# TropComplique/MultiPoseNet

Measured on AMD Instinct MI355X. Metric: images/sec keypoint fwd+bwd+Adam @512x512 bs32/GPU, higher is better.
Workload: dtype bf16; 1 GPU; MobileNet-v1+FPN+keypoint_subnet fwd+bwd+Adam, 512x512, per-GPU batch 32; global_batch=32, parallelism=dp1, hip_graph=True, rccl_ranks=1

## Files before the change

include/mpn.h:

```cpp
#ifndef MPN_H_
#define MPN_H_

#include <stddef.h>
#include <stdint.h>

#ifdef __cplusplus
extern "C" {
#endif

#define MPN_VERSION 600

enum { MPN_F32 = 0, MPN_BF16 = 1, MPN_F16 = 2  };

enum {
    MPN_OK = 0,
    MPN_ERR_BAD_SHAPE = -1,
    MPN_ERR_BAD_DTYPE = -2,
    MPN_ERR_BAD_ALIGN = -3,
    MPN_ERR_HIP = -4,
    MPN_ERR_BAD_ARG = -5,
    MPN_ERR_WORKSPACE = -6
};

enum { MPN_ACT_NONE = 0, MPN_ACT_RELU = 1, MPN_ACT_RELU6 = 2 };

typedef void* mpn_stream_t;

int mpn_version(void);
int mpn_last_error(char* buf, size_t n);

size_t mpn_heatmap_decode_workspace_bytes(int B);
int mpn_heatmap_decode(const void* heatmaps, int dtype, int B, int h, int w, int C,
                       const double* box_hw, float threshold,
                       int32_t* out_xyv, float* out_score, int32_t* out_index,
                       void* workspace, size_t workspace_bytes, mpn_stream_t stream);

size_t mpn_conv_packed_bytes(int Cin, int Cout, int ksize, int transpose, int dtype);
int mpn_conv_pack_weights(const float* w_hwio, int Cin, int Cout, int ksize, int transpose,
                          int dtype, void* out, mpn_stream_t stream);
size_t mpn_conv_pack_desc_bytes(void);
int mpn_conv_pack_desc_fill(void* desc_host, const float* w_hwio, int Cin, int Cout, int ksize, int transpose,
                            int dtype, void* out, int block_begin);
int mpn_conv_pack_weights_batched(const void* descs_device, int ndesc, int total_blocks, int dtype,
                                  mpn_stream_t stream);
int mpn_conv_num_parts(int N, int H, int W, int ksize);
int mpn_conv_stats_rows(int N, int H, int W, int Cin, int Cout, int ksize, int dtype);
int mpn_conv_fwd(const void* x, const void* w_packed, void* y, int N, int H, int W, int Cin,
                 int Cout, int x_stride, int y_stride, int ksize, int dtype, const float* in_scale,
                 const float* in_shift, int in_act, float* stats_part, const void* up_res,
                 mpn_stream_t stream);
int mpn_conv_fwd_grouped(int njobs, const void* const* x, const void* const* w_packed, void* const* y, int N, const int* H,
                         const int* W, int Cin, int Cout, const int* x_stride, const int* y_stride, int ksize, int dtype,
                         const float* const* in_scale, const float* const* in_shift, int in_act,
                         float* const* stats_part, mpn_stream_t stream);
int mpn_conv_bwd_data_bn_supported(int K, int C, int ksize, int dtype);
int mpn_conv_bwd_data_bn(const void* dy, const void* w_packed_t, void* dx, int N, int H, int W, int K, int C, int dy_stride,
                         int dx_stride, int ksize, int dtype, const void* bn_x, int bn_x_stride, const float* bn_scale,
                         const float* bn_shift, int bn_act, float* part, mpn_stream_t stream);
int mpn_conv_bwd_data_bn_grouped(int njobs, const void* const* dy, const void* const* w_packed_t, void* const* dx, int N,
                                 const int* H, const int* W, int K, int C, const int* dy_stride, const int* dx_stride,
                                 int dtype, const void* const* bn_x, const int* bn_x_stride, const float* const* bn_scale,
                                 const float* const* bn_shift, int bn_act, float* const* part, mpn_stream_t stream);

int mpn_conv_wgrad_num_parts(int N, int H, int W, int Cin, int Cout, int ksize, int dtype);
int mpn_conv_bwd_weight(const void* x, const void* dy, float* part, int N, int H, int W, int Cin,
                        int Cout, int x_stride, int dy_stride, int ksize, int dtype, const float* in_scale,
                        const float* in_shift, int in_act, mpn_stream_t stream);

int mpn_conv1x1_bwd_fused_supported(int Cin, int Cout, int dtype);
int mpn_conv1x1_bwd_fused(const void* x, const void* dy, const float* w, void* dx, float* wpart, float* bn_part, int N, int H, int W,
                          int Cin, int Cout, int x_stride, int dy_stride, int dx_stride, int dtype, const float* in_scale,
                          const float* in_shift, int in_act, mpn_stream_t stream);
int mpn_conv1x1_bwd_fused_apply_supported(int Cin, int Cout, int dtype);
int mpn_conv1x1_bwd_fused_apply(const void* x, const void* g, const void* y_raw, const float* w, void* dx, float* wpart, float* bn_part,
                                int N, int H, int W, int Cin, int Cout, int x_stride, int g_stride, int y_stride, int dx_stride,
                                int dtype, const float* in_scale, const float* in_shift, int in_act, const float* ap_scale,
                                const float* ap_shift, const float* ap_mean, const float* ap_invstd, const float* ap_k1,
                                const float* ap_k2, int ap_act, mpn_stream_t stream);
int mpn_conv_wgrad_grouped_num_parts(int njobs, int N, const int* H, const int* W, int Cin, int Cout, int ksize, int dtype,
                                     int* nparts);
int mpn_conv_bwd_weight_grouped(int njobs, const void* const* x, const void* const* dy, float* const* part, int N,
                                const int* H, const int* W, int Cin, int Cout, const int* x_stride, const int* dy_stride,
                                int ksize, int dtype, const float* const* in_scale, const float* const* in_shift,
                                int in_act, mpn_stream_t stream);

int mpn_bn_stats_num_parts(long long M);
int mpn_bn_stats(const void* x, long long M, int C, int dtype, float* part, mpn_stream_t stream);
int mpn_bn_finalize(float* part, int nparts, int C, long long count, const float* gamma,
                    const float* beta, float* moving_mean, float* moving_var, float momentum,
                    float eps, float* scale, float* shift, float* save_mean, float* save_invstd,
                    mpn_stream_t stream);
int mpn_bn_bwd_reduce_grouped(int njobs, void* const* dA, const void* const* x, const long long* M, int C, int dtype,
                              const float* const* scale, const float* const* shift, const float* const* mean,
                              const float* const* invstd, int act, float* const* part, const int* dA_stride,
                              const int* x_stride, mpn_stream_t stream);
int mpn_bn_bwd_apply_grouped(int njobs, void* const* dA, const void* const* x, const long long* M, int C, int dtype,
                             const float* const* scale, const float* const* shift, const float* const* mean,
                             const float* const* invstd, const float* const* k1, const float* const* k2, int act,
                             const float* const* add_ch0, const int* dA_stride, const int* x_stride,
                             mpn_stream_t stream);
size_t mpn_bn_fin_desc_bytes(void);
size_t mpn_bn_bwd_fin_desc_bytes(void);
int mpn_bn_fin_desc_fill(void* desc_host, const float* part, int nparts, int C, long long count, const float* gamma,
                         const float* beta, float* moving_mean, float* moving_var, float* scale, float* shift,
                         float* save_mean, float* save_invstd, int block_begin);
int mpn_bn_bwd_fin_desc_fill(void* desc_host, const float* part, int nparts, int C, long long count, float* dgamma,
                             float* dbeta, float* k1, float* k2, int block_begin);
int mpn_bn_bwd_fin_desc_fill_raw(void* desc_host, const float* part, int nparts, int C, long long count, float* dgamma,
                                 float* dbeta, float* k1, float* k2, const float* mean, const float* invstd,
                                 int block_begin);
int mpn_bn_finalize_batched(const void* descs_device, int ndesc, int total_blocks, float momentum, float eps,
                            mpn_stream_t stream);
int mpn_bn_bwd_finalize_batched(const void* descs_device, int ndesc, int total_blocks, mpn_stream_t stream);
int mpn_bn_inference_affine(int C, const float* gamma, const float* beta, const float* moving_mean,
                            const float* moving_var, float eps, float* scale, float* shift,
                            mpn_stream_t stream);
int mpn_bn_act_apply(const void* x, void* y, long long M, int C, int dtype, const float* scale,
                     const float* shift, int act, mpn_stream_t stream);
int mpn_bn_bwd_reduce(const void* dA, const void* x, long long M, int C, int dtype,
                      const float* scale, const float* shift, const float* mean,
                      const float* invstd, int act, float* part, mpn_stream_t stream);
int mpn_bn_bwd_finalize(float* part, int nparts, int C, long long count, float* dgamma,
                        float* dbeta, float* k1, float* k2, mpn_stream_t stream);
int mpn_bn_bwd_finalize_raw(float* part, int nparts, int C, long long count, float* dgamma, float* dbeta, float* k1,
                            float* k2, const float* mean, const float* invstd, mpn_stream_t stream);
int mpn_bn_bwd_apply(void* dA, const void* x, long long M, int C, int dtype, const float* scale,
                     const float* shift, const float* mean, const float* invstd, const float* k1,
                     const float* k2, int act, const float* add_ch0, mpn_stream_t stream);

int mpn_dwconv_out_size(int size, int stride);
int mpn_dwconv_num_parts(int N, int H, int W, int C, int stride, int dtype);
int mpn_dwconv_fwd(const void* x, const float* w, void* y, int N, int H, int W, int C, int stride,
                   int dtype, const float* in_scale, const float* in_shift, int in_act, int flip,
                   float* stats_part, mpn_stream_t stream);
int mpn_dwconv_bwd_data(const void* dy, const float* w, void* dx, int N, int H, int W, int C,
                        int stride, int dtype, mpn_stream_t stream);
int mpn_dwconv_bwd_data_bn_num_parts(int N, int H, int W, int C, int stride, int dtype);
int mpn_dwconv_bwd_data_bn(const void* dy, const float* w, void* dx, int N, int H, int W, int C, int stride, int dtype,
                           const void* x_bn, const float* scale, const float* shift, const float* mean,
                           const float* invstd, int act, float* part, mpn_stream_t stream);
int mpn_dwconv_bwd_data_add_supported(int N, int H, int W, int C, int stride, int dtype);
int mpn_dwconv_bwd_data_add(const void* dy, const float* w, void* dx, int N, int H, int W, int C, int stride, int dtype,
                            const void* addend, const void* x_bn, const float* scale, const float* shift,
                            const float* mean, const float* invstd, int act, float* part, mpn_stream_t stream);
int mpn_dwconv_wgrad_num_parts(int N, int H, int W, int C, int stride, int dtype);
int mpn_dwconv_bwd_weight(const void* x, const void* dy, float* part, int N, int H, int W, int C,
                          int stride, int dtype, const float* in_scale, const float* in_shift,
                          int in_act, mpn_stream_t stream);

int mpn_dwconv_bwd_fused_supported(int N, int H, int W, int C, int stride, int dtype);
int mpn_dwconv_bwd_fused(const void* x, const void* dy, const float* w, void* dx, float* wpart, int N, int H, int W, int C,
                         int dtype, const float* in_scale, const float* in_shift, int in_act, const float* mean,
                         const float* invstd, float* bn_part, mpn_stream_t stream);
int mpn_dwconv_bwd_fused_s2(const void* x, const void* dy, const float* w, void* dx, float* wpart, int N, int H, int W, int C,
                            int dtype, const float* in_scale, const float* in_shift, int in_act, const float* mean,
                            const float* invstd, float* bn_part, const void* addend, mpn_stream_t stream);

int mpn_stem_conv_fwd(const void* images, int images_u8, const float* w, void* y, int N, int H,
                      int W, int C0, int dtype, mpn_stream_t stream);
int mpn_stem_conv_fwd_num_parts(int N, int H, int W, int C0, int dtype);
int mpn_stem_conv_fwd_stats(const void* images, int images_u8, const float* w, void* y, int N, int H, int W, int C0,
                            int dtype, float* stats_part, mpn_stream_t stream);
int mpn_stem_conv_wgrad_num_parts(int N, int H, int W);
int mpn_stem_conv_bwd_weight(const void* images, int images_u8, const void* dy, float* part, int N,
                             int H, int W, int C0, int dtype, mpn_stream_t stream);

int mpn_bilinear_up_fwd(const void* x, void* y, int N, int h, int w, int C, int upsample,
                        int y_channel_offset, int y_channels_total, int dtype,
                        const float* in_scale, const float* in_shift, int in_act,
                        mpn_stream_t stream);
int mpn_bilinear_up_bwd(const void* dy, void* dx, int N, int h, int w, int C, int upsample,
                        int y_channel_offset, int y_channels_total, int dtype, mpn_stream_t stream);
int mpn_sumpool2x2(const void* src, void* dst, int N, int h, int w, int C, int accumulate,
                   int dtype, mpn_stream_t stream);
int mpn_add_inplace(void* dst, const void* src, long long n, int dtype, mpn_stream_t stream);

int mpn_heatmap_head_fwd(const void* x, const float* w, const float* bias, long long M, int Cin,
                         int dtype, const float* in_scale, const float* in_shift, int in_act,
                         int mode, float* out, float* out_seg, mpn_stream_t stream);
int mpn_heatmap_head_bwd_num_parts(long long M);
int mpn_heatmap_head_bwd(const void* x, const float* dlogits, const float* w, long long M, int Cin,
                         int dtype, const float* in_scale, const float* in_shift, int in_act,
                         void* dA, float* part, mpn_stream_t stream);
int mpn_heatmap_head_bwd_bn_supported(int Cin, int dtype);
int mpn_heatmap_head_bwd_bn(const void* x, const float* dlogits, const float* w, long long M, int Cin, int dtype,
                            const float* in_scale, const float* in_shift, int in_act, void* dA, float* part,
                            float* bn_part, mpn_stream_t stream);

int mpn_keypoint_loss_num_parts(int B, int h, int w);
int mpn_keypoint_loss(const float* logits, const float* heatmaps, const float* loss_masks,
                      const float* segmentation_masks, const int* num_boxes, const void* p2,
                      const void* p3, const void* p4, const void* p5, int p_channels, int p_dtype,
                      float* dlogits, float* daux2, float* daux3, float* daux4, float* daux5,
                      float* part, float* losses_out, int B, int h, int w, mpn_stream_t stream);

int mpn_adam_prepare(long long* step, float* hyper, double initial_learning_rate,
                     double decay_steps, double alpha, double beta1, double beta2,
                     mpn_stream_t stream);
int mpn_adam_step(float* params, const float* grads, float* m, float* v, long long n,
                  const float* hyper, float beta1, float beta2, float eps, float clip,
                  float grad_scale, mpn_stream_t stream);
int mpn_adam_step_cast(float* params, const float* grads, float* m, float* v, long long n, const float* hyper, float beta1,
                       float beta2, float eps, float clip, float grad_scale, int ncast, const long long* cast_begin,
                       const long long* cast_count, void* const* cast_dst, int cast_dtype, mpn_stream_t stream);
int mpn_reduce_partials(const float* part, int nparts, long long n, float* out, int accumulate,
                        float scale, mpn_stream_t stream);
size_t mpn_reduce_desc_bytes(void);
int mpn_reduce_desc_fill(void* desc_host, const float* part, int nparts, long long n, float* out, float scale,
                         int block_begin);
int mpn_reduce_partials_batched(const void* descs_device, int ndesc, int total_blocks, mpn_stream_t stream);
int mpn_axpy(long long n, float a, const float* x, float* y, mpn_stream_t stream);
int mpn_axpy_batched(int count, const float* const* x, float* const* y, const long long* n, float a, mpn_stream_t stream);
int mpn_l2_loss_accumulate(long long n, const float* w, float scale, float* acc, mpn_stream_t stream);
size_t mpn_l2_loss_batched_workspace_bytes(int count, const long long* n);
int mpn_l2_loss_batched(int count, const float* const* w, const long long* n, float scale, float* acc, void* workspace,
                        size_t workspace_bytes, mpn_stream_t stream);

size_t mpn_heatmap_render_workspace_bytes(int total_persons);
int mpn_heatmap_render(const int32_t* keypoints, const float* boxes, const int32_t* first_person,
                       int B, int total_persons, int width, int height, int downsample, float* out,
                       void* workspace, size_t workspace_bytes, mpn_stream_t stream);

enum {
    MPN_AUGMENT_ROTATE = 1, MPN_AUGMENT_COLOR = 2, MPN_AUGMENT_GRAYSCALE = 4, MPN_AUGMENT_PIXEL_SCALE = 8,
    MPN_AUGMENT_FLIP = 16, MPN_AUGMENT_EVAL = 32
};
#define MPN_KEYPOINT_AUGMENT_DESC_BYTES 192
typedef struct mpn_keypoint_augment_desc {
    int64_t src_offset, mask_offset;
    int32_t src_h, src_w, mask_h, mask_w;
    int32_t crop_y, crop_x, crop_h, crop_w;
    int32_t valid_h, valid_w, valid_mh, valid_mw;
    float transform[8], mask_transform[8];
    float window[4];
    float scale_y, scale_x;
    float mask_scale_y, mask_scale_x;
    float color[3];
    uint32_t seed;
    int32_t flags;
    int32_t reserved[3];
} mpn_keypoint_augment_desc;
#ifdef __cplusplus
static_assert(sizeof(mpn_keypoint_augment_desc) == MPN_KEYPOINT_AUGMENT_DESC_BYTES, "descriptor size is fixed");
#endif
size_t mpn_keypoint_augment_desc_bytes(void);
int mpn_keypoint_augment(const uint8_t* sources, const uint8_t* masks, const void* descs, int B, int H, int W,
                         float* images, float* loss_masks, float* segmentation_masks, mpn_stream_t stream);

// ... 89 lines not shown
```

multiposenet_amd/_lib.py:

```python
import ctypes
import os

_HERE = os.path.dirname(os.path.abspath(__file__))
LIB_PATH = os.environ.get("MPN_LIB") or os.path.join(_HERE, "libmpn_hip.so")

MPN_VERSION = 600
MPN_F32, MPN_BF16, MPN_F16 = 0, 1, 2
ACT_NONE, ACT_RELU, ACT_RELU6 = 0, 1, 2

_c = ctypes
_P = _c.c_void_p
_I = _c.c_int
_F = _c.c_float
_D = _c.c_double
_Z = _c.c_size_t
_L = _c.c_longlong

SIGNATURES = {
    "mpn_version": (_I, []),
    "mpn_last_error": (_I, [_c.c_char_p, _Z]),
    "mpn_heatmap_decode_workspace_bytes": (_Z, [_I]),
    "mpn_heatmap_decode": (_I, [_P, _I, _I, _I, _I, _I, _P, _F, _P, _P, _P, _P, _Z, _P]),
    "mpn_heatmap_render_workspace_bytes": (_Z, [_I]),
    "mpn_heatmap_render": (_I, [_P, _P, _P, _I, _I, _I, _I, _I, _P, _P, _Z, _P]),
    "mpn_keypoint_augment_desc_bytes": (_Z, []),
    "mpn_keypoint_augment": (_I, [_P, _P, _P, _I, _I, _I, _P, _P, _P, _P]),
    "mpn_detector_augment_desc_bytes": (_Z, []),
    "mpn_detector_augment": (_I, [_P, _P, _I, _I, _I, _P, _P]),
    "mpn_prn_example_desc_bytes": (_Z, []),
    "mpn_prn_examples_workspace_bytes": (_Z, [_I]),
    "mpn_prn_examples": (_I, [_P, _P, _I, _P, _P, _P, _I, _P, _I, _I, _I, _I, _P, _P, _P, _Z, _P]),
    "mpn_conv_packed_bytes": (_Z, [_I, _I, _I, _I, _I]),
    "mpn_conv_pack_weights": (_I, [_P, _I, _I, _I, _I, _I, _P, _P]),
    "mpn_conv_pack_desc_bytes": (_Z, []),
    "mpn_conv_pack_desc_fill": (_I, [_P, _P, _I, _I, _I, _I, _I, _P, _I]),
    "mpn_conv_pack_weights_batched": (_I, [_P, _I, _I, _I, _P]),
    "mpn_conv_num_parts": (_I, [_I, _I, _I, _I]),
    "mpn_conv_stats_rows": (_I, [_I, _I, _I, _I, _I, _I, _I]),
    "mpn_conv_fwd": (_I, [_P, _P, _P, _I, _I, _I, _I, _I, _I, _I, _I, _I, _P, _P, _I, _P, _P, _P]),
    "mpn_conv_fwd_grouped": (_I, [_I, _P, _P, _P, _I, _P, _P, _I, _I, _P, _P, _I, _I, _P, _P, _I, _P, _P]),
    "mpn_conv_wgrad_num_parts": (_I, [_I, _I, _I, _I, _I, _I, _I]),
    "mpn_conv_bwd_weight": (_I, [_P, _P, _P, _I, _I, _I, _I, _I, _I, _I, _I, _I, _P, _P, _I, _P]),
    "mpn_conv1x1_bwd_fused_supported": (_I, [_I, _I, _I]),
    "mpn_conv1x1_bwd_fused": (_I, [_P, _P, _P, _P, _P, _P, _I, _I, _I, _I, _I, _I, _I, _I, _I, _P, _P, _I, _P]),
    "mpn_conv1x1_bwd_fused_apply_supported": (_I, [_I, _I, _I]),
    "mpn_conv1x1_bwd_fused_apply": (_I, [_P, _P, _P, _P, _P, _P, _P, _I, _I, _I, _I, _I, _I, _I, _I, _I, _I, _P, _P, _I, _P, _P, _P, _P, _P, _P, _I, _P]),
    "mpn_conv_wgrad_grouped_num_parts": (_I, [_I, _I, _P, _P, _I, _I, _I, _I, _P]),
    "mpn_conv_bwd_weight_grouped": (_I, [_I, _P, _P, _P, _I, _P, _P, _I, _I, _P, _P, _I, _I, _P, _P, _I, _P]),
    "mpn_bn_stats_num_parts": (_I, [_L]),
    "mpn_bn_stats": (_I, [_P, _L, _I, _I, _P, _P]),
    "mpn_bn_finalize": (_I, [_P, _I, _I, _L, _P, _P, _P, _P, _F, _F, _P, _P, _P, _P, _P]),
    "mpn_bn_inference_affine": (_I, [_I, _P, _P, _P, _P, _F, _P, _P, _P]),
    "mpn_bn_act_apply": (_I, [_P, _P, _L, _I, _I, _P, _P, _I, _P]),
    "mpn_bn_bwd_reduce": (_I, [_P, _P, _L, _I, _I, _P, _P, _P, _P, _I, _P, _P]),
    "mpn_bn_bwd_finalize": (_I, [_P, _I, _I, _L, _P, _P, _P, _P, _P]),
    "mpn_bn_bwd_apply": (_I, [_P, _P, _L, _I, _I, _P, _P, _P, _P, _P, _P, _I, _P, _P]),
    "mpn_dwconv_out_size": (_I, [_I, _I]),
    "mpn_dwconv_num_parts": (_I, [_I, _I, _I, _I, _I, _I]),
    "mpn_dwconv_fwd": (_I, [_P, _P, _P, _I, _I, _I, _I, _I, _I, _P, _P, _I, _I, _P, _P]),
    "mpn_dwconv_bwd_data": (_I, [_P, _P, _P, _I, _I, _I, _I, _I, _I, _P]),
    "mpn_dwconv_bwd_data_bn_num_parts": (_I, [_I, _I, _I, _I, _I, _I]),
    "mpn_dwconv_bwd_data_bn": (_I, [_P, _P, _P, _I, _I, _I, _I, _I, _I, _P, _P, _P, _P, _P, _I, _P, _P]),
    "mpn_dwconv_bwd_data_add_supported": (_I, [_I, _I, _I, _I, _I, _I]),
    "mpn_dwconv_bwd_data_add": (_I, [_P, _P, _P, _I, _I, _I, _I, _I, _I, _P, _P, _P, _P, _P, _P, _I, _P, _P]),
    "mpn_dwconv_wgrad_num_parts": (_I, [_I, _I, _I, _I, _I, _I]),
    "mpn_dwconv_bwd_weight": (_I, [_P, _P, _P, _I, _I, _I, _I, _I, _I, _P, _P, _I, _P]),
    "mpn_dwconv_bwd_fused_supported": (_I, [_I, _I, _I, _I, _I, _I]),
    "mpn_dwconv_bwd_fused": (_I, [_P, _P, _P, _P, _P, _I, _I, _I, _I, _I, _P, _P, _I, _P, _P, _P, _P]),
    "mpn_dwconv_bwd_fused_s2": (_I, [_P, _P, _P, _P, _P, _I, _I, _I, _I, _I, _P, _P, _I, _P, _P, _P, _P, _P]),
    "mpn_stem_conv_fwd": (_I, [_P, _I, _P, _P, _I, _I, _I, _I, _I, _P]),
    "mpn_stem_conv_fwd_num_parts": (_I, [_I, _I, _I, _I, _I]),
    "mpn_stem_conv_fwd_stats": (_I, [_P, _I, _P, _P, _I, _I, _I, _I, _I, _P, _P]),
    "mpn_stem_conv_wgrad_num_parts": (_I, [_I, _I, _I]),
    "mpn_stem_conv_bwd_weight": (_I, [_P, _I, _P, _P, _I, _I, _I, _I, _I, _P]),
    "mpn_bilinear_up_fwd": (_I, [_P, _P, _I, _I, _I, _I, _I, _I, _I, _I, _P, _P, _I, _P]),
    "mpn_bilinear_up_bwd": (_I, [_P, _P, _I, _I, _I, _I, _I, _I, _I, _I, _P]),
    "mpn_sumpool2x2": (_I, [_P, _P, _I, _I, _I, _I, _I, _I, _P]),
    "mpn_add_inplace": (_I, [_P, _P, _L, _I, _P]),
    "mpn_heatmap_head_fwd": (_I, [_P, _P, _P, _L, _I, _I, _P, _P, _I, _I, _P, _P, _P]),
    "mpn_heatmap_head_bwd_num_parts": (_I, [_L]),
    "mpn_heatmap_head_bwd": (_I, [_P, _P, _P, _L, _I, _I, _P, _P, _I, _P, _P, _P]),
    "mpn_heatmap_head_bwd_bn_supported": (_I, [_I, _I]),
    "mpn_heatmap_head_bwd_bn": (_I, [_P, _P, _P, _L, _I, _I, _P, _P, _I, _P, _P, _P, _P]),
    "mpn_keypoint_loss_num_parts": (_I, [_I, _I, _I]),
    "mpn_keypoint_loss": (_I, [_P] * 9 + [_I, _I] + [_P] * 7 + [_I, _I, _I, _P]),
    "mpn_adam_prepare": (_I, [_P, _P, _D, _D, _D, _D, _D, _P]),
    "mpn_adam_step": (_I, [_P, _P, _P, _P, _L, _P, _F, _F, _F, _F, _F, _P]),
    "mpn_adam_step_cast": (_I, [_P, _P, _P, _P, _L, _P, _F, _F, _F, _F, _F, _I, _P, _P, _P, _I, _P]),
    "mpn_reduce_partials": (_I, [_P, _I, _L, _P, _I, _F, _P]),
    "mpn_reduce_desc_bytes": (_Z, []),
    "mpn_reduce_desc_fill": (_I, [_P, _P, _I, _L, _P, _F, _I]),
    "mpn_reduce_partials_batched": (_I, [_P, _I, _I, _P]),
    "mpn_gemm_nt_num_parts": (_I, [_I]),
    "mpn_gemm_nt": (_I, [_P, _P, _P, _I, _I, _I, _I, _P]),
    "mpn_transpose_cast": (_I, [_P, _I, _P, _I, _I, _I, _P]),
    "mpn_cast": (_I, [_P, _I, _P, _I, _L, _P]),
    "mpn_bias_relu_fwd": (_I, [_P, _I, _P, _P, _I, _I, _I, _P]),
    "mpn_bias_relu_bwd": (_I, [_P, _I, _P, _P, _I, _P, _I, _I, _P]),
    "mpn_prn_loss": (_I, [_P, _P, _I, _P, _I, _I, _I, _P, _P, _P, _F, _P]),
    "mpn_bn_bwd_reduce_grouped": (_I, [_I, _P, _P, _P, _I, _I, _P, _P, _P, _P, _I, _P, _P, _P, _P]),
    "mpn_bn_bwd_apply_grouped": (_I, [_I, _P, _P, _P, _I, _I, _P, _P, _P, _P, _P, _P, _I, _P, _P, _P, _P]),
    "mpn_bn_fin_desc_bytes": (_Z, []),
    "mpn_bn_bwd_fin_desc_bytes": (_Z, []),
    "mpn_bn_fin_desc_fill": (_I, [_P, _P, _I, _I, _L, _P, _P, _P, _P, _P, _P, _P, _P, _I]),
    "mpn_bn_bwd_fin_desc_fill": (_I, [_P, _P, _I, _I, _L, _P, _P, _P, _P, _I]),
    "mpn_bn_finalize_batched": (_I, [_P, _I, _I, _F, _F, _P]),
    "mpn_bn_bwd_finalize_batched": (_I, [_P, _I, _I, _P]),
    "mpn_heatmap_minmax": (_I, [_P, _I, _I, _I, _I, _P, _P]),
    "mpn_prn_crop": (_I, [_P, _P, _P, _P, _I, _I, _I, _I, _I, _I, _I, _F, _P, _P]),
    "mpn_prn_decode": (_I, [_P, _I, _I, _I, _I, _P, _P, _P]),
    "mpn_conv_bwd_data_bn_supported": (_I, [_I, _I, _I, _I]),
    "mpn_conv_bwd_data_bn": (_I, [_P, _P, _P, _I, _I, _I, _I, _I, _I, _I, _I, _I, _P, _I, _P, _P, _I, _P, _P]),
    "mpn_bn_bwd_finalize_raw": (_I, [_P, _I, _I, _L, _P, _P, _P, _P, _P, _P, _P]),
    "mpn_conv_bwd_data_bn_grouped": (_I, [_I, _P, _P, _P, _I, _P, _P, _I, _I, _P, _P, _I, _P, _P, _P, _P, _I, _P, _P]),
    "mpn_bn_bwd_fin_desc_fill_raw": (_I, [_P, _P, _I, _I, _L, _P, _P, _P, _P, _P, _P, _I]),
    "mpn_prn_crop_slots": (_I, [_P, _P, _P, _P, _I, _I, _I, _I, _I, _I, _I, _I, _I, _F, _P, _P]),
    "mpn_prn_residual": (_I, [_P, _P, _I, _L, _P, _P]),
    "mpn_retina_loss_finalize": (_I, [_P, _P, _F, _F, _P, _P, _P, _P]),
    "mpn_axpy": (_I, [_L, _F, _P, _P, _P]),
    "mpn_axpy_batched": (_I, [_I, _P, _P, _P, _F, _P]),
    "mpn_patchify3x3s2": (_I, [_P, _P, _I, _I, _I, _I, _I, _P, _P, _I, _P]),
    "mpn_unpatchify3x3s2": (_I, [_P, _P, _I, _I, _I, _I, _I, _P]),
    "mpn_retina_match_workspace_bytes": (_Z, [_I, _I]),
    "mpn_retina_match": (_I, [_P, _P, _P, _I, _I, _I, _F, _F, _P, _P, _P, _P, _Z, _P]),
    "mpn_retina_loss_num_parts": (_I, [_I, _I]),
    "mpn_retina_loss": (_I, [_P, _P, _P, _P, _P, _P, _I, _P, _P, _P, _P, _P, _I, _F, _F, _F, _F, _P, _P]),
    "mpn_retina_nms_workspace_bytes": (_Z, [_I, _I]),
    "mpn_retina_nms_overflow_offset": (_Z, [_I, _I]),
    "mpn_retina_nms": (_I, [_P, _P, _P, _P, _I, _P, _P, _P, _I, _F, _F, _I, _P, _P, _P, _P, _Z, _P]),
    "mpn_l2_loss_accumulate": (_I, [_L, _P, _F, _P, _P]),
    "mpn_l2_loss_batched_workspace_bytes": (_Z, [_I, _P]),
    "mpn_l2_loss_batched": (_I, [_I, _P, _P, _F, _P, _P, _Z, _P]),
}

_lib = None


class MpnError(RuntimeError):
    pass


def lib():
    global _lib
    if _lib is None:
        if not os.path.exists(LIB_PATH):
            raise MpnError(
                f"{LIB_PATH} not found: build it with `python -m multiposenet_amd.build` "
                "(there is no CPU fallback)")
        import torch
        hip_rt = os.path.join(os.path.dirname(torch.__file__), "lib", "libamdhip64.so")
        if os.path.exists(hip_rt):
            ctypes.CDLL(hip_rt, mode=ctypes.RTLD_GLOBAL)
        l = ctypes.CDLL(LIB_PATH)
        l.mpn_version.restype = _I
        if l.mpn_version() != MPN_VERSION:
            raise MpnError(f"{LIB_PATH} is ABI revision {l.mpn_version()}, this binding needs {MPN_VERSION}: "
                           "rebuild with `python -m multiposenet_amd.build --force`")
# ... 115 lines not shown
```

multiposenet_amd/csrc/common.h:

```cpp
#pragma once
#include <hip/hip_runtime.h>
#include <stdint.h>
#include <stddef.h>
#include <atomic>
#include "../../include/mpn.h"

void mpn_set_error(const char* fmt, ...);

#define MPN_FAIL(code, ...)            \
    do {                               \
        mpn_set_error(__VA_ARGS__);    \
        return (code);                 \
    } while (0)

#define MPN_REQUIRE(cond, code, ...)   \
    do {                               \
        if (!(cond)) MPN_FAIL(code, __VA_ARGS__); \
    } while (0)

#define MPN_LAUNCH_CHECK()                                                        \
    do {                                                                          \
        hipError_t e_ = hipGetLastError();                                        \
        if (e_ != hipSuccess)                                                     \
            MPN_FAIL(MPN_ERR_HIP, "%s:%d launch failed: %s", __FILE__, __LINE__, \
                     hipGetErrorString(e_));                                      \
    } while (0)

#define MPN_HIP(call)                                                             \
    do {                                                                          \
        hipError_t e_ = (call);                                                   \
        if (e_ != hipSuccess)                                                     \
            MPN_FAIL(MPN_ERR_HIP, "%s:%d %s: %s", __FILE__, __LINE__, #call,      \
                     hipGetErrorString(e_));                                      \
    } while (0)

typedef std::atomic<unsigned long long> mpn_attr_mask_t;
static inline hipError_t mpn_ensure_dynamic_lds(const void* func, int bytes, mpn_attr_mask_t* mask) {
    int dev = 0;
    hipError_t e = hipGetDevice(&dev);
    if (e != hipSuccess) return e;
    const unsigned long long bit = 1ull << (dev & 63);
    if (mask->load(std::memory_order_acquire) & bit) return hipSuccess;
    e = hipFuncSetAttribute(func, hipFuncAttributeMaxDynamicSharedMemorySize, bytes);
    if (e == hipSuccess) mask->fetch_or(bit, std::memory_order_release);
    return e;
}

static inline bool mpn_aligned16(const void* p) { return (((uintptr_t)p) & 15u) == 0; }

typedef __bf16 bf16_t;
typedef _Float16 half_t;

template <typename T> struct StoreTraits;
template <> struct StoreTraits<float> {
    static constexpr int kDtype = MPN_F32;
    static constexpr int kVec = 4;
};
template <> struct StoreTraits<bf16_t> {
    static constexpr int kDtype = MPN_BF16;
    static constexpr int kVec = 8;
};
template <> struct StoreTraits<half_t> {
    static constexpr int kDtype = MPN_F16;
    static constexpr int kVec = 8;
};

__device__ __forceinline__ float to_f32(float x) { return x; }
__device__ __forceinline__ float to_f32(bf16_t x) { return (float)x; }
__device__ __forceinline__ float to_f32(half_t x) { return (float)x; }
template <typename T> __device__ __forceinline__ T from_f32(float x);
template <> __device__ __forceinline__ float from_f32<float>(float x) { return x; }
template <> __device__ __forceinline__ bf16_t from_f32<bf16_t>(float x) { return (bf16_t)x; }
template <> __device__ __forceinline__ half_t from_f32<half_t>(float x) { return (half_t)x; }

__device__ __forceinline__ unsigned pack_bf16x2(float lo, float hi) {
    typedef __bf16 b2_t __attribute__((ext_vector_type(2)));
    typedef float f2_t __attribute__((ext_vector_type(2)));
    const f2_t v = {lo, hi};
    return __builtin_bit_cast(unsigned, __builtin_convertvector(v, b2_t));
}

template <typename T> struct Vec16;
template <> struct Vec16<float> {
    static constexpr int N = 4;
    float4 raw;
    __device__ __forceinline__ void load(const float* p) { raw = *reinterpret_cast<const float4*>(p); }
    __device__ __forceinline__ void load_nt(const float* p) {
        typedef float f32x4n_t __attribute__((ext_vector_type(4)));
        const f32x4n_t q = __builtin_nontemporal_load(reinterpret_cast<const f32x4n_t*>(p));
        raw = make_float4(q.x, q.y, q.z, q.w);
    }
    __device__ __forceinline__ void store(float* p) const { *reinterpret_cast<float4*>(p) = raw; }
    __device__ __forceinline__ void zero() { raw = make_float4(0.f, 0.f, 0.f, 0.f); }
    __device__ __forceinline__ void unpack(float (&f)[4]) const { f[0] = raw.x; f[1] = raw.y; f[2] = raw.z; f[3] = raw.w; }
    __device__ __forceinline__ void pack(const float (&f)[4]) { raw = make_float4(f[0], f[1], f[2], f[3]); }
};
template <> struct Vec16<bf16_t> {
    static constexpr int N = 8;
    uint4 raw;
    __device__ __forceinline__ void load(const bf16_t* p) { raw = *reinterpret_cast<const uint4*>(p); }
    __device__ __forceinline__ void load_nt(const bf16_t* p) {
        typedef unsigned u32x4_t __attribute__((ext_vector_type(4)));
        const u32x4_t q = __builtin_nontemporal_load(reinterpret_cast<const u32x4_t*>(p));
        raw = make_uint4(q.x, q.y, q.z, q.w);
    }
    __device__ __forceinline__ void store(bf16_t* p) const { *reinterpret_cast<uint4*>(p) = raw; }
    __device__ __forceinline__ void zero() { raw = make_uint4(0u, 0u, 0u, 0u); }
    __device__ __forceinline__ void unpack(float (&f)[8]) const {
        const unsigned u[4] = {raw.x, raw.y, raw.z, raw.w};
#pragma unroll
        for (int i = 0; i < 4; ++i) {
            f[2 * i] = __uint_as_float(u[i] << 16);
            f[2 * i + 1] = __uint_as_float(u[i] & 0xffff0000u);
        }
    }
    __device__ __forceinline__ void pack(const float (&f)[8]) {
        unsigned u[4];
#pragma unroll
        for (int i = 0; i < 4; ++i) {
            u[i] = pack_bf16x2(f[2 * i], f[2 * i + 1]);
        }
        raw = make_uint4(u[0], u[1], u[2], u[3]);
    }
};

template <> struct Vec16<half_t> {
    static constexpr int N = 8;
    uint4 raw;
    __device__ __forceinline__ void load(const half_t* p) { raw = *reinterpret_cast<const uint4*>(p); }
    __device__ __forceinline__ void load_nt(const half_t* p) {
        typedef unsigned u32x4_t __attribute__((ext_vector_type(4)));
        const u32x4_t q = __builtin_nontemporal_load(reinterpret_cast<const u32x4_t*>(p));
        raw = make_uint4(q.x, q.y, q.z, q.w);
    }
    __device__ __forceinline__ void store(half_t* p) const { *reinterpret_cast<uint4*>(p) = raw; }
    __device__ __forceinline__ void zero() { raw = make_uint4(0u, 0u, 0u, 0u); }
    __device__ __forceinline__ void unpack(float (&f)[8]) const {
        typedef _Float16 h2_t __attribute__((ext_vector_type(2)));
        const unsigned u[4] = {raw.x, raw.y, raw.z, raw.w};
#pragma unroll
        for (int i = 0; i < 4; ++i) {
            const h2_t h = __builtin_bit_cast(h2_t, u[i]);
            f[2 * i] = (float)h[0];
            f[2 * i + 1] = (float)h[1];
        }
    }
    __device__ __forceinline__ void pack(const float (&f)[8]) {
        typedef _Float16 h2_t __attribute__((ext_vector_type(2)));
        unsigned u[4];
#pragma unroll
        for (int i = 0; i < 4; ++i) {
            const h2_t h = {(_Float16)f[2 * i], (_Float16)f[2 * i + 1]};
            u[i] = __builtin_bit_cast(unsigned, h);
        }
        raw = make_uint4(u[0], u[1], u[2], u[3]);
    }
};

template <typename T> struct H16;
template <> struct H16<bf16_t> {
    typedef __bf16 x8 __attribute__((ext_vector_type(8)));
    typedef __bf16 x4 __attribute__((ext_vector_type(4)));
    typedef float acc_t __attribute__((ext_vector_type(4)));
    static __device__ __forceinline__ acc_t mfma(const x8& a, const x8& b, const acc_t& c) {
// ... 42 lines not shown
```

multiposenet_amd/csrc/conv_wgrad.hip:

```cpp
#include "common.h"
#include <type_traits>

namespace {

template <typename T> using HT = H16<std::conditional_t<sizeof(T) == 2, T, bf16_t>>;
typedef float f32x4_t __attribute__((ext_vector_type(4)));

constexpr int kThreads = 256;
constexpr int kHaloW = 18, kHaloH = 10;

struct WgradParams {
    const void* x;
    const void* dy;
    float* part;
    const float* in_scale;
    const float* in_shift;
    int in_act;
    int N, H, W, Cin, Cout;
    int xs, dys;
    int tiles_x, tiles_y;
    long long M;
    int ntiles;
    int nsplit;
    int n_cg, n_cb;
    int xcd_remap;
    const float* wf;
    void* dx;
    int dxs;
    float* bn_part;
    const void* ap_x;
    int ap_xs;
    const float* ap_scale; const float* ap_shift; const float* ap_mean; const float* ap_invstd; const float* ap_k1; const float* ap_k2;
    int ap_act;
#ifdef MPN_DIAG
    unsigned long long* dbg;
#endif
};

__device__ __forceinline__ int fsw256(int r) { return (r & 3) | (((r >> 3) & 1) << 2); }
__device__ __forceinline__ int fsw64(int) { return 0; }
__device__ __forceinline__ int fsw128(int r) { return ((r >> 1) & 1) | (((r >> 3) & 1) << 1); }

template <int RB> __device__ __forceinline__ int lds_off(int row, int seg, int within) {
    const int f = (RB == 64) ? fsw64(row) : (RB == 128 ? fsw128(row) : fsw256(row));
    return row * RB + ((seg ^ f) << 5) + within;
}

template <typename T> struct Raw4h { uint2 v; };
__device__ __forceinline__ void raw4_unpack(const Raw4h<bf16_t>& r, float (&f)[4]) {
    f[0] = __uint_as_float(r.v.x << 16); f[1] = __uint_as_float(r.v.x & 0xffff0000u);
    f[2] = __uint_as_float(r.v.y << 16); f[3] = __uint_as_float(r.v.y & 0xffff0000u);
}
__device__ __forceinline__ void raw4_unpack(const Raw4h<half_t>& r, float (&f)[4]) {
    typedef _Float16 h2_t __attribute__((ext_vector_type(2)));
    const h2_t a = __builtin_bit_cast(h2_t, r.v.x), b = __builtin_bit_cast(h2_t, r.v.y);
    f[0] = (float)a[0]; f[1] = (float)a[1]; f[2] = (float)b[0]; f[3] = (float)b[1];
}
template <typename T> __device__ __forceinline__ float round_to_storage(float v);
template <> __device__ __forceinline__ float round_to_storage<bf16_t>(float v) { return to_f32((bf16_t)v); }
template <> __device__ __forceinline__ float round_to_storage<half_t>(float v) { return (float)(_Float16)v; }
template <typename T> __device__ __forceinline__ uint2 pack4_storage(const float (&g)[4]);
template <> __device__ __forceinline__ uint2 pack4_storage<bf16_t>(const float (&g)[4]) {
    return make_uint2(pack_bf16x2(g[0], g[1]), pack_bf16x2(g[2], g[3]));
}
template <> __device__ __forceinline__ uint2 pack4_storage<half_t>(const float (&g)[4]) {
    typedef _Float16 h2_t __attribute__((ext_vector_type(2)));
    const h2_t a = {(_Float16)g[0], (_Float16)g[1]}, b = {(_Float16)g[2], (_Float16)g[3]};
    return make_uint2(__builtin_bit_cast(unsigned, a), __builtin_bit_cast(unsigned, b));
}

template <typename H> __device__ __forceinline__ typename H::x4 tr_read(const unsigned char* base, int off) {
    return H::tr_read(base + off);
}

template <typename T, int TAPS, int RBA, int RBD>
__global__ __launch_bounds__(kThreads, 2) void conv_wgrad_kernel(const WgradParams p) {
    constexpr int ES = (int)sizeof(T);
    constexpr int VE = 16 / ES;
    constexpr int CG = RBA / ES;
    constexpr int BNW = RBD / ES;
    constexpr int DSLOTS = RBD / 16;
    constexpr int NPIXA = TAPS == 9 ? kHaloW * kHaloH : 128;
    constexpr int MT_TOTAL = CG / 16, NT_TOTAL = BNW / 16;
    constexpr int WM = MT_TOTAL >= 2 ? 2 : 1;
    constexpr int WN = 4 / WM;
    constexpr int MTW = MT_TOTAL / WM;
    constexpr int NTW = NT_TOTAL / WN;
    constexpr int KPIX = ES == 2 ? 32 : 4;
    constexpr int KSTEPS = 128 / KPIX;
    constexpr int ASLOTS = RBA / 16;
    constexpr int AVEC = (NPIXA * ASLOTS + kThreads - 1) / kThreads;
    constexpr int DVEC = 128 * DSLOTS / kThreads;

    extern __shared__ __attribute__((aligned(16))) unsigned char smem[];
    unsigned char* As = smem;
    unsigned char* Ds = smem + NPIXA * RBA;

    const int tid = threadIdx.x;
    const int lane = tid & 63, wave = tid >> 6;
    const int l15 = lane & 15, lq = lane >> 4;

    int b;
    {
        const int nwg = gridDim.x, q = nwg >> 3, r = nwg & 7, xcd = blockIdx.x & 7, k = blockIdx.x >> 3;
        b = (xcd < r ? xcd * (q + 1) : r * (q + 1) + (xcd - r) * q) + k;
    }
    const int cg = b % p.n_cg; b /= p.n_cg;
    const int cb = b % p.n_cb;
    const int split = b / p.n_cb;
    const int ci0 = cg * CG, co0 = cb * BNW;

    const int mt0 = (wave / WN) * MTW;
    const int nt0 = (wave % WN) * NTW;

    f32x4_t acc[TAPS][MTW][NTW];
#pragma unroll
// ... 166 lines not shown
    for (int t = 0; t < TAPS; ++t)
#pragma unroll
        for (int i = 0; i < MTW; ++i)
#pragma unroll
            for (int j = 0; j < NTW; ++j)
#pragma unroll
                for (int r = 0; r < 4; ++r) {
                    const int ci = ci0 + (mt0 + i) * 16 + lq * 4 + r;
                    const int co = co0 + (nt0 + j) * 16 + l15;
                    if (ci < p.Cin && co < p.Cout)
                        dst[((long long)t * p.Cin + ci) * p.Cout + co] = acc[t][i][j][r];
                }
}

template <typename T, int TAPS, int RBA, int RBD, int WM, bool STAGGER, bool DG = false, bool DAPPLY = false>
__device__ __forceinline__ void conv_wgrad_bf16_body(const WgradParams& p, const int blk, const int nblk) {
    using H = H16<T>;
    using X8 = typename H::x8;
    using X4 = typename H::x4;
    constexpr int NT = 512;
    constexpr int VE = 8;
    constexpr int CG = RBA / 2, BNW = RBD / 2;
    constexpr int ASLOTS = RBA / 16, DSLOTS = RBD / 16;
    constexpr int NPIXA = TAPS == 9 ? kHaloW * kHaloH : 128;
    constexpr int MT_TOTAL = CG / 16, NT_TOTAL = BNW / 16;
    constexpr int WN = 8 / WM;
    constexpr int MTW = MT_TOTAL / WM, NTW = NT_TOTAL / WN;
    static_assert(MTW * WM == MT_TOTAL && NTW * WN == NT_TOTAL, "wave layout must tile the block");
    constexpr int AVEC = (NPIXA * ASLOTS + NT - 1) / NT;
    constexpr int DVEC = 128 * DSLOTS / NT;
    constexpr int SA = RBA + 32, SD = RBD + 32;
    constexpr int ABYTES = NPIXA * SA, DBYTES = 128 * SD;
    static_assert(!DG || (TAPS == 1 && !STAGGER), "the fused data gradient: 1x1, waves in step");
    constexpr int OS = RBA + 16;
    constexpr int RBYTES = DG ? 128 * SA : 0, OBYTES = DG ? 128 * OS : 0;
    constexpr int KS2 = BNW / 32;

    constexpr int NBUF = DG ? 1 : 2;
    extern __shared__ __attribute__((aligned(16))) unsigned char smem[];
    float* aff = reinterpret_cast<float*>(smem + NBUF * ABYTES + NBUF * DBYTES);
    unsigned char* Rs = smem + NBUF * ABYTES + NBUF * DBYTES + 2 * CG * (int)sizeof(float);
    unsigned char* Os = Rs + RBYTES;

    const int tid = threadIdx.x;
    const int lane = tid & 63, wave = tid >> 6;
    const int l15 = lane & 15, lq = lane >> 4;

    int b = blk;
    if (p.xcd_remap) {
        const int nwg = nblk, q = nwg >> 3, r = nwg & 7, xcd = blk & 7, k = blk >> 3;
        b = (xcd < r ? xcd * (q + 1) : r * (q + 1) + (xcd - r) * q) + k;
    }
    const int cg = b % p.n_cg; b /= p.n_cg;
    const int cb = b % p.n_cb;
    const int split = b / p.n_cb;
    const int ci0 = cg * CG, co0 = cb * BNW;
    const int mt0 = (wave / WN) * MTW, nt0 = (wave % WN) * NTW;

    f32x4_t acc[TAPS][MTW][NTW];
#pragma unroll
    for (int t = 0; t < TAPS; ++t)
#pragma unroll
        for (int i = 0; i < MTW; ++i)
#pragma unroll
            for (int j = 0; j < NTW; ++j) acc[t][i][j] = (f32x4_t){0.f, 0.f, 0.f, 0.f};

    const T* __restrict__ x = reinterpret_cast<const T*>(p.x);
    const T* __restrict__ dy = reinterpret_cast<const T*>(p.dy);
    const bool affine = p.in_scale != nullptr;
    const float lo = (affine && p.in_act != MPN_ACT_NONE) ? 0.f : -INFINITY;
    const float hi = (affine && p.in_act == MPN_ACT_RELU6) ? 6.f : INFINITY;
    for (int c = tid; c < CG; c += NT) {
        const bool ok = affine && ci0 + c < p.Cin;
        aff[c] = ok ? p.in_scale[ci0 + c] : 1.f;
        aff[CG + c] = ok ? p.in_shift[ci0 + c] : 0.f;
    }

    const int aslot = tid % ASLOTS;
    const int dslot = tid % DSLOTS;

    Vec16<T> v[AVEC], dv[DVEC];
    Vec16<T> ev[DAPPLY ? DVEC : 1];
    unsigned inb = 0u, inbd = 0u;
    static_assert(!DAPPLY || DG, "the apply pass folds into the fused thin backward");
    float* apc = reinterpret_cast<float*>(Os + OBYTES + (DG ? 8 * 2 * CG * (int)sizeof(float) : 0));
    float alo = -INFINITY, ahi = INFINITY;
    if constexpr (DAPPLY) {
        for (int c = tid; c < BNW; c += NT) {
            const bool ok = co0 + c < p.Cout;
            const float s_ = ok ? p.ap_scale[co0 + c] : 0.f, h_ = ok ? p.ap_shift[co0 + c] : 0.f, m_ = ok ? p.ap_mean[co0 + c] : 0.f;
            const float i_ = ok ? p.ap_invstd[co0 + c] : 0.f, a_ = ok ? p.ap_k1[co0 + c] : 0.f, b_ = ok ? p.ap_k2[co0 + c] : 0.f;
            apc[c] = s_; apc[BNW + c] = h_;
            apc[2 * BNW + c] = -s_ * b_ * i_;
            apc[3 * BNW + c] = -s_ * (a_ - m_ * i_ * b_);
        }
        alo = (p.ap_act != MPN_ACT_NONE) ? 0.f : -INFINITY;
        ahi = (p.ap_act == MPN_ACT_RELU6) ? 6.f : INFINITY;
    }

    int relA[AVEC], hyx[AVEC], relD[DVEC];
    {
        const int ace = ci0 + aslot * VE, dce = co0 + dslot * VE;
#pragma unroll
        for (int i = 0; i < AVEC; ++i) {
            const int vi = tid + i * NT;
            const int pix = vi / ASLOTS;
            const bool ok = ace < p.Cin && vi < NPIXA * ASLOTS;
            if (TAPS == 9) {
                const int hy = pix / kHaloW, hx = pix - hy * kHaloW;
                relA[i] = ((hy - 1) * p.W + (hx - 1)) * p.xs + ace;
                hyx[i] = ok ? (hy << 8 | hx) : 0x7fff00;
            } else {
                relA[i] = pix * p.xs + ace;
                hyx[i] = ok ? pix : 0x7fffffff;
            }
        }
#pragma unroll
        for (int i = 0; i < DVEC; ++i) {
            const int r = (tid / DSLOTS) + i * (NT / DSLOTS);
            relD[i] = (TAPS == 9 ? ((r >> 4) * p.W + (r & 15)) : r) * p.dys + dce;
        }
    }
    const bool dvalid = co0 + dslot * VE < p.Cout;
    const int drow0 = tid / DSLOTS;
    constexpr bool BUF = TAPS == 1;
    typedef unsigned u32x4_t __attribute__((ext_vector_type(4)));
    unsigned relAb[BUF ? AVEC : 1], relDb[BUF ? DVEC : 1], relEb[(BUF && DAPPLY) ? DVEC : 1];
    __amdgpu_buffer_rsrc_t rsx, rsd, rse;
    if constexpr (BUF) {
        constexpr unsigned kOut = 0x80000000u;
#pragma unroll
        for (int i = 0; i < AVEC; ++i) relAb[i] = hyx[i] == 0x7fffffff ? kOut : (unsigned)relA[i] * (unsigned)sizeof(T);
#pragma unroll
        for (int i = 0; i < DVEC; ++i) relDb[i] = dvalid ? (unsigned)relD[i] * (unsigned)sizeof(T) : kOut;
        rsx = __builtin_amdgcn_make_buffer_rsrc(const_cast<T*>(x), 0, (int)(((p.M - 1) * p.xs + p.Cin) * (long long)sizeof(T)), 0x00020000);
        rsd = __builtin_amdgcn_make_buffer_rsrc(const_cast<T*>(dy), 0, (int)(((p.M - 1) * p.dys + p.Cout) * (long long)sizeof(T)), 0x00020000);
        if constexpr (DAPPLY) {
#pragma unroll
            for (int i = 0; i < DVEC; ++i)
                relEb[i] = dvalid ? (unsigned)((drow0 + i * (NT / DSLOTS)) * p.ap_xs + co0 + dslot * VE) * (unsigned)sizeof(T) : kOut;
            rse = __builtin_amdgcn_make_buffer_rsrc(const_cast<void*>(p.ap_x), 0, (int)(((p.M - 1) * p.ap_xs + p.Cout) * (long long)sizeof(T)), 0x00020000);
        }
    }

    auto load_tile = [&](int tile) {
        if constexpr (BUF) {
            const unsigned tbA = (unsigned)tile * 128u * (unsigned)p.xs * (unsigned)sizeof(T);
            const unsigned tbD = (unsigned)tile * 128u * (unsigned)p.dys * (unsigned)sizeof(T);
            if constexpr (DAPPLY) {
                const int mleft = (int)(p.M - (long long)tile * 128);
                unsigned md = 0u;
#pragma unroll
                for (int i = 0; i < DVEC; ++i) md |= ((dvalid && drow0 + i * (NT / DSLOTS) < mleft) ? 1u : 0u) << i;
                inbd = md;
            }
            __builtin_amdgcn_sched_barrier(0);
#pragma unroll
            for (int i = 0; i < AVEC; ++i) {
                const u32x4_t q = __builtin_amdgcn_raw_buffer_load_b128(rsx, (int)(relAb[i] + tbA), 0, 0);
                v[i].raw = make_uint4(q.x, q.y, q.z, q.w);
            }
#pragma unroll
            for (int i = 0; i < DVEC; ++i) {
                const u32x4_t q = __builtin_amdgcn_raw_buffer_load_b128(rsd, (int)(relDb[i] + tbD), 0, 0);
                dv[i].raw = make_uint4(q.x, q.y, q.z, q.w);
            }
            if constexpr (DAPPLY) {
                const unsigned tbE = (unsigned)tile * 128u * (unsigned)p.ap_xs * (unsigned)sizeof(T);
#pragma unroll
                for (int i = 0; i < DVEC; ++i) {
                    const u32x4_t q = __builtin_amdgcn_raw_buffer_load_b128(rse, (int)(relEb[i] + tbE), 0, 0);
                    ev[i].raw = make_uint4(q.x, q.y, q.z, q.w);
                }
            }
            __builtin_amdgcn_sched_barrier(0);
            return;
        }
        int oy0 = 0, ox0 = 0, baseA, baseD, mleft = 0;
        if (TAPS == 9) {
            const int tx = tile % p.tiles_x;
            const int t2 = tile / p.tiles_x;
            const int ty = t2 % p.tiles_y;
            const int img = t2 / p.tiles_y;
            oy0 = ty * 8;
            ox0 = tx * 16;
            const int pix0 = (img * p.H + oy0) * p.W + ox0;
            baseA = pix0 * p.xs;
            baseD = pix0 * p.dys;
        } else {
            baseA = tile * 128 * p.xs;
            baseD = tile * 128 * p.dys;
            mleft = (int)(p.M - (long long)tile * 128);
        }
        int oa[AVEC], od[DVEC];
        unsigned ma = 0u, md = 0u;
#pragma unroll
        for (int i = 0; i < AVEC; ++i) {
            bool ok;
            if (TAPS == 9) {
                const int iy = oy0 + (hyx[i] >> 8) - 1, ix = ox0 + (hyx[i] & 255) - 1;
                ok = (unsigned)iy < (unsigned)p.H && (unsigned)ix < (unsigned)p.W;
            } else {
                ok = hyx[i] < mleft;
            }
            oa[i] = ok ? baseA + relA[i] : 0;
            ma |= (ok ? 1u : 0u) << i;
        }
#pragma unroll
        for (int i = 0; i < DVEC; ++i) {
            const int r = drow0 + i * (NT / DSLOTS);
            bool ok = dvalid;
            if (TAPS == 9) ok = ok && oy0 + (r >> 4) < p.H && ox0 + (r & 15) < p.W;
            else ok = ok && r < mleft;
            od[i] = ok ? baseD + relD[i] : 0;
            md |= (ok ? 1u : 0u) << i;
        }
        inb = ma;
        inbd = md;
        __builtin_amdgcn_sched_barrier(0);
#pragma unroll
        for (int i = 0; i < AVEC; ++i) v[i].load(x + oa[i]);
#pragma unroll
        for (int i = 0; i < DVEC; ++i) dv[i].load(dy + od[i]);
        if constexpr (DAPPLY) {
            const T* __restrict__ ax = reinterpret_cast<const T*>(p.ap_x);
#pragma unroll
            for (int i = 0; i < DVEC; ++i) {
                const int r = drow0 + i * (NT / DSLOTS);
                const bool ok = (inbd >> i) & 1u;
                ev[i].load(ax + (ok ? (long long)(tile * 128 + r) * p.ap_xs + co0 + dslot * VE : 0));
            }
        }
        __builtin_amdgcn_sched_barrier(0);
    };

    auto commit_tile = [&](unsigned char* As, unsigned char* Ds) {
        float sc[VE], sh[VE];
        if (affine) {
#pragma unroll
            for (int j = 0; j < VE; j += 4) {
                const float4 a = *reinterpret_cast<const float4*>(aff + aslot * VE + j);
                const float4 c = *reinterpret_cast<const float4*>(aff + CG + aslot * VE + j);
                sc[j] = a.x; sc[j + 1] = a.y; sc[j + 2] = a.z; sc[j + 3] = a.w;
                sh[j] = c.x; sh[j + 1] = c.y; sh[j + 2] = c.z; sh[j + 3] = c.w;
            }
        }
#pragma unroll
        for (int i = 0; i < AVEC; ++i) {
            const int vi = tid + i * NT;
            if (vi < NPIXA * ASLOTS) {
                const int pix = vi / ASLOTS;
                uint4 q = *reinterpret_cast<const uint4*>(&v[i].raw);
                if (affine) {
                    float f[VE];
                    v[i].unpack(f);
#pragma unroll
                    for (int j = 0; j < VE; ++j) f[j] = __builtin_amdgcn_fmed3f(f[j] * sc[j] + sh[j], lo, hi);
                    Vec16<T> o;
                    o.pack(f);
                    q = *reinterpret_cast<const uint4*>(&o.raw);
                }
                if (!BUF && !((inb >> i) & 1u)) q = make_uint4(0u, 0u, 0u, 0u);
                *reinterpret_cast<uint4*>(As + pix * SA + aslot * 16) = q;
                if constexpr (DG) {
                    uint4 r = *reinterpret_cast<const uint4*>(&v[i].raw);
                    if (!BUF && !((inb >> i) & 1u)) r = make_uint4(0u, 0u, 0u, 0u);
                    *reinterpret_cast<uint4*>(Rs + pix * SA + aslot * 16) = r;
                }
            }
        }
#pragma unroll
        for (int i = 0; i < DVEC; ++i) {
            const int r = (tid / DSLOTS) + i * (NT / DSLOTS);
            uint4 q = *reinterpret_cast<const uint4*>(&dv[i].raw);
            if constexpr (DAPPLY) {
                float d[VE], f[VE], asc[VE], ash[VE], acb[VE], acc_[VE];
                dv[i].unpack(d);
                ev[i].unpack(f);
#pragma unroll
                for (int j4 = 0; j4 < VE; j4 += 4) {
                    const f32x4_t q0 = *reinterpret_cast<const f32x4_t*>(apc + dslot * VE + j4), q1 = *reinterpret_cast<const f32x4_t*>(apc + BNW + dslot * VE + j4);
                    const f32x4_t q2 = *reinterpret_cast<const f32x4_t*>(apc + 2 * BNW + dslot * VE + j4), q3 = *reinterpret_cast<const f32x4_t*>(apc + 3 * BNW + dslot * VE + j4);
#pragma unroll
                    for (int j = 0; j < 4; ++j) { asc[j4 + j] = q0[j]; ash[j4 + j] = q1[j]; acb[j4 + j] = q2[j]; acc_[j4 + j] = q3[j]; }
                }
#pragma unroll
                for (int j = 0; j < VE; ++j) {
                    const float pre = f[j] * asc[j] + ash[j];
                    const float gg = (pre > alo && pre < ahi) ? d[j] : 0.f;
                    d[j] = asc[j] * gg + (acb[j] * f[j] + acc_[j]);
                }
                Vec16<T> o;
                o.pack(d);
                q = *reinterpret_cast<const uint4*>(&o.raw);
            }
            if ((!BUF || DAPPLY) && !((inbd >> i) & 1u)) q = make_uint4(0u, 0u, 0u, 0u);
            *reinterpret_cast<uint4*>(Ds + r * SD + dslot * 16) = q;
        }
    };

#ifdef MPN_DIAG
    unsigned long long ph[4] = {0, 0, 0, 0}, t_prev = 0;
#define MPN_WG_STAMP(k) do { if (p.dbg) { const unsigned long long t_ = __builtin_amdgcn_s_memtime(); \
                                          ph[k] += t_ - t_prev; t_prev = t_; } } while (0)
#else
#define MPN_WG_STAMP(k) do { } while (0)
#endif
    const int grp = STAGGER ? wave >> 2 : 0;
    const int ntl = p.ntiles > split ? (p.ntiles - split + p.nsplit - 1) / p.nsplit : 0;
    const int ahead = 1 + grp;
    constexpr int DGS = MT_TOTAL >= 8 ? 4 : (MT_TOTAL >= 4 ? 2 : 1), MTH = MT_TOTAL / DGS;
    const int dg_mt0 = DG ? (wave % DGS) * MTH : 0, dg_pt0 = DG ? (wave / DGS) * DGS : 0;
    X8 wfr[DG ? MTH : 1][DG ? KS2 : 1];
    float bsum[DG ? MTH : 1][4], bsq[DG ? MTH : 1][4];
    if constexpr (DG) {
#pragma unroll
        for (int mt = 0; mt < MTH; ++mt) {
#pragma unroll
            for (int ks = 0; ks < KS2; ++ks) {
                const int ci = ci0 + (dg_mt0 + mt) * 16 + l15, co = co0 + ks * 32 + lq * 8;
                float f[8];
#pragma unroll
                for (int j = 0; j < 8; ++j) f[j] = (ci < p.Cin && co + j < p.Cout) ? p.wf[(long long)ci * p.Cout + co + j] : 0.f;
                Vec16<T> o;
                o.pack(f);
                wfr[mt][ks] = __builtin_bit_cast(X8, o.raw);
            }
#pragma unroll
            for (int r = 0; r < 4; ++r) { bsum[mt][r] = 0.f; bsq[mt][r] = 0.f; }
        }
    }
    if (ntl > 0) load_tile(split);
    __syncthreads();
    if (ntl > 0) commit_tile(smem, smem + NBUF * ABYTES);
    if (grp == 1) {
        if (ntl > 1) load_tile(split + p.nsplit);
        __syncthreads();
        if (ntl > 1) commit_tile(smem + ABYTES, smem + NBUF * ABYTES + DBYTES);
    }
#ifdef MPN_DIAG
    if (p.dbg) t_prev = __builtin_amdgcn_s_memtime();
#endif
#pragma unroll 1
    for (int it = 0; it < ntl; ++it) {
        const int buf = NBUF == 2 ? (it & 1) : 0;
        unsigned char* As = smem + buf * ABYTES;
        unsigned char* Ds = smem + NBUF * ABYTES + buf * DBYTES;
        const bool more = it + ahead < ntl;
        if (more) load_tile(split + (it + ahead) * p.nsplit);
        MPN_WG_STAMP(1);
        __syncthreads();
        MPN_WG_STAMP(2);
        const int qq = l15 >> 2, pp = l15 & 3;
        const unsigned char* a_lane = As + (4 * lq + qq) * SA + pp * 8 + mt0 * 32;
        const unsigned char* d_lane = Ds + (4 * lq + qq) * SD + pp * 8 + nt0 * 32;
        constexpr int STEPS = TAPS * MTW;
        constexpr int TOTAL = 4 * STEPS;
        constexpr int RING0 = NTW >= 4 ? 4 : ((TAPS == 9 && RBA == 256) ? 4 : 6);
        constexpr int RING = RING0 < STEPS ? RING0 : STEPS;
        constexpr int KSA = (TAPS == 9 ? 2 * kHaloW : 32) * SA, KSD = 32 * SD;
        auto a_load = [&](int gs) -> X8 {
            const int ks = gs / STEPS, step = gs % STEPS;
            const int t = step / MTW, i = step % MTW;
            const int row = TAPS == 9 ? (t / 3) * kHaloW + (t % 3) : 0;
            const int second = TAPS == 9 ? kHaloW : 16;
            const X4 l4 = tr_read<H>(a_lane, ks * KSA + row * SA + i * 32);
            const X4 h4 = tr_read<H>(a_lane, ks * KSA + (row + second) * SA + i * 32);
            return __builtin_shufflevector(l4, h4, 0, 1, 2, 3, 4, 5, 6, 7);
        };
        auto b_load = [&](int ks, int j) -> X8 {
            const X4 l4 = tr_read<H>(d_lane, ks * KSD + j * 32);
            const X4 h4 = tr_read<H>(d_lane, ks * KSD + 16 * SD + j * 32);
            return __builtin_shufflevector(l4, h4, 0, 1, 2, 3, 4, 5, 6, 7);
        };
        X8 bfr[2][NTW];
        X8 ar[RING];
#pragma unroll
        for (int j = 0; j < NTW; ++j) bfr[0][j] = b_load(0, j);
#pragma unroll
        for (int r = 0; r < RING - 1; ++r) ar[r] = a_load(r);
        __builtin_amdgcn_sched_barrier(0);
#pragma unroll
        for (int gs = 0; gs < TOTAL; ++gs) {
            const int ks = gs / STEPS, step = gs % STEPS;
            if (step == STEPS - RING && ks + 1 < 4) {
#pragma unroll
                for (int j = 0; j < NTW; ++j) bfr[(ks + 1) & 1][j] = b_load(ks + 1, j);
            }
            if (gs + RING - 1 < TOTAL) ar[(gs + RING - 1) % RING] = a_load(gs + RING - 1);
            const int t = step / MTW, i = step % MTW;
#pragma unroll
            for (int j = 0; j < NTW; ++j)
                acc[t][i][j] = H::mfma(ar[gs % RING], bfr[ks & 1][j], acc[t][i][j]);
            __builtin_amdgcn_sched_barrier(0);
        }
        if constexpr (DG) {
            const bool bnr = p.bn_part != nullptr;
#pragma unroll 1
            for (int j = 0; j < DGS; ++j) {
                const int px = (dg_pt0 + j) * 16 + l15;
                f32x4_t dacc[MTH];
#pragma unroll
                for (int mt = 0; mt < MTH; ++mt) dacc[mt] = (f32x4_t){0.f, 0.f, 0.f, 0.f};
#pragma unroll
                for (int ks = 0; ks < KS2; ++ks) {
                    const X8 dfr = *reinterpret_cast<const X8*>(Ds + px * SD + ks * 64 + lq * 16);
#pragma unroll
                    for (int mt = 0; mt < MTH; ++mt) dacc[mt] = H::mfma(wfr[mt][ks], dfr, dacc[mt]);
                }
#pragma unroll
                for (int mt = 0; mt < MTH; ++mt) {
                    const int cl = (dg_mt0 + mt) * 16 + lq * 4;
                    Raw4h<T> r4;
                    r4.v = *reinterpret_cast<const uint2*>(Rs + px * SA + cl * 2);
                    float xf[4];
                    raw4_unpack(r4, xf);
                    const f32x4_t sc4 = *reinterpret_cast<const f32x4_t*>(aff + cl), sh4 = *reinterpret_cast<const f32x4_t*>(aff + CG + cl);
                    float g[4];
#pragma unroll
                    for (int r = 0; r < 4; ++r) {
                        const float pre = xf[r] * sc4[r] + sh4[r];
                        const float d = round_to_storage<T>(dacc[mt][r]);
                        g[r] = (!bnr || (pre > lo && pre < hi)) ? d : 0.f;
                        bsum[mt][r] += g[r];
                        bsq[mt][r] += g[r] * xf[r];
                    }
                    *reinterpret_cast<uint2*>(Os + px * OS + cl * 2) = pack4_storage<T>(g);
                }
            }
        }
        MPN_WG_STAMP(3);
        __syncthreads();
        MPN_WG_STAMP(2);
        if (more) {
            const int nb = NBUF == 2 ? ((it + ahead) & 1) : 0;
            commit_tile(smem + nb * ABYTES, smem + NBUF * ABYTES + nb * DBYTES);
        }
        if constexpr (DG) {
            const int tile = split + it * p.nsplit;
            const int mleft = (int)(p.M - (long long)tile * 128);
            T* __restrict__ dxp = reinterpret_cast<T*>(p.dx) + (long long)tile * 128 * p.dxs + ci0;
            for (int v0 = tid; v0 < 128 * ASLOTS; v0 += NT) {
                const int pr = v0 / ASLOTS, sl = v0 - pr * ASLOTS;
                if (pr < mleft && ci0 + sl * 8 < p.Cin)
                    *reinterpret_cast<uint4*>(dxp + (long long)pr * p.dxs + sl * 8) = *reinterpret_cast<const uint4*>(Os + pr * OS + sl * 16);
            }
        }
        MPN_WG_STAMP(0);
    }
    if (STAGGER && grp == 0) __syncthreads();
#ifdef MPN_DIAG
    if (p.dbg && lane == 0) {
#pragma unroll
        for (int k = 0; k < 4; ++k) p.dbg[((size_t)blockIdx.x * 8 + wave) * 4 + k] = ph[k];
    }
#endif
#undef MPN_WG_STAMP

    if constexpr (DG) {
        float* red = reinterpret_cast<float*>(Os + OBYTES);
        __syncthreads();
        for (int o = tid; o < 8 * 2 * CG; o += NT) red[o] = 0.f;
        __syncthreads();
#pragma unroll
        for (int mt = 0; mt < MTH; ++mt)
#pragma unroll
            for (int r = 0; r < 4; ++r) {
                float a = bsum[mt][r], b = bsq[mt][r];
#pragma unroll
                for (int o = 1; o < 16; o <<= 1) { a += __shfl_xor(a, o, 64); b += __shfl_xor(b, o, 64); }
                if (l15 == 0) {
                    red[(wave * 2 + 0) * CG + (dg_mt0 + mt) * 16 + lq * 4 + r] = a;
                    red[(wave * 2 + 1) * CG + (dg_mt0 + mt) * 16 + lq * 4 + r] = b;
                }
            }
        __syncthreads();
        for (int o = tid; o < 2 * CG; o += NT) {
            const int which = o / CG, c = o - which * CG;
            if (p.bn_part != nullptr && ci0 + c < p.Cin) {
                float a = 0.f;
#pragma unroll
                for (int w8 = 0; w8 < 8; ++w8) a += red[(w8 * 2 + which) * CG + c];
                p.bn_part[((long long)split * 2 + which) * p.Cin + ci0 + c] = a;
            }
        }
    }
    float* __restrict__ dst = p.part + (long long)split * TAPS * p.Cin * p.Cout;
#pragma unroll
    for (int t = 0; t < TAPS; ++t)
#pragma unroll
        for (int i = 0; i < MTW; ++i)
#pragma unroll
            for (int j = 0; j < NTW; ++j)
#pragma unroll
                for (int r = 0; r < 4; ++r) {
                    const int ci = ci0 + (mt0 + i) * 16 + lq * 4 + r;
                    const int co = co0 + (nt0 + j) * 16 + l15;
                    if (ci < p.Cin && co < p.Cout) {
                        __builtin_nontemporal_store(acc[t][i][j][r], &dst[((long long)t * p.Cin + ci) * p.Cout + co]);
                    }
                }
}

template <typename T, int TAPS, int RBA, int RBD, int WM, bool STAGGER>
__global__ __launch_bounds__(512, 1) void conv_wgrad_bf16_kernel(const WgradParams p) {
    conv_wgrad_bf16_body<T, TAPS, RBA, RBD, WM, STAGGER>(p, blockIdx.x, gridDim.x);
}

template <typename T, int RBA, int RBD, int WM, bool DAPPLY>
__global__ __launch_bounds__(512, 1) void conv1x1_bwd_fused_kernel(const WgradParams p) {
    conv_wgrad_bf16_body<T, 1, RBA, RBD, WM, false, true, DAPPLY>(p, blockIdx.x, gridDim.x);
}

constexpr int kMaxWgradGroup = 5;
struct WgradGroup {
    WgradParams p[kMaxWgradGroup];
    int begin[kMaxWgradGroup + 1];
    int njobs;
};
template <typename T, int TAPS, int RBA, int RBD, int WM, bool STAGGER>
__global__ __launch_bounds__(512, 1) void conv_wgrad_bf16_grouped_kernel(const WgradGroup g) {
    int job = 0;
#pragma unroll
    for (int j = 1; j < kMaxWgradGroup; ++j)
        if (j < g.njobs && (int)blockIdx.x >= g.begin[j]) job = j;
    conv_wgrad_bf16_body<T, TAPS, RBA, RBD, WM, STAGGER>(g.p[job], (int)blockIdx.x - g.begin[job], g.begin[job + 1] - g.begin[job]);
}

struct WgradGeom {
    int n_cg, n_cb, ntiles, nsplit;
};

static bool wgrad_thin1x1(int Cin, int Cout, int ksize) { return ksize == 1 && Cin <= 32 && Cout <= 64; }

WgradGeom wgrad_geom(int N, int H, int W, int Cin, int Cout, int ksize, int es) {
    WgradGeom g;
    int cgsz, bnw, blocks;
    if (es == 2) {
        const bool narrow = ksize == 3 && Cout <= 64;
        cgsz = (ksize == 3 && !narrow) ? 64 : 128;
        bnw = narrow ? 64 : 128;
        if (wgrad_thin1x1(Cin, Cout, ksize)) { cgsz = 32; bnw = 64; }
        blocks = 256;
    } else {
        const bool narrow = ksize == 3 && Cout * es <= 128;
        cgsz = (narrow ? 128 : (ksize == 3 ? 64 : 256)) / es;
        bnw = (narrow ? 128 : 256) / es;
        blocks = 512;
    }
    g.n_cg = (Cin + cgsz - 1) / cgsz;
    g.n_cb = (Cout + bnw - 1) / bnw;
    g.ntiles = ksize == 3 ? N * ((H + 7) / 8) * ((W + 15) / 16) : (int)(((long long)N * H * W + 127) / 128);
    int ns = blocks / (g.n_cg * g.n_cb);
    if (ns < 1) ns = 1;
    const int min_tiles = es == 2 ? 4 : 1;
    if (ns > g.ntiles / min_tiles) ns = g.ntiles / min_tiles;
    if (ns < 1) ns = 1;
    g.nsplit = ns;
    return g;
}

template <typename T, int TAPS, int RBA, int RBD, int WM, bool STAGGER>
int launch_wgrad_bf16(const WgradParams& p, hipStream_t st) {
    constexpr int NPIXA = TAPS == 9 ? kHaloW * kHaloH : 128;
    constexpr int smem = 2 * NPIXA * (RBA + 32) + 2 * 128 * (RBD + 32) + 2 * (RBA / 2) * (int)sizeof(float);
    static_assert(smem <= 160 * 1024, "LDS budget");
    static mpn_attr_mask_t attr_mask{0};
    MPN_HIP(mpn_ensure_dynamic_lds((const void*)conv_wgrad_bf16_kernel<T, TAPS, RBA, RBD, WM, STAGGER>, smem, &attr_mask));
    conv_wgrad_bf16_kernel<T, TAPS, RBA, RBD, WM, STAGGER><<<dim3((unsigned)(p.n_cg * p.n_cb * p.nsplit)), dim3(512), smem, st>>>(p);
    MPN_LAUNCH_CHECK();
    return MPN_OK;
}

template <typename T, int TAPS, int RBA, int RBD>
int launch_wgrad_g(const WgradParams& p, hipStream_t st) {
    constexpr int NPIXA = TAPS == 9 ? kHaloW * kHaloH : 128;
    constexpr int smem = NPIXA * RBA + 128 * RBD;
    static mpn_attr_mask_t attr_mask{0};
    MPN_HIP(mpn_ensure_dynamic_lds((const void*)conv_wgrad_kernel<T, TAPS, RBA, RBD>, smem, &attr_mask));
    conv_wgrad_kernel<T, TAPS, RBA, RBD><<<dim3((unsigned)(p.n_cg * p.n_cb * p.nsplit)), dim3(kThreads), smem, st>>>(p);
    MPN_LAUNCH_CHECK();
    return MPN_OK;
}

template <typename T, int TAPS>
int launch_wgrad(const WgradParams& p, hipStream_t st) {
    constexpr int ES = (int)sizeof(T);
    if (TAPS == 9 && p.Cout * ES <= 128) return launch_wgrad_g<T, TAPS, 128, 128>(p, st);
    return launch_wgrad_g<T, TAPS, (TAPS == 9 ? 64 : 256), 256>(p, st);
}

#ifdef MPN_DIAG
void* g_wgrad_dbg = nullptr;
#endif

}

#ifdef MPN_DIAG
extern "C" void mpn_diag_set_wgrad_stamps(void* buf) { g_wgrad_dbg = buf; }
#endif

extern "C" int mpn_conv_wgrad_num_parts(int N, int H, int W, int Cin, int Cout, int ksize, int dtype) {
    return wgrad_geom(N, H, W, Cin, Cout, ksize, dtype == MPN_F32 ? 4 : 2).nsplit;
}

namespace {
template <typename T, int TAPS, int RBA, int RBD, int WM, bool STAGGER>
int launch_wgrad_bf16_grouped(const WgradGroup& g, int blocks, hipStream_t st);
template <typename T>
int launch_wgrad_single_as_group(const WgradParams& p, hipStream_t st) {
    WgradGroup grp = {};
    grp.p[0] = p;
    const int blocks = p.n_cg * p.n_cb * p.nsplit;
    grp.begin[0] = 0;
    for (int j = 1; j <= kMaxWgradGroup; ++j) grp.begin[j] = blocks;
    grp.njobs = 1;
    return launch_wgrad_bf16_grouped<T, 9, 128, 256, 4, true>(grp, blocks, st);
}
}

extern "C" int mpn_conv_bwd_weight(const void* x, const void* dy, float* part, int N, int H, int W, int Cin, int Cout,
                                   int x_stride, int dy_stride, int ksize, int dtype, const float* in_scale,
                                   const float* in_shift, int in_act, mpn_stream_t stream) {
    MPN_REQUIRE(ksize == 1 || ksize == 3, MPN_ERR_BAD_SHAPE, "conv wgrad: ksize must be 1 or 3");
    MPN_REQUIRE(dtype == MPN_F32 || dtype == MPN_BF16 || dtype == MPN_F16, MPN_ERR_BAD_DTYPE, "conv wgrad: dtype %d", dtype);
    const int es = dtype == MPN_F32 ? 4 : 2;
    const int ve = 16 / es;
    MPN_REQUIRE(N > 0 && H > 0 && W > 0 && Cin > 0 && Cout > 0 && Cin % ve == 0 && Cout % ve == 0, MPN_ERR_BAD_SHAPE,
                "conv wgrad: bad shape (channels must be multiples of %d)", ve);
    MPN_REQUIRE(x && dy && part, MPN_ERR_BAD_ARG, "conv wgrad: null pointer");
    MPN_REQUIRE(mpn_aligned16(x) && mpn_aligned16(dy), MPN_ERR_BAD_ALIGN, "conv wgrad: pointers must be 16-byte aligned");
    MPN_REQUIRE((in_scale == nullptr) == (in_shift == nullptr), MPN_ERR_BAD_ARG, "conv wgrad: scale/shift mismatch");
    MPN_REQUIRE((long long)N * H * W * Cin < (1ll << 31) && (long long)N * H * W * Cout < (1ll << 31), MPN_ERR_BAD_SHAPE,
                "conv wgrad: tensors must have fewer than 2^31 elements");
    const WgradGeom g = wgrad_geom(N, H, W, Cin, Cout, ksize, es);
    WgradParams p;
    p.x = x; p.dy = dy; p.part = part;
    p.in_scale = in_scale; p.in_shift = in_shift; p.in_act = in_act;
    p.N = N; p.H = H; p.W = W; p.Cin = Cin; p.Cout = Cout;
    p.xs = x_stride > 0 ? x_stride : Cin; p.dys = dy_stride > 0 ? dy_stride : Cout;
    MPN_REQUIRE(p.xs >= Cin && p.dys >= Cout && p.xs % ve == 0 && p.dys % ve == 0, MPN_ERR_BAD_SHAPE,
                "conv wgrad: pixel strides (%d, %d) must be multiples of %d not below the channel counts", x_stride, dy_stride, ve);
    MPN_REQUIRE((long long)N * H * W * p.xs < (1ll << 31) && (long long)N * H * W * p.dys < (1ll << 31), MPN_ERR_BAD_SHAPE,
                "conv wgrad: strided tensors must span fewer than 2^31 elements");
    MPN_REQUIRE(ksize != 1 || es != 2 || ((long long)N * H * W * p.xs < (1ll << 30) && (long long)N * H * W * p.dys < (1ll << 30)),
                MPN_ERR_BAD_SHAPE, "conv wgrad: 16-bit 1x1 tensors must span fewer than 2^31 bytes");
    p.tiles_x = (W + 15) / 16; p.tiles_y = (H + 7) / 8;
    p.M = (long long)N * H * W;
    p.ntiles = g.ntiles; p.nsplit = g.nsplit; p.n_cg = g.n_cg; p.n_cb = g.n_cb; p.xcd_remap = 1;
#ifdef MPN_DIAG
    p.dbg = (unsigned long long*)g_wgrad_dbg;
#endif
// ... 129 lines not shown
template <typename T, int RBA, int RBD, int WM, bool DAPPLY = false>
int launch_conv1x1_bwd_fused(const WgradParams& p, hipStream_t st) {
    constexpr int CG = RBA / 2;
    constexpr int smem = 128 * (RBA + 32) + 128 * (RBD + 32) + 2 * CG * (int)sizeof(float) + 128 * (RBA + 32) + 128 * (RBA + 16) +
                         8 * 2 * CG * (int)sizeof(float) + (DAPPLY ? 4 * (RBD / 2) * (int)sizeof(float) : 0);
    static_assert(smem <= 160 * 1024, "LDS budget");
    static mpn_attr_mask_t attr_mask{0};
    MPN_HIP(mpn_ensure_dynamic_lds((const void*)conv1x1_bwd_fused_kernel<T, RBA, RBD, WM, DAPPLY>, smem, &attr_mask));
    conv1x1_bwd_fused_kernel<T, RBA, RBD, WM, DAPPLY><<<dim3((unsigned)p.nsplit), dim3(512), smem, st>>>(p);
    MPN_LAUNCH_CHECK();
    return MPN_OK;
}
}

extern "C" int mpn_conv1x1_bwd_fused_supported(int Cin, int Cout, int dtype) {
    return (dtype == MPN_BF16 && Cin > 0 && Cout > 0 && Cin % 8 == 0 && Cout % 8 == 0 && Cin <= 128 && Cout <= 128) ? 1 : 0;
}

namespace {
struct Conv1x1Apply { const void* y_raw; int y_stride; const float *scale, *shift, *mean, *invstd, *k1, *k2; int act; };
int conv1x1_bwd_fused_impl(const void* x, const void* dy, const float* w, void* dx, float* wpart, float* bn_part, int N, int H,
                           int W, int Cin, int Cout, int x_stride, int dy_stride, int dx_stride, int dtype,
                           const float* in_scale, const float* in_shift, int in_act, const Conv1x1Apply* ap, mpn_stream_t stream) {
    MPN_REQUIRE(mpn_conv1x1_bwd_fused_supported(Cin, Cout, dtype), MPN_ERR_BAD_SHAPE, "conv1x1_bwd_fused: layer not covered (Cin %d, Cout %d)", Cin, Cout);
    MPN_REQUIRE(x && dy && w && dx && wpart && in_scale && in_shift && N > 0 && H > 0 && W > 0, MPN_ERR_BAD_ARG, "conv1x1_bwd_fused: bad arguments");
    MPN_REQUIRE(bn_part != nullptr || ap == nullptr, MPN_ERR_BAD_ARG, "conv1x1_bwd_fused_apply: needs the reduction's slab");
    MPN_REQUIRE(mpn_aligned16(x) && mpn_aligned16(dy) && mpn_aligned16(dx), MPN_ERR_BAD_ALIGN, "conv1x1_bwd_fused: pointers must be 16-byte aligned");
    MPN_REQUIRE(dx != x && dx != dy, MPN_ERR_BAD_ARG, "conv1x1_bwd_fused: dx must not alias an input");
    WgradParams p = {};
    p.x = x; p.dy = dy; p.part = wpart; p.in_scale = in_scale; p.in_shift = in_shift; p.in_act = in_act;
    p.N = N; p.H = H; p.W = W; p.Cin = Cin; p.Cout = Cout;
    p.xs = x_stride > 0 ? x_stride : Cin; p.dys = dy_stride > 0 ? dy_stride : Cout; p.dxs = dx_stride > 0 ? dx_stride : Cin;
    MPN_REQUIRE(p.xs >= Cin && p.dys >= Cout && p.dxs >= Cin && p.xs % 8 == 0 && p.dys % 8 == 0 && p.dxs % 8 == 0, MPN_ERR_BAD_SHAPE,
                "conv1x1_bwd_fused: pixel strides must be multiples of 8 not below the channel counts");
    MPN_REQUIRE((long long)N * H * W * p.xs < (1ll << 31) && (long long)N * H * W * p.dys < (1ll << 31), MPN_ERR_BAD_SHAPE,
                "conv1x1_bwd_fused: tensors must span fewer than 2^31 elements");
    MPN_REQUIRE((long long)N * H * W * p.xs < (1ll << 30) && (long long)N * H * W * p.dys < (1ll << 30), MPN_ERR_BAD_SHAPE,
                "conv1x1_bwd_fused: tensors must span fewer than 2^31 bytes");
    const WgradGeom g = wgrad_geom(N, H, W, Cin, Cout, 1, 2);
    MPN_REQUIRE(g.n_cg == 1 && g.n_cb == 1, MPN_ERR_BAD_SHAPE, "conv1x1_bwd_fused: one block tile must hold the layer");
    p.tiles_x = (W + 15) / 16; p.tiles_y = (H + 7) / 8;
    p.M = (long long)N * H * W;
    p.ntiles = g.ntiles; p.nsplit = g.nsplit; p.n_cg = 1; p.n_cb = 1; p.xcd_remap = 1;
    p.wf = w; p.dx = dx; p.bn_part = bn_part;
#ifdef MPN_DIAG
    p.dbg = nullptr;
#endif
    hipStream_t st = (hipStream_t)stream;
    const bool thin32 = Cin <= 32 && Cout <= 64, wide = Cin > 64;
    if (ap != nullptr) {
        MPN_REQUIRE(!wide, MPN_ERR_BAD_SHAPE, "conv1x1_bwd_fused_apply: layer not covered (Cin %d, Cout %d)", Cin, Cout);
        MPN_REQUIRE(ap->y_raw && ap->scale && ap->shift && ap->mean && ap->invstd && ap->k1 && ap->k2 && mpn_aligned16(ap->y_raw), MPN_ERR_BAD_ARG,
                    "conv1x1_bwd_fused_apply: bad batch-norm arguments");
        p.ap_x = ap->y_raw; p.ap_xs = ap->y_stride > 0 ? ap->y_stride : Cout;
        MPN_REQUIRE(p.ap_xs >= Cout && p.ap_xs % 8 == 0 && (long long)N * H * W * p.ap_xs < (1ll << 31), MPN_ERR_BAD_SHAPE, "conv1x1_bwd_fused_apply: bad raw-output stride");
        p.ap_scale = ap->scale; p.ap_shift = ap->shift; p.ap_mean = ap->mean; p.ap_invstd = ap->invstd; p.ap_k1 = ap->k1; p.ap_k2 = ap->k2; p.ap_act = ap->act;
        return thin32 ? launch_conv1x1_bwd_fused<bf16_t, 64, 128, 2, true>(p, st) : launch_conv1x1_bwd_fused<bf16_t, 128, 256, 2, true>(p, st);
    }
    if (wide) return launch_conv1x1_bwd_fused<bf16_t, 256, 256, 4>(p, st);
    return thin32 ? launch_conv1x1_bwd_fused<bf16_t, 64, 128, 2>(p, st) : launch_conv1x1_bwd_fused<bf16_t, 128, 256, 2>(p, st);
}
}

extern "C" int mpn_conv1x1_bwd_fused(const void* x, const void* dy, const float* w, void* dx, float* wpart, float* bn_part, int N, int H,
                                     int W, int Cin, int Cout, int x_stride, int dy_stride, int dx_stride, int dtype,
                                     const float* in_scale, const float* in_shift, int in_act, mpn_stream_t stream) {
    return conv1x1_bwd_fused_impl(x, dy, w, dx, wpart, bn_part, N, H, W, Cin, Cout, x_stride, dy_stride, dx_stride, dtype, in_scale, in_shift,
                                  in_act, nullptr, stream);
}

extern "C" int mpn_conv1x1_bwd_fused_apply_supported(int Cin, int Cout, int dtype) {
    return (mpn_conv1x1_bwd_fused_supported(Cin, Cout, dtype) && Cin <= 64) ? 1 : 0;
}

extern "C" int mpn_conv1x1_bwd_fused_apply(const void* x, const void* g, const void* y_raw, const float* w, void* dx, float* wpart,
                                           float* bn_part, int N, int H, int W, int Cin, int Cout, int x_stride, int g_stride, int y_stride,
                                           int dx_stride, int dtype, const float* in_scale, const float* in_shift, int in_act,
                                           const float* ap_scale, const float* ap_shift, const float* ap_mean, const float* ap_invstd,
                                           const float* ap_k1, const float* ap_k2, int ap_act, mpn_stream_t stream) {
    const Conv1x1Apply ap = {y_raw, y_stride, ap_scale, ap_shift, ap_mean, ap_invstd, ap_k1, ap_k2, ap_act};
    return conv1x1_bwd_fused_impl(x, g, w, dx, wpart, bn_part, N, H, W, Cin, Cout, x_stride, g_stride, dx_stride, dtype, in_scale, in_shift,
                                  in_act, &ap, stream);
}
```

multiposenet_amd/csrc/stem.hip:

```cpp
#include "common.h"

namespace {

constexpr int kThreads = 256;
constexpr int kTile = 16;
constexpr int kIn = 2 * kTile + 1;
constexpr int kMaxC0 = 64;
constexpr int kFwdTW = 2 * kTile;

template <typename T, bool U8>
__device__ __forceinline__ void stage_patch(const void* images, float* patch, int img, int oy0, int ox0, int H, int W,
                                            int pad_t, int pad_l) {
    const int iy0 = oy0 * 2 - pad_t, ix0 = ox0 * 2 - pad_l;
    constexpr int NEL = kIn * kIn * 3;
    constexpr int PER = (NEL + kThreads - 1) / kThreads;
    float v[PER];
#pragma unroll
    for (int k = 0; k < PER; ++k) {
        const int i = threadIdx.x + k * kThreads;
        const int ch = i % 3;
        const int px = (i / 3) % kIn;
        const int py = i / (3 * kIn);
        const int iy = iy0 + py, ix = ix0 + px;
        float raw = 0.5f;
// ... 289 lines not shown
            pmask |= (ok ? 1u : 0u) << k;
        }
#pragma unroll
        for (int k = 0; k < DPER; ++k) {
            if (k < ndv) {
                const int i = threadIdx.x + k * kThreads;
                const int vq = i % vpp, px = i / vpp;
                const int oy = oy0 + px / kTile, ox = ox0 + px % kTile;
                const bool ok = oy < OH && ox < OW;
                dvv[k].load(dy + (ok ? (((long long)img * OH + oy) * OW + ox) * C0 + vq * VE : 0));
                dmask |= (ok ? 1u : 0u) << k;
            }
        }
    };
    auto commit_tile = [&]() {
#pragma unroll
        for (int k = 0; k < PER; ++k) {
            const int i = threadIdx.x + k * kThreads;
            if (i < NEL) patch[i] = ((pmask >> k) & 1u) ? 2.0f * pv[k] - 1.0f : 0.0f;
        }
#pragma unroll
        for (int k = 0; k < DPER; ++k) {
            if (k < ndv) {
                const int i = threadIdx.x + k * kThreads;
                const int vq = i % vpp, px = i / vpp;
                float f[VE];
                dvv[k].unpack(f);
                const bool ok = (dmask >> k) & 1u;
#pragma unroll
                for (int j = 0; j < VE; j += 4)
                    *reinterpret_cast<float4*>(g + px * C0 + vq * VE + j) =
                        ok ? make_float4(f[j], f[j + 1], f[j + 2], f[j + 3]) : make_float4(0.f, 0.f, 0.f, 0.f);
            }
        }
    };

    int t = blockIdx.x;
    if (t < ntiles) {
        load_tile(t);
        commit_tile();
    }
    for (; t < ntiles; t += gridDim.x) {
        const bool more = t + (int)gridDim.x < ntiles;
        if (more) load_tile(t + gridDim.x);
        __syncthreads();
        if (active) {
            for (int px = ph; px < kTile * kTile; px += nphase) {
                const int ly = px / kTile, lx = px - ly * kTile;
                const float* pp = patch + ((2 * ly + ky) * kIn + 2 * lx + kx) * 3;
                const float a0 = pp[0], a1 = pp[1], a2 = pp[2];
                const float4 g0 = *reinterpret_cast<const float4*>(g + px * C0 + cq * 8);
                const float4 g1 = *reinterpret_cast<const float4*>(g + px * C0 + cq * 8 + 4);
                const f32x2_t gv[4] = {(f32x2_t){g0.x, g0.y}, (f32x2_t){g0.z, g0.w}, (f32x2_t){g1.x, g1.y}, (f32x2_t){g1.z, g1.w}};
                const f32x2_t b0 = (f32x2_t){a0, a0}, b1 = (f32x2_t){a1, a1}, b2 = (f32x2_t){a2, a2};
#pragma unroll
                for (int j = 0; j < 4; ++j) {
                    acc[0][j] += b0 * gv[j];
                    acc[1][j] += b1 * gv[j];
                    acc[2][j] += b2 * gv[j];
                }
            }
        }
        __syncthreads();
        if (more) commit_tile();
    }
    __syncthreads();
    if (active) {
#pragma unroll
        for (int a = 0; a < 3; ++a)
#pragma unroll
            for (int j = 0; j < 4; ++j) {
                g[ph * nout + (pos * 3 + a) * C0 + cq * 8 + 2 * j] = acc[a][j].x;
                g[ph * nout + (pos * 3 + a) * C0 + cq * 8 + 2 * j + 1] = acc[a][j].y;
            }
    }
    __syncthreads();
    for (int o = threadIdx.x; o < nout; o += kThreads) {
        float s = 0.f;
        for (int q = 0; q < nphase; ++q) s += g[q * nout + o];
        part[(long long)blockIdx.x * nout + o] = s;
    }
}

template <bool U8, int MB>
__global__ __launch_bounds__(kThreads) void stem_wgrad_mfma_kernel(const void* __restrict__ images, const bf16_t* __restrict__ dy,
                                                                   float* __restrict__ part, int N, int H, int W, int OH, int OW,
                                                                   int pad_t, int pad_l, int tiles_x, int tiles_y) {
    typedef H16<bf16_t> HT;
    typedef HT::x8 x8;
    typedef HT::x4 x4;
    typedef HT::acc_t acc_t;
    constexpr int C0 = 16 * MB;
    constexpr int DRS = C0 * 2 + 16;
    extern __shared__ __attribute__((aligned(16))) unsigned char stem_smem[];
    float* patch = reinterpret_cast<float*>(stem_smem);
    unsigned char* dimg = stem_smem + kPR * kPS * sizeof(float);
    const int ntiles = N * tiles_y * tiles_x;
    const int lane = threadIdx.x & 63, wv = threadIdx.x >> 6;
    const int n = lane & 15, kg = lane >> 4, q = n >> 2, pq = n & 3;
    constexpr int VPP = C0 / 8;
    constexpr int DV = kTile * kFwdTW * VPP / kThreads;
    float pv[kPR];
    uint4 dv[DV];
    unsigned long long pmask = 0ull;
    unsigned dmask = 0u;
    const int p_pc = threadIdx.x < kPC ? threadIdx.x : 0;
    auto load_tile = [&](int t) __attribute__((always_inline)) {
        const int tx = t % tiles_x;
        const int t2 = t / tiles_x;
        const int ty = t2 % tiles_y;
        const int img = t2 / tiles_y;
        const int iy0 = ty * kTile * 2 - pad_t, ix0 = tx * kFwdTW * 2 - pad_l;
        pmask = 0ull;
        dmask = 0u;
        int tid = threadIdx.x;
        asm volatile("" : "+v"(tid));
        {
            const int ix = ix0 + p_pc / 3;
            const bool col_ok = tid < kPC && ix >= 0 && ix < W;
            const long long base = ((long long)img * H * W + ix0) * 3 + p_pc;
#pragma unroll
            for (int py = 0; py < kPR; ++py) {
                const int iy = iy0 + py;
                const bool ok = col_ok && iy >= 0 && iy < H;
                const long long off = ok ? base + (long long)iy * W * 3 : 0;
                pv[py] = U8 ? (float)reinterpret_cast<const unsigned char*>(images)[off] * (1.0f / 255.0f)
                            : reinterpret_cast<const float*>(images)[off];
                pmask |= (unsigned long long)(ok ? 1u : 0u) << py;
            }
        }
#pragma unroll
        for (int k = 0; k < DV; ++k) {
            const int i = tid + k * kThreads;
            const int vq = i % VPP, px = i / VPP;
            const int oy = ty * kTile + px / kFwdTW, ox = tx * kFwdTW + px % kFwdTW;
            const bool ok = oy < OH && ox < OW;
            dv[k] = *reinterpret_cast<const uint4*>(dy + (ok ? (((long long)img * OH + oy) * OW + ox) * C0 + vq * 8 : 0));
            dmask |= (ok ? 1u : 0u) << k;
        }
    };
    auto commit_tile = [&]() __attribute__((always_inline)) {
        int tid = threadIdx.x;
        asm volatile("" : "+v"(tid));
        if (tid < kPC) {
#pragma unroll
            for (int py = 0; py < kPR; ++py)
                patch[py * kPS + p_pc] = ((pmask >> py) & 1ull) ? 2.0f * pv[py] - 1.0f : 0.0f;
        }
#pragma unroll
        for (int k = 0; k < DV; ++k) {
            const int i = tid + k * kThreads;
            const int vq = i % VPP, px = i / VPP;
            *reinterpret_cast<uint4*>(dimg + px * DRS + vq * 16) = ((dmask >> k) & 1u) ? dv[k] : make_uint4(0u, 0u, 0u, 0u);
        }
    };
    int kbase[2];
    bool kval[2];
#pragma unroll
    for (int nb = 0; nb < 2; ++nb) {
        const int k = nb * 16 + n;
        kval[nb] = k < 27;
        kbase[nb] = kval[nb] ? (k / 9) * kPS + (k % 9) : 0;
    }
    acc_t acc[MB][2];
#pragma unroll
    for (int mb = 0; mb < MB; ++mb)
#pragma unroll
        for (int nb = 0; nb < 2; ++nb) acc[mb][nb] = (acc_t){0.f, 0.f, 0.f, 0.f};

    int t = blockIdx.x;
    if (t < ntiles) {
        load_tile(t);
        commit_tile();
    }
    for (; t < ntiles; t += gridDim.x) {
        const bool more = t + (int)gridDim.x < ntiles;
        if (more) load_tile(t + gridDim.x);
        __syncthreads();
#pragma unroll 1
        for (int sr = 0; sr < 4; ++sr) {
            const int r = wv * 4 + sr;
            x8 a[MB];
#pragma unroll
            for (int mb = 0; mb < MB; ++mb) {
                const unsigned char* src = dimg + (r * kFwdTW + 8 * kg + q) * DRS + (mb * 16 + 4 * pq) * 2;
                const x4 lo4 = HT::tr_read(src);
                const x4 hi4 = HT::tr_read(src + 4 * DRS);
                a[mb] = __builtin_shufflevector(lo4, hi4, 0, 1, 2, 3, 4, 5, 6, 7);
            }
#pragma unroll
            for (int nb = 0; nb < 2; ++nb) {
                const float* src = patch + (2 * r) * kPS + 6 * (8 * kg) + kbase[nb];
                x8 b_hi, b_lo;
#pragma unroll
                for (int i = 0; i < 8; ++i) {
                    const float raw = src[6 * i];
                    const float f = kval[nb] ? raw : 0.0f;
                    const bf16_t h = (bf16_t)f;
                    b_hi[i] = h;
                    b_lo[i] = (bf16_t)(f - (float)h);
                }
#pragma unroll
                for (int mb = 0; mb < MB; ++mb) {
                    acc[mb][nb] = HT::mfma(a[mb], b_lo, acc[mb][nb]);
                    acc[mb][nb] = HT::mfma(a[mb], b_hi, acc[mb][nb]);
                }
            }
        }
        __syncthreads();
        if (more) commit_tile();
    }
    __syncthreads();
    float* red = reinterpret_cast<float*>(stem_smem);
#pragma unroll
    for (int mb = 0; mb < MB; ++mb)
#pragma unroll
        for (int nb = 0; nb < 2; ++nb)
            *reinterpret_cast<float4*>(red + ((wv * (MB * 2) + mb * 2 + nb) * 64 + lane) * 4) =
                make_float4(acc[mb][nb][0], acc[mb][nb][1], acc[mb][nb][2], acc[mb][nb][3]);
    __syncthreads();
    for (int o = threadIdx.x; o < 27 * C0; o += kThreads) {
        const int k = o / C0, co = o - k * C0;
        const int nb = k >> 4, nn = k & 15, mb = co >> 4, m = co & 15;
        const int ln = (m >> 2) * 16 + nn, e = m & 3;
        float sacc = 0.f;
#pragma unroll
        for (int w4 = 0; w4 < 4; ++w4) sacc += red[((w4 * (MB * 2) + mb * 2 + nb) * 64 + ln) * 4 + e];
        part[(long long)blockIdx.x * (27 * C0) + o] = sacc;
    }
}

template <bool U8, int MB>
int launch_stem_wgrad_mfma(int grid, hipStream_t st, const void* images, const void* dy, float* part, int N, int H, int W, int OH,
                           int OW, int pt, int pl, int tiles_x, int tiles_y) {
    constexpr int sm = kPR * kPS * (int)sizeof(float) + kTile * kFwdTW * (16 * MB * 2 + 16);
    static mpn_attr_mask_t attr_mask{0};
    MPN_HIP(mpn_ensure_dynamic_lds((const void*)stem_wgrad_mfma_kernel<U8, MB>, sm, &attr_mask));
    stem_wgrad_mfma_kernel<U8, MB><<<grid, kThreads, sm, st>>>(images, (const bf16_t*)dy, part, N, H, W, OH, OW, pt, pl, tiles_x, tiles_y);
    return MPN_OK;
}

void same_pad(int size, int* out, int* pad_before) {
    *out = (size + 1) / 2;
    int total = (*out - 1) * 2 + 3 - size;
    if (total < 0) total = 0;
    *pad_before = total / 2;
}

int check(int N, int H, int W, int C0, int dtype) {
    MPN_REQUIRE(dtype == MPN_F32 || dtype == MPN_BF16, MPN_ERR_BAD_DTYPE, "stem: dtype %d", dtype);
    const int ve = dtype == MPN_F32 ? 4 : 8;
    MPN_REQUIRE(N > 0 && H > 0 && W > 0, MPN_ERR_BAD_SHAPE, "stem: bad shape");
    MPN_REQUIRE(C0 > 0 && C0 <= kMaxC0 && C0 % ve == 0, MPN_ERR_BAD_SHAPE, "stem: C0 (%d) must be <= %d and a multiple of %d",
                C0, kMaxC0, ve);
    return MPN_OK;
}

}

extern "C" int mpn_stem_conv_fwd_num_parts(int N, int H, int W, int C0, int dtype) {
    if (check(N, H, W, C0, dtype)) return 0;
    const int ppr = C0 * (dtype == MPN_F32 ? 4 : 2) / 16;
    if (ppr <= 0 || kThreads % ppr != 0 || 2 * C0 > kThreads) return 0;
    int OH, OW, pt, pl;
    same_pad(H, &OH, &pt);
    same_pad(W, &OW, &pl);
    return N * ((OH + kTile - 1) / kTile) * ((OW + kFwdTW - 1) / kFwdTW);
}

extern "C" int mpn_stem_conv_fwd(const void* images, int images_u8, const float* w, void* y, int N, int H, int W, int C0,
                                 int dtype, mpn_stream_t stream) {
    return mpn_stem_conv_fwd_stats(images, images_u8, w, y, N, H, W, C0, dtype, nullptr, stream);
}

extern "C" int mpn_stem_conv_fwd_stats(const void* images, int images_u8, const float* w, void* y, int N, int H, int W, int C0,
                                       int dtype, float* stats_part, mpn_stream_t stream) {
    if (int rc = check(N, H, W, C0, dtype)) return rc;
    MPN_REQUIRE(images && w && y, MPN_ERR_BAD_ARG, "stem_fwd: null pointer");
    MPN_REQUIRE(stats_part == nullptr || mpn_stem_conv_fwd_num_parts(N, H, W, C0, dtype) > 0, MPN_ERR_BAD_SHAPE,
                "stem_fwd: fused statistics not available for C0 = %d (mpn_stem_conv_fwd_num_parts == 0)", C0);
    int OH, OW, pt, pl;
    same_pad(H, &OH, &pt);
    same_pad(W, &OW, &pl);
    const int tiles_y = (OH + kTile - 1) / kTile, tiles_x = (OW + kFwdTW - 1) / kFwdTW;
    const int grid = N * tiles_y * tiles_x;
    hipStream_t st = (hipStream_t)stream;
    if (dtype == MPN_BF16 && C0 % 16 == 0) {
        const int otile_bytes = 2 * kThreads * (C0 * 2 + 16), patch_bytes = kPR * kPS * (int)sizeof(float);
        const int sm = otile_bytes > patch_bytes ? otile_bytes : patch_bytes;
#define MPN_STEM_MFMA(MB)                                                                                                       \
    do {                                                                                                                        \
        if (images_u8) stem_fwd_mfma_kernel<true, MB><<<grid, kThreads, sm, st>>>(images, w, (bf16_t*)y, N, H, W, OH, OW, pt, pl, tiles_x, tiles_y, stats_part); \
        else stem_fwd_mfma_kernel<false, MB><<<grid, kThreads, sm, st>>>(images, w, (bf16_t*)y, N, H, W, OH, OW, pt, pl, tiles_x, tiles_y, stats_part); \
    } while (0)
        if (sm <= 64 * 1024) {
            switch (C0 / 16) {
                case 1: MPN_STEM_MFMA(1); break;
                case 2: MPN_STEM_MFMA(2); break;
                case 3: MPN_STEM_MFMA(3); break;
                default: MPN_STEM_MFMA(4); break;
            }
#undef MPN_STEM_MFMA
            MPN_LAUNCH_CHECK();
            return MPN_OK;
        }
    }
    MPN_DISPATCH_DTYPE(dtype, {
        const int sm = 2 * kThreads * (C0 * (int)sizeof(T) + 16);
        if (images_u8) {
            if (sm > 48 * 1024)
                MPN_HIP(hipFuncSetAttribute((const void*)stem_fwd_kernel<T, true>, hipFuncAttributeMaxDynamicSharedMemorySize, sm));
            stem_fwd_kernel<T, true><<<grid, kThreads, sm, st>>>(images, w, (T*)y, N, H, W, C0, OH, OW, pt, pl, tiles_x, tiles_y, stats_part);
        } else {
            if (sm > 48 * 1024)
                MPN_HIP(hipFuncSetAttribute((const void*)stem_fwd_kernel<T, false>, hipFuncAttributeMaxDynamicSharedMemorySize, sm));
            stem_fwd_kernel<T, false><<<grid, kThreads, sm, st>>>(images, w, (T*)y, N, H, W, C0, OH, OW, pt, pl, tiles_x, tiles_y, stats_part);
        }
    });
    MPN_LAUNCH_CHECK();
    return MPN_OK;
}

extern "C" int mpn_stem_conv_wgrad_num_parts(int N, int H, int W) {
    const int ntiles = N * (((H + 1) / 2 + kTile - 1) / kTile) * (((W + 1) / 2 + kTile - 1) / kTile);
    return ntiles < 512 ? ntiles : 512;
}

extern "C" int mpn_stem_conv_bwd_weight(const void* images, int images_u8, const void* dy, float* part, int N, int H, int W,
                                        int C0, int dtype, mpn_stream_t stream) {
    if (int rc = check(N, H, W, C0, dtype)) return rc;
    MPN_REQUIRE(images && dy && part, MPN_ERR_BAD_ARG, "stem_wgrad: null pointer");
    int OH, OW, pt, pl;
    same_pad(H, &OH, &pt);
    same_pad(W, &OW, &pl);
    const int tiles_y = (OH + kTile - 1) / kTile, tiles_x = (OW + kTile - 1) / kTile;
    const int grid = mpn_stem_conv_wgrad_num_parts(N, H, W);
    hipStream_t st = (hipStream_t)stream;
    MPN_REQUIRE(C0 % 8 == 0, MPN_ERR_BAD_SHAPE, "stem_wgrad: C0 must be a multiple of 8");
    if (dtype == MPN_BF16 && C0 % 16 == 0) {
        const int tx32 = (OW + kFwdTW - 1) / kFwdTW;
        int rc;
#define MPN_STEM_WG(MB)                                                                                                         \
    rc = images_u8 ? launch_stem_wgrad_mfma<true, MB>(grid, st, images, dy, part, N, H, W, OH, OW, pt, pl, tx32, tiles_y)       \
                   : launch_stem_wgrad_mfma<false, MB>(grid, st, images, dy, part, N, H, W, OH, OW, pt, pl, tx32, tiles_y)
        switch (C0 / 16) {
            case 1: MPN_STEM_WG(1); break;
            case 2: MPN_STEM_WG(2); break;
            case 3: MPN_STEM_WG(3); break;
            default: MPN_STEM_WG(4); break;
        }
#undef MPN_STEM_WG
        if (rc) return rc;
        MPN_LAUNCH_CHECK();
        return MPN_OK;
    }
    const size_t sm = (size_t)(kIn * kIn * 3 + 1 + kTile * kTile * C0) * sizeof(float);
    MPN_REQUIRE(sm <= 64 * 1024, MPN_ERR_BAD_SHAPE, "stem_wgrad: C0 too large");
    MPN_DISPATCH_DTYPE(dtype, {
        if (images_u8)
            stem_wgrad_kernel<T, true><<<grid, kThreads, sm, st>>>(images, (const T*)dy, part, N, H, W, C0, OH, OW, pt, pl, tiles_x, tiles_y);
        else
            stem_wgrad_kernel<T, false><<<grid, kThreads, sm, st>>>(images, (const T*)dy, part, N, H, W, C0, OH, OW, pt, pl, tiles_x, tiles_y);
    });
    MPN_LAUNCH_CHECK();
    return MPN_OK;
}
```

multiposenet_amd/net.py:

```python
import math
import os
from collections import OrderedDict

import numpy as np
import torch

from . import _lib, ops
from ._lib import ACT_NONE, ACT_RELU, ACT_RELU6
from .model_state import ModelState, _Arena, is_trainable, resolve_device

NUM_KEYPOINTS = 17
DOWNSAMPLE = 4
DIVISOR = 128
DEPTH = 128
STRIDES_AND_FILTERS = [(1, 64), (2, 128), (1, 128), (2, 256), (1, 256), (2, 512), (1, 512), (1, 512),
                       (1, 512), (1, 512), (1, 512), (2, 1024), (1, 1024)]
FEATURE_BLOCKS = {3: "c2", 5: "c3", 11: "c4", 13: "c5"}


def depth(x, depth_multiplier):
    return max(int(x * depth_multiplier), 8)


def variable_shapes(depth_multiplier=1.0):
    s = OrderedDict()

    def bn(prefix, c):
        for n in ("gamma", "beta", "moving_mean", "moving_variance"):
            s[f"{prefix}/{n}"] = (c,)

    c = depth(32, depth_multiplier)
    s["MobilenetV1/Conv2d_0/weights"] = (3, 3, 3, c)
    bn("MobilenetV1/Conv2d_0/BatchNorm", c)
    for i, (_, f) in enumerate(STRIDES_AND_FILTERS, 1):
        s[f"MobilenetV1/Conv2d_{i}_depthwise/depthwise_weights"] = (3, 3, c, 1)
        bn(f"MobilenetV1/Conv2d_{i}_depthwise/BatchNorm", c)
        f = depth(f, depth_multiplier)
        s[f"MobilenetV1/Conv2d_{i}_pointwise/weights"] = (1, 1, c, f)
        bn(f"MobilenetV1/Conv2d_{i}_pointwise/BatchNorm", f)
        c = f
    feat = {2: depth(128, depth_multiplier), 3: depth(256, depth_multiplier),
            4: depth(512, depth_multiplier), 5: depth(1024, depth_multiplier)}
    s["keypoint_fpn/lateral5/kernel"] = (1, 1, feat[5], DEPTH)
    s["keypoint_fpn/p5/kernel"] = (3, 3, DEPTH, DEPTH)
    for i in (4, 3, 2):
        s[f"keypoint_fpn/lateral{i}/kernel"] = (1, 1, feat[i], DEPTH)
        s[f"keypoint_fpn/p{i}/kernel"] = (3, 3, DEPTH, DEPTH)
    for l in (2, 3, 4, 5):
        bn(f"p{l}_batch_norm", DEPTH)
    for l in (2, 3, 4, 5):
        s[f"phi_subnet_{l}/conv1/kernel"] = (3, 3, DEPTH, DEPTH)
        bn(f"phi_subnet_{l}/bn1", DEPTH)
        s[f"phi_subnet_{l}/conv2/kernel"] = (3, 3, DEPTH, DEPTH)
        bn(f"phi_subnet_{l}/bn2", DEPTH)
    s["final_conv3x3/kernel"] = (3, 3, 4 * DEPTH, 64)
    bn("final_bn", 64)
    s["heatmaps/kernel"] = (1, 1, 64, NUM_KEYPOINTS + 1)
    s["heatmaps/bias"] = (NUM_KEYPOINTS + 1,)
    return s


def internal_shapes(depth_multiplier=1.0):
    ref = variable_shapes(depth_multiplier)
    c0 = depth(32, depth_multiplier)
    c0p = (c0 + 15) // 16 * 16
    if c0p == c0:
        return ref, {}
    shapes, pads = OrderedDict(), {}
    for name, shape in ref.items():
        axis = None
        if name.startswith("MobilenetV1/Conv2d_0/") or name.startswith("MobilenetV1/Conv2d_1_depthwise/BatchNorm/"):
            axis = len(shape) - 1
        elif name in ("MobilenetV1/Conv2d_1_depthwise/depthwise_weights", "MobilenetV1/Conv2d_1_pointwise/weights"):
            axis = 2
        if axis is not None:
            assert shape[axis] == c0
            pads[name] = (axis, c0)
            shape = tuple(c0p if i == axis else d for i, d in enumerate(shape))
        shapes[name] = shape
    return shapes, pads


def initial_values(seed=0, depth_multiplier=1.0):
    rs = np.random.RandomState(seed)
    out = OrderedDict()
    for name, shape in variable_shapes(depth_multiplier).items():
        if name.endswith("/gamma") or name.endswith("moving_variance"):
            v = np.ones(shape)
        elif name.endswith("/beta") or name.endswith("moving_mean"):
            v = np.zeros(shape)
        elif name == "heatmaps/bias":
            v = np.array([-math.log(99.0)] * NUM_KEYPOINTS + [0.0])
        elif name == "heatmaps/kernel":
            v = rs.randn(*shape) * 1e-4
        else:
            fan_in = shape[0] * shape[1] * (shape[2] if not name.endswith("depthwise_weights") else 1)
            v = rs.randn(*shape) * math.sqrt(1.0 / fan_in) * 1.2
        out[name] = v.astype(np.float32)
    return out


DP_DEEP_FROM_BLOCK = 7


def backbone_deep_begin_of(arena, first_block=DP_DEEP_FROM_BLOCK):
    return arena.offsets[f"MobilenetV1/Conv2d_{first_block}_depthwise/depthwise_weights"][0]


def backbone_grad_end_of(arena):
    end = 0
    for k, (o, n, _) in arena.offsets.items():
        if k.startswith("MobilenetV1/"):
            end = max(end, o + (n + 3) // 4 * 4)
    return end


@ops._lib.device_guarded("_init", "load_state_dict", "repack_weights", "prepare_inference", "forward", "predict",
                         "backbone_forward", "subnet_forward", "compute_losses", "backward", "add_weight_decay_gradients",
                         "add_weight_decay_loss", "optimizer_step")
class KeypointNet(ModelState):
    def __init__(self, values=None, depth_multiplier=1.0, dtype=torch.bfloat16, device="cuda:0", seed=0):
        if dtype not in (torch.float32, torch.bfloat16):
            raise ValueError("dtype must be torch.float32 or torch.bfloat16")
        self.dtype, self.device, self.dm = dtype, resolve_device(device), depth_multiplier
        self._init(values, depth_multiplier, dtype, seed)

    def _init(self, values, depth_multiplier, dtype, seed):
        shapes, pads = internal_shapes(depth_multiplier)
        for n, s in shapes.items():
            if n.endswith("gamma") and (s[0] % 16 != 0):
                raise ValueError(f"depth_multiplier={depth_multiplier}: {n} has {s[0]} channels; every layer behind the stem "
                                 f"must be a multiple of 16 channels wide (depth multipliers that are multiples of 0.25)")
        self._init_state(shapes, pads=pads)
        self.load_state_dict(values if values is not None else initial_values(seed, depth_multiplier))
        self._build_layers()
        self._bufs = {}

    def _build_layers(self):
        self.stem_w = self.vars["MobilenetV1/Conv2d_0/weights"]
        self.stem_dw = self.grads["MobilenetV1/Conv2d_0/weights"]
        self.stem_bn = self._bn("MobilenetV1/Conv2d_0/BatchNorm", ACT_RELU6)
        self.blocks = []
        for i, (stride, _) in enumerate(STRIDES_AND_FILTERS, 1):
            d, p = f"MobilenetV1/Conv2d_{i}_depthwise", f"MobilenetV1/Conv2d_{i}_pointwise"
            self.blocks.append(dict(
                i=i, stride=stride,
                dw_w=self.vars[d + "/depthwise_weights"], dw_dw=self.grads[d + "/depthwise_weights"],
                dw_bn=self._bn(d + "/BatchNorm", ACT_RELU6),
                pw=self._conv(p + "/weights"), pw_bn=self._bn(p + "/BatchNorm", ACT_RELU6)))
        self.lateral = {l: self._conv(f"keypoint_fpn/lateral{l}/kernel") for l in (5, 4, 3, 2)}
        self.pconv = {l: self._conv(f"keypoint_fpn/p{l}/kernel") for l in (5, 4, 3, 2)}
        self.p_bn = {l: self._bn(f"p{l}_batch_norm", ACT_RELU) for l in (2, 3, 4, 5)}
        self.phi = {}
        for l in (2, 3, 4, 5):
            s = f"phi_subnet_{l}"
            self.phi[l] = dict(conv1=self._conv(s + "/conv1/kernel"), bn1=self._bn(s + "/bn1", ACT_RELU),
                               conv2=self._conv(s + "/conv2/kernel"), bn2=self._bn(s + "/bn2", ACT_RELU))
        self.final_conv = self._conv("final_conv3x3/kernel")
        self.final_bn = self._bn("final_bn", ACT_RELU)
        self.concat_scale = torch.ones(4 * DEPTH, dtype=torch.float32, device=self.device)
        self.concat_shift = torch.zeros(4 * DEPTH, dtype=torch.float32, device=self.device)
        self.phi[2]["bn2"].scale = self.concat_scale[:DEPTH]
        self.phi[2]["bn2"].shift = self.concat_shift[:DEPTH]
        self.concat_affine = ops.Affine(self.concat_scale, self.concat_shift, ACT_RELU)
        self.heat_w, self.heat_b = self.vars["heatmaps/kernel"], self.vars["heatmaps/bias"]
        ok, nk, _ = self._train_arena.offsets["heatmaps/kernel"]
        ob, nb, _ = self._train_arena.offsets["heatmaps/bias"]
        assert ob == ok + nk, "heatmaps/kernel and heatmaps/bias must be adjacent in the arena"
        self._head_grad = self.grad[ok:ob + nb]
        self.fuse_dw_bn = True
        self.fuse_conv_bn = True
        self._l2 = None
        self._wd = None
        self.cache_inference_affine = False
        self._infer_clean = False
        self.fuse_stem_stats = True
        self._build_pack_table()
        self.all_bn = [self.stem_bn] + [b[k] for b in self.blocks for k in ("dw_bn", "pw_bn")] + \
            [self.p_bn[l] for l in (2, 3, 4, 5)] + [self.phi[l][k] for l in (2, 3, 4, 5) for k in ("bn1", "bn2")] + [self.final_bn]

    def _build_pack_table(self):
        import ctypes
        lib = ops._lib.lib()
        nb = lib.mpn_conv_pack_desc_bytes()
        jobs = [(c, t) for c in self.convs for t in (0, 1)]
        host = (ctypes.c_ubyte * (nb * len(jobs)))()
        begin = 0
        dc = ops._lib.dtype_code(self.dtype)
        for j, (c, t) in enumerate(jobs):
            out = c.packed.bwd if t else c.packed.fwd
            blocks = lib.mpn_conv_pack_desc_fill(ctypes.byref(host, j * nb), ops.ptr(c.w), c.cin, c.cout, c.ksize, t, dc,
                                                 ops.ptr(out), begin)
            assert blocks > 0
            begin += blocks
        self._pack_table = torch.frombuffer(bytearray(host), dtype=torch.uint8).to(self.device)
        self._pack_jobs, self._pack_blocks = len(jobs), begin

    def repack_weights(self):
        if ops.LAUNCH_JOBS_ALONE:
            for c in self.convs:
                c.packed.repack()
            return
        ops.call("mpn_conv_pack_weights_batched", ops.ptr(self._pack_table), self._pack_jobs, self._pack_blocks,
                 ops._lib.dtype_code(self.dtype), ops.stream_ptr())

    def _buffers(self, N, H, W, head=True):
        key = (N, H, W) if head else (N, H, W, "backbone")
        b = self._bufs.get(key)
        if b is not None:
            return b
        if H % DIVISOR or W % DIVISOR:
            raise ValueError(f"image height and width must be multiples of {DIVISOR} (got {H}x{W})")
        dt, dev = self.dtype, self.device

        def act(h, w, c):
            return torch.empty((N, h, w, c), dtype=dt, device=dev)

        b = {"shape": (N, H, W)}
        h, w = H // 2, W // 2
        c = self.stem_w.shape[3]
        b["stem"] = act(h, w, c)
        b["dw"], b["pw"], b["hw"] = [], [], [(h, w)]
        for blk in self.blocks:
            if blk["stride"] == 2:
                h, w = h // 2, w // 2
            b["dw"].append(act(h, w, c))
            c = blk["pw"].cout
            b["pw"].append(act(h, w, c))
            b["hw"].append((h, w))
        if not head:
            nbn0 = ops._lib.lib().mpn_bn_stats_num_parts
            b["stat_part"] = torch.empty(nbn0(N * (H // 2) * (W // 2)) * 2 * b["stem"].shape[3], dtype=torch.float32, device=dev)
            self._bufs[key] = b
            return b
        lv = {l: (H >> l, W >> l) for l in (2, 3, 4, 5)}
        b["lv"] = lv
        b["x"] = {l: act(*lv[l], DEPTH) for l in lv}
        b["p"] = {l: act(*lv[l], DEPTH) for l in lv}
        b["y1"] = {l: act(*lv[l], DEPTH) for l in lv}
        b["concat"] = act(*lv[2], 4 * DEPTH)
        b["y2"] = {l: act(*lv[l], DEPTH) for l in lv if l != 2}
        b["y2"][2] = b["concat"][..., :DEPTH]
        b["final"] = act(*lv[2], 64)
        b["logits"] = torch.empty((N, lv[2][0], lv[2][1], NUM_KEYPOINTS + 1), dtype=torch.float32, device=dev)
        nbn = ops._lib.lib().mpn_bn_stats_num_parts

        def rows(t):
            return t.numel() // t.shape[3]

        stat_floats = nbn(rows(b["stem"])) * 2 * b["stem"].shape[3]
        for i, blk in enumerate(self.blocks):
            hh, ww = b["hw"][i]
            cdw, cpw = b["dw"][i].shape[3], blk["pw"].cout
            stat_floats = max(stat_floats, ops.dwconv_num_parts(N, hh, ww, cdw, blk["stride"], dt) * 2 * cdw,
                              nbn(rows(b["dw"][i])) * 2 * cdw,
                              ops.conv_num_parts(N, *b["hw"][i + 1], 1) * 2 * cpw, nbn(rows(b["pw"][i])) * 2 * cpw,
                              ops.dwconv_bwd_data_bn_num_parts(N, hh, ww, cdw, blk["stride"], dt) * 2 * cdw,
                              ops.dwconv_wgrad_num_parts(N, hh, ww, cdw, blk["stride"], dt) * 2 * cdw,
                              ops.conv_wgrad_num_parts(N, *b["hw"][i + 1], cdw, cpw, 1, dt) * 2 * cdw)
        for l in lv:
            stat_floats = max(stat_floats, ops.conv_num_parts(N, *lv[l], 3) * 2 * DEPTH, nbn(N * lv[l][0] * lv[l][1]) * 2 * DEPTH)
        b["stat_part"] = torch.empty(stat_floats, dtype=torch.float32, device=dev)
        b["stat_lv"] = {l: torch.empty(max(ops.conv_num_parts(N, *lv[l], 3), nbn(N * lv[l][0] * lv[l][1])) * 2 * DEPTH,
                                       dtype=torch.float32, device=dev) for l in lv}
        b["fin"] = None
        b["loss_part"] = torch.empty(ops._lib.lib().mpn_keypoint_loss_num_parts(N, *lv[2]) * 8, dtype=torch.float32, device=dev)
        b["losses"] = torch.zeros(8, dtype=torch.float32, device=dev)
        self._bufs[key] = b
        return b

    def _grad_buffers(self, b):
        if "g" in b:
            return b["g"]
        N, H, W = b["shape"]
        dt, dev = self.dtype, self.device
        g = {}
        g["dlogits"] = torch.empty_like(b["logits"])
        g["daux"] = {l: torch.empty((N, *b["lv"][l]), dtype=torch.float32, device=dev) for l in b["lv"]}
        g["final"] = torch.empty_like(b["final"])
        g["concat"] = torch.empty_like(b["concat"])
        for k in ("y1", "p", "x"):
            g[k] = {l: torch.empty_like(b[k][l]) for l in b["lv"]}
        g["y2"] = {l: torch.empty_like(b["y2"][l]) for l in b["lv"] if l != 2}
        g["y2"][2] = g["concat"][..., :DEPTH]
        g["c"] = {}
        for i, name in FEATURE_BLOCKS.items():
            g["c"][name] = torch.empty_like(b["pw"][i - 1])
        g["pw"] = [torch.empty_like(t) for t in b["pw"]]
        g["dw"] = [torch.empty_like(t) for t in b["dw"]]
        g["stem"] = torch.empty_like(b["stem"])
        lib, dc = ops._lib.lib(), ops._lib.dtype_code(dt)
        sites = []
        grouped_np = {}
        for group in self._wgrad_groups():
            hws = [self._conv_hw(b, c) for c in group]
            for c, np_ in zip(group, ops.conv_wgrad_grouped_num_parts(N, hws, group[0].cin, group[0].cout, group[0].ksize, dt)):
                grouped_np[id(c.dw)] = np_
        for c in self.convs:
            hw = self._conv_hw(b, c)
            np_ = grouped_np.get(id(c.dw))
            if np_ is None:
                np_ = ops.conv_wgrad_num_parts(N, hw[0], hw[1], c.cin, c.cout, c.ksize, dt)
            sites.append((id(c.dw), np_, c.w.numel(), c.dw))
        for i, blk in enumerate(self.blocks):
            hh, ww = b["hw"][i]
            cc = b["dw"][i].shape[3]
            sites.append((id(blk["dw_dw"]), lib.mpn_dwconv_wgrad_num_parts(N, hh, ww, cc, blk["stride"], dc), 9 * cc, blk["dw_dw"]))
        sites.append((id(self.stem_dw), lib.mpn_stem_conv_wgrad_num_parts(N, H, W), self.stem_w.numel(), self.stem_dw))
        sites.append((id(self._head_grad), lib.mpn_heatmap_head_bwd_num_parts(N * b["lv"][2][0] * b["lv"][2][1]),
                      self._head_grad.numel(), self._head_grad))
        total = sum(((np_ * n + 3) // 4) * 4 for _, np_, n, _ in sites)
        slab = torch.empty(total, dtype=torch.float32, device=dev)
        deep_keys = {id(blk[k]) if k == "dw_dw" else id(blk[k].dw) for blk in self.blocks if blk["i"] >= DP_DEEP_FROM_BLOCK
                     for k in ("pw", "dw_dw")}
        shallow_keys = {id(blk[k]) if k == "dw_dw" else id(blk[k].dw) for blk in self.blocks if blk["i"] < DP_DEEP_FROM_BLOCK
                        for k in ("pw", "dw_dw")} | {id(self.stem_dw)}
        g["slab"], jobs, off = {}, ([], [], []), 0
        for key, np_, n, out in sites:
            view = slab[off:off + np_ * n]
            g["slab"][key] = view
            jobs[1 if key in deep_keys else (2 if key in shallow_keys else 0)].append((view, np_, n, out.view(-1)))
            off += ((np_ * n + 3) // 4) * 4
        g["reducer"] = tuple(ops.SlabReducer(j, dev) for j in jobs)
        b["g"] = g
        return g

    def _wgrad_groups(self):
        LV = (2, 3, 4, 5)
        return [[self.phi[l]["conv2"] for l in LV], [self.phi[l]["conv1"] for l in LV], [self.pconv[l] for l in LV]]

    def _conv_hw(self, b, c):
        n = c.name
        if n.startswith("MobilenetV1"):
            i = int(n.split("Conv2d_")[1].split("_")[0])
            return b["hw"][i]
        if n.startswith("keypoint_fpn") or n.startswith("phi_subnet"):
            l = int(n.split("/")[0][-1]) if n.startswith("phi") else int(n.split("/")[1].replace("lateral", "").replace("p", ""))
            return b["lv"][l]
        return b["lv"][2]

    def _finish_bn(self, bn, b, nparts, count, training):
        if training:
            ops.bn_finalize(bn, b["stat_part"], nparts, count, training=True)

    def prepare_inference(self):
        if self.cache_inference_affine and self._infer_clean:
            return
        for bn in self.all_bn:
            ops.bn_inference_affine(bn)
        self._infer_clean = True

    def backbone_forward(self, images, is_training, b=None):
        N, H, W, _ = images.shape
        b = b or self._buffers(N, H, W)
        if not is_training:
            self.prepare_inference()
        else:
            self.mark_variables_changed()
        sp = b["stat_part"]
        c0 = self.stem_w.shape[3]
        stem_rows = ops.stem_conv_fwd_num_parts(N, H, W, c0, self.dtype) if (is_training and self.fuse_stem_stats) else 0
        if stem_rows * 2 * c0 > sp.numel():
            stem_rows = 0
        stem = ops.stem_conv_fwd(images, self.stem_w, c0, self.dtype, out=b["stem"], stats_part=sp if stem_rows > 0 else None)
        if is_training:
            cnt = stem.numel() // stem.shape[3]
            if stem_rows > 0:
                ops.bn_finalize(self.stem_bn, sp, stem_rows, cnt)
            else:
                _, nparts = ops.bn_stats(stem, sp)
                ops.bn_finalize(self.stem_bn, sp, nparts, cnt)
        x, aff = stem, self.stem_bn.affine
        feats = {}
# ... 112 lines not shown
        if part in (None, 0):
            self._backward_head(b, g, feats, sp, slab)
            g["reducer"][0].run()
        for ph in (1, 2):
            if part in (None, ph):
                self._backward_backbone(b, g, images, sp, slab, ph)
                g["reducer"][ph].run()

    def _backward_head(self, b, g, feats, sp, slab):
        if self._fused_conv_bn() and ops.heatmap_head_bwd_bn_supported(b["final"].shape[3], self.dtype):
            rows = ops.heatmap_head_bwd(b["final"], g["dlogits"], self.heat_w, self.final_bn.affine, g["final"], self._head_grad,
                                        slab[id(self._head_grad)], reduce=False, bn_part=sp)
            ops.bn_backward(self.final_bn, g["final"], b["final"], sp, reduced_parts=rows, raw=True)
        else:
            ops.heatmap_head_bwd(b["final"], g["dlogits"], self.heat_w, self.final_bn.affine, g["final"], self._head_grad,
                                 slab[id(self._head_grad)], reduce=False)
            ops.bn_backward(self.final_bn, g["final"], b["final"], sp)
        ops.conv_bwd_weight(b["concat"], g["final"], 3, self.concat_affine, self.final_conv.dw, slab[id(self.final_conv.dw)], reduce=False)
        ops.conv_fwd(g["final"], self.final_conv.packed.bwd, 4 * DEPTH, 3, None, out=g["concat"])
        if b["fin"] is None:
            b["fin"] = self._finalize_tables(b)
        fin, spl = b["fin"], b["stat_lv"]
        LV = (2, 3, 4, 5)
        sps = [spl[l] for l in LV]
        bn2s, bn1s, pbns = [self.phi[l]["bn2"] for l in LV], [self.phi[l]["bn1"] for l in LV], [self.p_bn[l] for l in LV]
        gy2, gy1, gp = [g["y2"][l] for l in LV], [g["y1"][l] for l in LV], [g["p"][l] for l in LV]
        by2, by1, bp = [b["y2"][l] for l in LV], [b["y1"][l] for l in LV], [b["p"][l] for l in LV]
        for l in (3, 4, 5):
            ops.bilinear_up_bwd(g["concat"], 2 ** (l - 2), (l - 2) * DEPTH, DEPTH, out=g["y2"][l])
        ops.bn_bwd_reduce_grouped(bn2s, gy2, by2, sps)
        fin["dbn2"].run()
        none4 = [None] * 4
        fused = self._fused_conv_bn()
        ops.bn_bwd_apply_grouped(bn2s, gy2, by2)
        ops.conv_bwd_weight_grouped(by1, gy2, 3, [self.phi[l]["bn1"].affine for l in LV], [slab[id(self.phi[l]["conv2"].dw)] for l in LV])
        if fused:
            ops.conv_bwd_data_bn_grouped(gy2, [self.phi[l]["conv2"].packed.bwd for l in LV], DEPTH, bn1s, by1, gy1, sps)
        else:
            ops.conv_fwd_grouped([g["y2"][l] for l in LV], [self.phi[l]["conv2"].packed.bwd for l in LV], DEPTH, 3, none4,
                                 [g["y1"][l] for l in LV], none4)
            ops.bn_bwd_reduce_grouped(bn1s, gy1, by1, sps)
        fin["dbn1"].run()
        ops.bn_bwd_apply_grouped(bn1s, gy1, by1)
        ops.conv_bwd_weight_grouped(bp, gy1, 3, [self.p_bn[l].affine for l in LV], [slab[id(self.phi[l]["conv1"].dw)] for l in LV])
        if fused:
            ops.conv_bwd_data_bn_grouped(gy1, [self.phi[l]["conv1"].packed.bwd for l in LV], DEPTH, pbns, bp, gp, sps)
        else:
            ops.conv_fwd_grouped([g["y1"][l] for l in LV], [self.phi[l]["conv1"].packed.bwd for l in LV], DEPTH, 3, none4,
                                 [g["p"][l] for l in LV], none4)
            ops.bn_bwd_reduce_grouped(pbns, gp, bp, sps)
        fin["dp"].run()
        ops.bn_bwd_apply_grouped(pbns, gp, bp, [g["daux"][l] for l in LV])
        ops.conv_bwd_weight_grouped([b["x"][l] for l in LV], gp, 3, none4, [slab[id(self.pconv[l].dw)] for l in LV])
        ops.conv_fwd_grouped(gp, [self.pconv[l].packed.bwd for l in LV], DEPTH, 3, none4, [g["x"][l] for l in LV], none4)
        g["c5_reduced"] = 0
        for l in (2, 3, 4, 5):
            if l > 2:
                ops.sumpool2x2(g["x"][l - 1], g["x"][l], accumulate=True)
            raw, aff = feats[f"c{l}"]
            ops.conv_bwd_weight(raw, g["x"][l], 1, aff, self.lateral[l].dw, slab[id(self.lateral[l].dw)], reduce=False)
            if l == 5 and self.fuse_conv_bn and ops.conv_bwd_data_bn_supported(DEPTH, raw.shape[3], 1, self.dtype):
                g["c5_reduced"] = ops.conv_bwd_data_bn(g["x"][l], self.lateral[l].packed.bwd, raw.shape[3], 1, self.blocks[-1]["pw_bn"], raw,
                                                       g["c"][f"c{l}"], sp)
            else:
                ops.conv_fwd(g["x"][l], self.lateral[l].packed.bwd, raw.shape[3], 1, None, out=g["c"][f"c{l}"])

    def _backward_backbone(self, b, g, images, sp, slab, phase):
        first, last = DP_DEEP_FROM_BLOCK - 1, len(self.blocks) - 1
        if phase == 1:
            dA, reduced, lateral_added = g["c"]["c5"], g.get("c5_reduced", 0), False
            rng = range(last, first - 1, -1)
        else:
            dA, reduced, lateral_added = g["bb_chain"]
            rng = range(first - 1, -1, -1)
        for i in rng:
            feature = FEATURE_BLOCKS.get(self.blocks[i]["i"])
            if feature in ("c2", "c3", "c4") and not lateral_added:
                ops.add_inplace(dA, g["c"][feature])
            dY = self._backward_pointwise(b, g, sp, slab, i, dA, reduced, raw=i == last)
            dA, reduced, lateral_added = self._backward_depthwise(b, g, sp, slab, i, dY)
        if phase == 1:
            g["bb_chain"] = (dA, reduced, lateral_added)
            return
        ops.bn_backward(self.stem_bn, g["stem"], b["stem"], sp, reduced_parts=reduced)
        ops.stem_conv_bwd_weight(images, g["stem"], self.stem_dw, slab[id(self.stem_dw)], reduce=False)

    def _backward_pointwise(self, b, g, sp, slab, i, dA, reduced, raw):
        blk = self.blocks[i]
        pw, x, dY = blk["pw"], b["dw"][i], g["dw"][i]
        fused = self.fuse_conv_bn and ops.conv1x1_bwd_fused_supported(pw.cin, pw.cout, self.dtype) and pw.cin <= 64
        apply = fused and ops.conv1x1_bwd_fused_apply_supported(pw.cin, pw.cout, self.dtype)
        ops.bn_backward(blk["pw_bn"], dA, b["pw"][i], sp, reduced_parts=reduced, raw=raw, apply=not apply)
        rows = 0
        with _lib.tagged("pointwise"):
            if fused:
                rows = ops.conv1x1_bwd_fused(x, dA, pw.w, blk["dw_bn"], dY, slab[id(pw.dw)], sp,
                                             apply_bn=blk["pw_bn"] if apply else None, y_raw=b["pw"][i] if apply else None)
            else:
                ops.conv_bwd_weight(x, dA, 1, blk["dw_bn"].affine, pw.dw, slab[id(pw.dw)], reduce=False)
                if self.fuse_conv_bn and ops.conv_bwd_data_bn_supported(pw.cout, pw.cin, 1, self.dtype):
                    rows = ops.conv_bwd_data_bn(dA, pw.packed.bwd, pw.cin, 1, blk["dw_bn"], x, dY, sp)
                else:
                    ops.conv_fwd(dA, pw.packed.bwd, pw.cin, 1, None, out=dY)
        ops.bn_backward(blk["dw_bn"], dY, x, sp, reduced_parts=rows, raw=True)
        return dY

    def _backward_depthwise(self, b, g, sp, slab, i, dY):
        blk = self.blocks[i]
        x, bn, dA = (b["pw"][i - 1], self.blocks[i - 1]["pw_bn"], g["pw"][i - 1]) if i > 0 else (b["stem"], self.stem_bn, g["stem"])
        N, hw, C, s = dA.shape[0], b["hw"][i], dA.shape[3], blk["stride"]
        lateral = g["c"][FEATURE_BLOCKS[self.blocks[i - 1]["i"]]] if i > 0 and self.blocks[i - 1]["i"] in FEATURE_BLOCKS else None
        if self.fuse_dw_bn and (s == 2 or lateral is None) and ops.dwconv_bwd_fused_supported(N, *hw, C, s, self.dtype):
            _, reduced = ops.dwconv_bwd_fused(x, dY, blk["dw_w"], bn, None, out=dA, wpart=slab[id(blk["dw_dw"])], bn_part=sp,
                                              reduce=False, stride=s, addend=lateral)
            return dA, reduced, lateral is not None
        ops.dwconv_bwd_weight(x, dY, s, bn.affine, blk["dw_dw"], slab[id(blk["dw_dw"])], reduce=False)
        late = lateral is not None and not ops.dwconv_bwd_data_add_supported(N, *hw, C, s, self.dtype)
        addend = None if late else lateral
        if self.fuse_dw_bn and not late and ops.dwconv_bwd_data_bn_num_parts(N, *hw, C, s, self.dtype) > 0:
            _, reduced = ops.dwconv_bwd_data(dY, blk["dw_w"], hw, s, out=dA, bn=bn, x_bn=x, part=sp, addend=addend)
            return dA, reduced, addend is not None
        ops.dwconv_bwd_data(dY, blk["dw_w"], hw, s, out=dA, addend=addend)
        return dA, 0, addend is not None

    def add_weight_decay_gradients(self, weight_decay):
        if self._wd is None:
            ks = [k for k in self.vars if ("weights" in k or "kernel" in k) and "depthwise_weights" not in k]
            self._wd = ops.AxpyBatch([self.vars[k] for k in ks], [self.grads[k] for k in ks])
        self._wd.run(weight_decay)

    def add_weight_decay_loss(self, weight_decay):
        total = self._last[0]["losses"][6:7]
        if self._l2 is None:
            self._l2 = ops.L2LossBatch([w for k, w in self.vars.items()
                                        if ("weights" in k or "kernel" in k) and "depthwise_weights" not in k])
        self._l2.run(weight_decay, total)

    def optimizer_step(self, initial_learning_rate, num_steps, grad_scale=1.0):
        ops.adam_prepare(self.global_step, self.hyper, initial_learning_rate, num_steps)
        ops.adam_step(self.theta, self.grad, self.adam_m, self.adam_v, self.hyper, grad_scale=grad_scale)
        self.mark_variables_changed()
        self.repack_weights()
```

multiposenet_amd/ops.py:

```python
import ctypes
from collections import namedtuple

import torch

from . import _lib
from ._lib import ACT_NONE, ACT_RELU, ACT_RELU6, call, ptr, stream_ptr

BN_MOMENTUM = 0.95
BN_EPSILON = 1e-3

LAUNCH_JOBS_ALONE = False

Affine = namedtuple("Affine", ["scale", "shift", "act"])


def _f32(n, dev):
    return torch.empty(n, dtype=torch.float32, device=dev)


def _check_nhwc(x, name="x"):
    if x.dim() != 4 or not x.is_contiguous():
        raise ValueError(f"{name} must be a contiguous NHWC tensor, got shape {tuple(x.shape)}")
    if x.dtype not in (torch.float32, torch.bfloat16):
        raise ValueError(f"{name}: unsupported dtype {x.dtype}")
# ... 63 lines not shown
        raise ValueError(f"x must be an NHWC f32/bf16/f16 tensor, got {tuple(x.shape)} {x.dtype}")
    N, H, W, cin = x.shape
    xs = _slice_stride(x, cin)
    if out is None:
        out = torch.empty((N, H, W, cout), dtype=x.dtype, device=x.device)
    ys = _slice_stride(out, cout)
    sc, sh, act = _aff(affine)
    call("mpn_conv_fwd", ptr(x), ptr(packed), ptr(out), N, H, W, cin, cout, xs, ys, ksize, _lib.dtype_code(x.dtype),
         sc, sh, act, ptr(stats_part), ptr(up_res), stream_ptr())
    return out


def conv_fwd_grouped(xs, packeds, cout, ksize, affines, outs, stats_parts):
    import ctypes
    n = len(xs)
    if LAUNCH_JOBS_ALONE and n > 1:
        for j in range(n):
            conv_fwd_grouped([xs[j]], [packeds[j]], cout, ksize, [affines[j]], [outs[j]], [stats_parts[j]])
        return outs
    N, _, _, cin = xs[0].shape
    PA, IA = ctypes.c_void_p * n, ctypes.c_int * n
    sc, sh, act = [], [], ACT_NONE
    for a in affines:
        s_, h_, a_ = _aff(a)
        sc.append(s_); sh.append(h_)
        if a is not None:
            act = a_
    call("mpn_conv_fwd_grouped", n, PA(*[ptr(x) for x in xs]), PA(*[ptr(p) for p in packeds]), PA(*[ptr(o) for o in outs]), N,
         IA(*[x.shape[1] for x in xs]), IA(*[x.shape[2] for x in xs]), cin, cout, IA(*[_slice_stride(x, cin) for x in xs]),
         IA(*[_slice_stride(o, cout) for o in outs]), ksize, _lib.dtype_code(xs[0].dtype), PA(*sc), PA(*sh), int(act), PA(*[ptr(t) for t in stats_parts]), stream_ptr())
    return outs


def conv_bwd_data_bn_supported(k, c, ksize, dtype):
    return bool(_lib.lib().mpn_conv_bwd_data_bn_supported(int(k), int(c), int(ksize), _lib.dtype_code(dtype)))


def conv_bwd_data_bn(dy, packed_t, c, ksize, bn, x_bn, out, part):
    N, H, W, k = dy.shape
    call("mpn_conv_bwd_data_bn", ptr(dy), ptr(packed_t), ptr(out), N, H, W, k, int(c), _slice_stride(dy, k), _slice_stride(out, c), int(ksize),
         _lib.dtype_code(dy.dtype), ptr(x_bn), _slice_stride(x_bn, c), ptr(bn.scale), ptr(bn.shift), int(bn.act), ptr(part), stream_ptr())
    return conv_stats_rows(N, H, W, k, c, ksize, dy.dtype)


def conv_bwd_data_bn_grouped(dys, packeds_t, c, bns, xs_bn, outs, parts):
    import ctypes
    n = len(dys)
    if LAUNCH_JOBS_ALONE and n > 1:
        return [conv_bwd_data_bn_grouped([dys[j]], [packeds_t[j]], c, [bns[j]], [xs_bn[j]], [outs[j]], [parts[j]])[0] for j in range(n)]
    N, _, _, k = dys[0].shape
    PA, IA = ctypes.c_void_p * n, ctypes.c_int * n
    call("mpn_conv_bwd_data_bn_grouped", n, PA(*[ptr(t) for t in dys]), PA(*[ptr(p) for p in packeds_t]), PA(*[ptr(o) for o in outs]), N,
         IA(*[t.shape[1] for t in dys]), IA(*[t.shape[2] for t in dys]), k, int(c), IA(*[_slice_stride(t, k) for t in dys]),
         IA(*[_slice_stride(o, c) for o in outs]), _lib.dtype_code(dys[0].dtype), PA(*[ptr(x) for x in xs_bn]),
         IA(*[_slice_stride(x, c) for x in xs_bn]), PA(*[ptr(b.scale) for b in bns]), PA(*[ptr(b.shift) for b in bns]), int(bns[0].act),
         PA(*[ptr(t) for t in parts]), stream_ptr())
    return [conv_stats_rows(N, t.shape[1], t.shape[2], k, c, 3, t.dtype) for t in dys]


def conv1x1_bwd_fused_supported(cin, cout, dtype):
    return _lib.lib().mpn_conv1x1_bwd_fused_supported(int(cin), int(cout), _lib.dtype_code(dtype)) == 1


def conv1x1_bwd_fused_apply_supported(cin, cout, dtype):
    return _lib.lib().mpn_conv1x1_bwd_fused_apply_supported(int(cin), int(cout), _lib.dtype_code(dtype)) == 1


def conv1x1_bwd_fused(x, dy, w, bn, out, wpart, bn_part, apply_bn=None, y_raw=None):
    N, H, W, cin = x.shape
    cout = dy.shape[3]
    rows = conv_wgrad_num_parts(N, H, W, cin, cout, 1, x.dtype)
    if wpart.numel() < rows * cin * cout or (bn_part is not None and bn_part.numel() < rows * 2 * cin):
        raise ValueError("conv1x1_bwd_fused: partial slab too small")
    if apply_bn is not None:
        a = apply_bn
        call("mpn_conv1x1_bwd_fused_apply", ptr(x), ptr(dy), ptr(y_raw), ptr(w), ptr(out), ptr(wpart), ptr(bn_part), N, H, W, cin, cout,
             _slice_stride(x, cin), _slice_stride(dy, cout), _slice_stride(y_raw, cout), _slice_stride(out, cin), _lib.dtype_code(x.dtype),
             ptr(bn.scale), ptr(bn.shift), int(bn.act), ptr(a.scale), ptr(a.shift), ptr(a.mean), ptr(a.invstd), ptr(a.k1), ptr(a.k2),
             int(a.act), stream_ptr())
        return rows
    call("mpn_conv1x1_bwd_fused", ptr(x), ptr(dy), ptr(w), ptr(out), ptr(wpart), ptr(bn_part), N, H, W, cin, cout, _slice_stride(x, cin),
         _slice_stride(dy, cout), _slice_stride(out, cin), _lib.dtype_code(x.dtype), ptr(bn.scale), ptr(bn.shift), int(bn.act), stream_ptr())
    return rows


def conv_wgrad_num_parts(N, H, W, cin, cout, ksize, dtype):
    return _lib.lib().mpn_conv_wgrad_num_parts(N, H, W, cin, cout, ksize, _lib.dtype_code(dtype))


def conv_bwd_weight(x, dy, ksize, affine, dw_out, part=None, reduce=True):
    N, H, W, cin = x.shape
    cout = dy.shape[3]
    nparts = conv_wgrad_num_parts(N, H, W, cin, cout, ksize, x.dtype)
    n = ksize * ksize * cin * cout
    if part is None:
        part = _f32(nparts * n, x.device)
    sc, sh, act = _aff(affine)
    call("mpn_conv_bwd_weight", ptr(x), ptr(dy), ptr(part), N, H, W, cin, cout, _slice_stride(x, cin), _slice_stride(dy, cout),
         ksize, _lib.dtype_code(x.dtype), sc, sh, act, stream_ptr())
    if reduce:
        call("mpn_reduce_partials", ptr(part), nparts, n, ptr(dw_out), 0, 1.0, stream_ptr())
    return dw_out


class SlabReducer:

    def __init__(self, jobs, device):
        import ctypes
        self._alone = [SlabReducer([j], device) for j in jobs] if LAUNCH_JOBS_ALONE and len(jobs) > 1 else None
        lib = _lib.lib()
        nb = lib.mpn_reduce_desc_bytes()
        host = (ctypes.c_ubyte * (nb * len(jobs)))()
        begin = 0
        for j, (part, nparts, n, out) in enumerate(jobs):
            blocks = lib.mpn_reduce_desc_fill(ctypes.byref(host, j * nb), ptr(part), int(nparts), int(n), ptr(out), 1.0, begin)
            if blocks <= 0:
                raise ValueError("bad slab reduction job")
            begin += blocks
        self.table = torch.frombuffer(bytearray(host), dtype=torch.uint8).to(device)
        self.njobs, self.blocks = len(jobs), begin
        self._keep = jobs

    def run(self):
        if self._alone is not None:
            for r in self._alone:
                r.run()
            return
        call("mpn_reduce_partials_batched", ptr(self.table), self.njobs, self.blocks, stream_ptr())


def conv_wgrad_grouped_num_parts(N, hws, cin, cout, ksize, dtype):
    import ctypes
    n = len(hws)
    if LAUNCH_JOBS_ALONE and n > 1:
        return [conv_wgrad_grouped_num_parts(N, [hw], cin, cout, ksize, dtype)[0] for hw in hws]
    IA = ctypes.c_int * n
    out = IA()
    call("mpn_conv_wgrad_grouped_num_parts", n, N, IA(*[h for h, _ in hws]), IA(*[w for _, w in hws]), cin, cout, ksize,
         _lib.dtype_code(dtype), out)
    return list(out)


def conv_bwd_weight_grouped(xs, dys, ksize, affines, parts):
    import ctypes
    n = len(xs)
    if LAUNCH_JOBS_ALONE and n > 1:
        for j in range(n):
            conv_bwd_weight_grouped([xs[j]], [dys[j]], ksize, [affines[j]], [parts[j]])
        return
    PA, IA = ctypes.c_void_p * n, ctypes.c_int * n
    N, cin, cout = xs[0].shape[0], xs[0].shape[3], dys[0].shape[3]
    sc, sh, act = zip(*[_aff(a) for a in affines])
    if len(set(act)) != 1:
        raise ValueError("grouped jobs must share the activation")
    call("mpn_conv_bwd_weight_grouped", n, PA(*[ptr(t) for t in xs]), PA(*[ptr(t) for t in dys]), PA(*[ptr(t) for t in parts]), N,
         IA(*[t.shape[1] for t in xs]), IA(*[t.shape[2] for t in xs]), cin, cout, IA(*[_slice_stride(t, cin) for t in xs]),
         IA(*[_slice_stride(t, cout) for t in dys]), ksize, _lib.dtype_code(xs[0].dtype), PA(*sc), PA(*sh), int(act[0]), stream_ptr())


class BNState:

    def __init__(self, gamma, beta, moving_mean, moving_var, act):
        C = gamma.numel()
        dev = gamma.device
        self.C, self.act = C, act
        self.gamma, self.beta, self.moving_mean, self.moving_var = gamma, beta, moving_mean, moving_var
# ... 242 lines not shown


def dwconv_bwd_weight(x, dy, stride, affine, dw_out, part=None, reduce=True):
    N, H, W, C = x.shape
    dc = _lib.dtype_code(x.dtype)
    nparts = _lib.lib().mpn_dwconv_wgrad_num_parts(N, H, W, C, stride, dc)
    if part is None:
        part = _f32(nparts * 9 * C, x.device)
    sc, sh, act = _aff(affine)
    call("mpn_dwconv_bwd_weight", ptr(x), ptr(dy), ptr(part), N, H, W, C, stride, dc, sc, sh, act, stream_ptr())
    if reduce:
        call("mpn_reduce_partials", ptr(part), nparts, 9 * C, ptr(dw_out), 0, 1.0, stream_ptr())
    return dw_out


def dwconv_bwd_fused_supported(N, H, W, C, stride, dtype):
    return _lib.lib().mpn_dwconv_bwd_fused_supported(N, H, W, C, stride, _lib.dtype_code(dtype)) == 1


def dwconv_bwd_fused(x, dy, w, bn, dw_out, out=None, wpart=None, bn_part=None, reduce=True, reduce_bn=True, stride=1, addend=None):
    N, H, W, C = x.shape
    dc = _lib.dtype_code(x.dtype)
    if not dwconv_bwd_fused_supported(N, H, W, C, stride, x.dtype):
        raise ValueError("dwconv_bwd_fused: shape not supported")
    if addend is not None and (stride != 2 or addend.shape != x.shape or addend.dtype != x.dtype or not addend.is_contiguous()):
        raise ValueError("dwconv_bwd_fused: addend needs stride 2 and the result's shape and dtype")
    if out is None:
        out = torch.empty_like(x)
    rows = _lib.lib().mpn_dwconv_wgrad_num_parts(N, H, W, C, stride, dc)
    if wpart is None:
        wpart = _f32(rows * 9 * C, x.device)
    if reduce_bn and bn_part is None:
        bn_part = _f32(rows * 2 * C, x.device)
    if wpart.numel() < rows * 9 * C or (reduce_bn and bn_part.numel() < rows * 2 * C):
        raise ValueError("dwconv_bwd_fused: partial slab too small")
    if stride == 2:
        call("mpn_dwconv_bwd_fused_s2", ptr(x), ptr(dy), ptr(w), ptr(out), ptr(wpart), N, H, W, C, dc, ptr(bn.scale), ptr(bn.shift),
             int(bn.act), ptr(bn.mean), ptr(bn.invstd), ptr(bn_part) if reduce_bn else None, ptr(addend), stream_ptr())
    else:
        call("mpn_dwconv_bwd_fused", ptr(x), ptr(dy), ptr(w), ptr(out), ptr(wpart), N, H, W, C, dc, ptr(bn.scale), ptr(bn.shift),
             int(bn.act), ptr(bn.mean), ptr(bn.invstd), ptr(bn_part) if reduce_bn else None, stream_ptr())
    if reduce:
        call("mpn_reduce_partials", ptr(wpart), rows, 9 * C, ptr(dw_out), 0, 1.0, stream_ptr())
    return out, (rows if reduce_bn else 0)


def stem_conv_fwd_num_parts(N, H, W, c0, dtype):
    return _lib.lib().mpn_stem_conv_fwd_num_parts(N, H, W, c0, _lib.dtype_code(dtype))


def stem_conv_fwd(images, w, c0, dtype, out=None, stats_part=None):
    if images.dim() != 4 or images.shape[3] != 3 or not images.is_contiguous():
        raise ValueError("images must be contiguous [N,H,W,3]")
    u8 = images.dtype == torch.uint8
    if not u8 and images.dtype != torch.float32:
        raise ValueError("images must be float32 in [0,1] or uint8")
    N, H, W, _ = images.shape
    if out is None:
        out = torch.empty((N, (H + 1) // 2, (W + 1) // 2, c0), dtype=dtype, device=images.device)
    if stats_part is not None:
        rows = stem_conv_fwd_num_parts(N, H, W, c0, dtype)
        if rows <= 0 or stats_part.numel() < rows * 2 * c0:
            raise ValueError("stem_conv_fwd: fused statistics not available for this shape, or slab too small")
        call("mpn_stem_conv_fwd_stats", ptr(images), int(u8), ptr(w), ptr(out), N, H, W, c0, _lib.dtype_code(dtype),
             ptr(stats_part), stream_ptr())
        return out
    call("mpn_stem_conv_fwd", ptr(images), int(u8), ptr(w), ptr(out), N, H, W, c0, _lib.dtype_code(dtype), stream_ptr())
    return out


def stem_conv_bwd_weight(images, dy, dw_out, part=None, reduce=True):
    N, H, W, _ = images.shape
    c0 = dy.shape[3]
    nparts = _lib.lib().mpn_stem_conv_wgrad_num_parts(N, H, W)
    if part is None:
        part = _f32(nparts * 27 * c0, dy.device)
    call("mpn_stem_conv_bwd_weight", ptr(images), int(images.dtype == torch.uint8), ptr(dy), ptr(part), N, H, W, c0,
         _lib.dtype_code(dy.dtype), stream_ptr())
    if reduce:
        call("mpn_reduce_partials", ptr(part), nparts, 27 * c0, ptr(dw_out), 0, 1.0, stream_ptr())
    return dw_out


def bilinear_up_fwd(x, upsample, out, channel_offset, affine=None):
    N, h, w, C = x.shape
    sc, sh, act = _aff(affine)
    call("mpn_bilinear_up_fwd", ptr(x), ptr(out), N, h, w, C, upsample, channel_offset, out.shape[3],
         _lib.dtype_code(x.dtype), sc, sh, act, stream_ptr())
    return out


def bilinear_up_bwd(dy, upsample, channel_offset, C, out=None):
    N, OH, OW, ctot = dy.shape
    h, w = OH // upsample, OW // upsample
    if out is None:
        out = torch.empty((N, h, w, C), dtype=dy.dtype, device=dy.device)
    call("mpn_bilinear_up_bwd", ptr(dy), ptr(out), N, h, w, C, upsample, channel_offset, ctot, _lib.dtype_code(dy.dtype),
         stream_ptr())
    return out


def sumpool2x2(src, dst=None, accumulate=False):
    N, H2, W2, C = src.shape
    if dst is None:
        dst = torch.empty((N, H2 // 2, W2 // 2, C), dtype=src.dtype, device=src.device)
    call("mpn_sumpool2x2", ptr(src), ptr(dst), N, H2 // 2, W2 // 2, C, int(accumulate), _lib.dtype_code(src.dtype), stream_ptr())
    return dst


def add_inplace(dst, src):
    if dst.shape != src.shape or dst.dtype != src.dtype:
        raise ValueError("add_inplace: shape/dtype mismatch")
    call("mpn_add_inplace", ptr(dst), ptr(src), dst.numel(), _lib.dtype_code(dst.dtype), stream_ptr())
    return dst


def heatmap_head_fwd(x, w, bias, affine, inference=False, out=None, out_seg=None):
    N, H, W, cin = x.shape
    M = N * H * W
    sc, sh, act = _aff(affine)
    if inference:
        if out is None:
            out = torch.empty((N, H, W, 17), dtype=torch.float32, device=x.device)
        if out_seg is None:
            out_seg = torch.empty((N, H, W), dtype=torch.float32, device=x.device)
    elif out is None:
        out = torch.empty((N, H, W, 18), dtype=torch.float32, device=x.device)
    call("mpn_heatmap_head_fwd", ptr(x), ptr(w), ptr(bias), M, cin, _lib.dtype_code(x.dtype), sc, sh, act,
         int(inference), ptr(out), ptr(out_seg), stream_ptr())
    return (out, out_seg) if inference else out


def heatmap_head_bwd_bn_supported(cin, dtype):
    return bool(_lib.lib().mpn_heatmap_head_bwd_bn_supported(int(cin), _lib.dtype_code(dtype)))


def heatmap_head_bwd(x, dlogits, w, affine, dA, dw_db_out, part=None, reduce=True, bn_part=None):
    N, H, W, cin = x.shape
    M = N * H * W
    nparts = _lib.lib().mpn_heatmap_head_bwd_num_parts(M)
    nout = cin * 18 + 18
    if part is None:
        part = _f32(nparts * nout, x.device)
    sc, sh, act = _aff(affine)
    if bn_part is not None:
        if bn_part.numel() < nparts * 2 * cin:
            raise ValueError("heatmap_head_bwd: bn_part too small")
        call("mpn_heatmap_head_bwd_bn", ptr(x), ptr(dlogits), ptr(w), M, cin, _lib.dtype_code(x.dtype), sc, sh, act, ptr(dA),
             ptr(part), ptr(bn_part), stream_ptr())
    else:
        call("mpn_heatmap_head_bwd", ptr(x), ptr(dlogits), ptr(w), M, cin, _lib.dtype_code(x.dtype), sc, sh, act, ptr(dA),
             ptr(part), stream_ptr())
    if reduce:
        call("mpn_reduce_partials", ptr(part), nparts, nout, ptr(dw_db_out), 0, 1.0, stream_ptr())
    return nparts if bn_part is not None else dA


LOSS_NAMES = ["focal_loss", "regression_loss", "segmentation_loss_at_level_2", "segmentation_loss_at_level_3",
              "segmentation_loss_at_level_4", "segmentation_loss_at_level_5", "total_loss", "per_pixel_reg_loss"]


def keypoint_loss(logits, labels, ps, dlogits=None, daux=None, part=None, losses_out=None):
    B, h, w, _ = logits.shape
    dev = logits.device
    nparts = _lib.lib().mpn_keypoint_loss_num_parts(B, h, w)
    if part is None:
# ... 120 lines not shown
```

Baseline: 4289 images/s.

## Fold BN-backward apply into 1x1 and stem weight-gradient kernels

Adds variants of the 1x1 weight-gradient kernel and the stem weight-gradient kernel that apply the batch-norm backward (activation mask plus affine correction) to the incoming gradient while loading it. The 1x1 variant also writes the applied gradient back out for the following data-gradient conv. This removes a separate BN-apply pass over the activation gradient for selected channel shapes and for the stem, saving a full read and write of those tensors. In exchange it adds in-place writes, an extra buffer for wide layers, and ordering-sensitive float arithmetic meant to match the standalone apply bit for bit.

```diff
diff --git a/include/mpn.h b/include/mpn.h
--- a/include/mpn.h
+++ b/include/mpn.h
@@ -77,6 +77,12 @@
                                 int dtype, const float* in_scale, const float* in_shift, int in_act, const float* ap_scale,
                                 const float* ap_shift, const float* ap_mean, const float* ap_invstd, const float* ap_k1,
                                 const float* ap_k2, int ap_act, mpn_stream_t stream);
+int mpn_conv1x1_bwd_weight_apply_supported(int Cin, int Cout, int dtype);
+int mpn_conv1x1_bwd_weight_apply(const void* x, const void* g, const void* y_raw, void* dy_out, float* wpart, int N, int H, int W,
+                                 int Cin, int Cout, int x_stride, int g_stride, int y_stride, int out_stride, int dtype,
+                                 const float* in_scale, const float* in_shift, int in_act, const float* ap_scale,
+                                 const float* ap_shift, const float* ap_mean, const float* ap_invstd, const float* ap_k1,
+                                 const float* ap_k2, int ap_act, mpn_stream_t stream);
 int mpn_conv_wgrad_grouped_num_parts(int njobs, int N, const int* H, const int* W, int Cin, int Cout, int ksize, int dtype,
                                      int* nparts);
 int mpn_conv_bwd_weight_grouped(int njobs, const void* const* x, const void* const* dy, float* const* part, int N,
@@ -164,6 +170,10 @@
 int mpn_stem_conv_wgrad_num_parts(int N, int H, int W);
 int mpn_stem_conv_bwd_weight(const void* images, int images_u8, const void* dy, float* part, int N,
                              int H, int W, int C0, int dtype, mpn_stream_t stream);
+int mpn_stem_conv_bwd_weight_apply_supported(int C0, int dtype);
+int mpn_stem_conv_bwd_weight_apply(const void* images, int images_u8, const void* g, const void* y_raw, float* part, int N, int H,
+                                   int W, int C0, int dtype, const float* ap_scale, const float* ap_shift, const float* ap_mean,
+                                   const float* ap_invstd, const float* ap_k1, const float* ap_k2, int ap_act, mpn_stream_t stream);
 
 int mpn_bilinear_up_fwd(const void* x, void* y, int N, int h, int w, int C, int upsample,
                         int y_channel_offset, int y_channels_total, int dtype,
diff --git a/multiposenet_amd/_lib.py b/multiposenet_amd/_lib.py
--- a/multiposenet_amd/_lib.py
+++ b/multiposenet_amd/_lib.py
@@ -45,6 +45,8 @@
     "mpn_conv1x1_bwd_fused": (_I, [_P, _P, _P, _P, _P, _P, _I, _I, _I, _I, _I, _I, _I, _I, _I, _P, _P, _I, _P]),
     "mpn_conv1x1_bwd_fused_apply_supported": (_I, [_I, _I, _I]),
     "mpn_conv1x1_bwd_fused_apply": (_I, [_P, _P, _P, _P, _P, _P, _P, _I, _I, _I, _I, _I, _I, _I, _I, _I, _I, _P, _P, _I, _P, _P, _P, _P, _P, _P, _I, _P]),
+    "mpn_conv1x1_bwd_weight_apply_supported": (_I, [_I, _I, _I]),
+    "mpn_conv1x1_bwd_weight_apply": (_I, [_P, _P, _P, _P, _P, _I, _I, _I, _I, _I, _I, _I, _I, _I, _I, _P, _P, _I, _P, _P, _P, _P, _P, _P, _I, _P]),
     "mpn_conv_wgrad_grouped_num_parts": (_I, [_I, _I, _P, _P, _I, _I, _I, _I, _P]),
     "mpn_conv_bwd_weight_grouped": (_I, [_I, _P, _P, _P, _I, _P, _P, _I, _I, _P, _P, _I, _I, _P, _P, _I, _P]),
     "mpn_bn_stats_num_parts": (_I, [_L]),
@@ -73,6 +75,8 @@
     "mpn_stem_conv_fwd_stats": (_I, [_P, _I, _P, _P, _I, _I, _I, _I, _I, _P, _P]),
     "mpn_stem_conv_wgrad_num_parts": (_I, [_I, _I, _I]),
     "mpn_stem_conv_bwd_weight": (_I, [_P, _I, _P, _P, _I, _I, _I, _I, _I, _P]),
+    "mpn_stem_conv_bwd_weight_apply_supported": (_I, [_I, _I]),
+    "mpn_stem_conv_bwd_weight_apply": (_I, [_P, _I, _P, _P, _P, _I, _I, _I, _I, _I, _P, _P, _P, _P, _P, _P, _I, _P]),
     "mpn_bilinear_up_fwd": (_I, [_P, _P, _I, _I, _I, _I, _I, _I, _I, _I, _P, _P, _I, _P]),
     "mpn_bilinear_up_bwd": (_I, [_P, _P, _I, _I, _I, _I, _I, _I, _I, _I, _P]),
     "mpn_sumpool2x2": (_I, [_P, _P, _I, _I, _I, _I, _I, _I, _P]),
diff --git a/multiposenet_amd/csrc/common.h b/multiposenet_amd/csrc/common.h
--- a/multiposenet_amd/csrc/common.h
+++ b/multiposenet_amd/csrc/common.h
@@ -80,6 +80,24 @@
     return __builtin_bit_cast(unsigned, __builtin_convertvector(v, b2_t));
 }
 
+__device__ __forceinline__ void bn_apply_fold(float sc, float mean, float invstd, float k1, float k2, float& cb, float& cc) {
+#pragma clang fp contract(off)
+    cb = (-sc * k2) * invstd;
+    cc = -sc * __builtin_fmaf(-(mean * invstd), k2, k1);
+}
+__device__ __forceinline__ bool bn_apply_fuse67(long long vec_index) { return ((vec_index >> 8) & 3) == 2; }
+__device__ __forceinline__ void bn_apply_piece(float (&d)[8], const float (&y)[8], const float (&sc)[8], const float (&sh)[8],
+                                               const float (&cb)[8], const float (&cc)[8], float lo, float hi, bool fuse67) {
+#pragma clang fp contract(off)
+#pragma unroll
+    for (int j = 0; j < 8; ++j) {
+        const float pre = __builtin_fmaf(y[j], sc[j], sh[j]);
+        const float g = (pre > lo && pre < hi) ? d[j] : 0.f;
+        const float fused = __builtin_fmaf(sc[j], g, __builtin_fmaf(cb[j], y[j], cc[j]));
+        d[j] = (j < 6 || fuse67) ? fused : (cc[j] + cb[j] * y[j]) + sc[j] * g;
+    }
+}
+
 template <typename T> struct Vec16;
 template <> struct Vec16<float> {
     static constexpr int N = 4;
diff --git a/multiposenet_amd/csrc/conv_wgrad.hip b/multiposenet_amd/csrc/conv_wgrad.hip
--- a/multiposenet_amd/csrc/conv_wgrad.hip
+++ b/multiposenet_amd/csrc/conv_wgrad.hip
@@ -32,6 +32,8 @@
     int ap_xs;
     const float* ap_scale; const float* ap_shift; const float* ap_mean; const float* ap_invstd; const float* ap_k1; const float* ap_k2;
     int ap_act;
+    void* ap_out;
+    int ap_os;
 #ifdef MPN_DIAG
     unsigned long long* dbg;
 #endif
@@ -364,7 +366,7 @@
     Vec16<T> v[AVEC], dv[DVEC];
     Vec16<T> ev[DAPPLY ? DVEC : 1];
     unsigned inb = 0u, inbd = 0u;
-    static_assert(!DAPPLY || DG, "the apply pass folds into the fused thin backward");
+    static_assert(!DAPPLY || TAPS == 1, "the apply pass folds into the 1x1 kernels");
     float* apc = reinterpret_cast<float*>(Os + OBYTES + (DG ? 8 * 2 * CG * (int)sizeof(float) : 0));
     float alo = -INFINITY, ahi = INFINITY;
     if constexpr (DAPPLY) {
@@ -373,8 +375,12 @@
             const float s_ = ok ? p.ap_scale[co0 + c] : 0.f, h_ = ok ? p.ap_shift[co0 + c] : 0.f, m_ = ok ? p.ap_mean[co0 + c] : 0.f;
             const float i_ = ok ? p.ap_invstd[co0 + c] : 0.f, a_ = ok ? p.ap_k1[co0 + c] : 0.f, b_ = ok ? p.ap_k2[co0 + c] : 0.f;
             apc[c] = s_; apc[BNW + c] = h_;
-            apc[2 * BNW + c] = -s_ * b_ * i_;
-            apc[3 * BNW + c] = -s_ * (a_ - m_ * i_ * b_);
+            if constexpr (DG) {
+                apc[2 * BNW + c] = -s_ * b_ * i_;
+                apc[3 * BNW + c] = -s_ * (a_ - m_ * i_ * b_);
+            } else {
+                bn_apply_fold(s_, m_, i_, a_, b_, apc[2 * BNW + c], apc[3 * BNW + c]);
+            }
         }
         alo = (p.ap_act != MPN_ACT_NONE) ? 0.f : -INFINITY;
         ahi = (p.ap_act == MPN_ACT_RELU6) ? 6.f : INFINITY;
@@ -451,7 +457,8 @@
                 const unsigned tbE = (unsigned)tile * 128u * (unsigned)p.ap_xs * (unsigned)sizeof(T);
 #pragma unroll
                 for (int i = 0; i < DVEC; ++i) {
-                    const u32x4_t q = __builtin_amdgcn_raw_buffer_load_b128(rse, (int)(relEb[i] + tbE), 0, 0);
+                    const u32x4_t q = (!DG && p.n_cg == 1) ? __builtin_amdgcn_raw_buffer_load_b128(rse, (int)(relEb[i] + tbE), 0, 2)
+                                                          : __builtin_amdgcn_raw_buffer_load_b128(rse, (int)(relEb[i] + tbE), 0, 0);
                     ev[i].raw = make_uint4(q.x, q.y, q.z, q.w);
                 }
             }
@@ -516,7 +523,7 @@
         __builtin_amdgcn_sched_barrier(0);
     };
 
-    auto commit_tile = [&](unsigned char* As, unsigned char* Ds) {
+    auto commit_tile = [&](unsigned char* As, unsigned char* Ds, int tile) {
         float sc[VE], sh[VE];
         if (affine) {
 #pragma unroll
@@ -566,15 +573,24 @@
 #pragma unroll
                     for (int j = 0; j < 4; ++j) { asc[j4 + j] = q0[j]; ash[j4 + j] = q1[j]; acb[j4 + j] = q2[j]; acc_[j4 + j] = q3[j]; }
                 }
-#pragma unroll
-                for (int j = 0; j < VE; ++j) {
-                    const float pre = f[j] * asc[j] + ash[j];
-                    const float gg = (pre > alo && pre < ahi) ? d[j] : 0.f;
-                    d[j] = asc[j] * gg + (acb[j] * f[j] + acc_[j]);
+                if constexpr (DG) {
+#pragma unroll
+                    for (int j = 0; j < VE; ++j) {
+                        const float pre = f[j] * asc[j] + ash[j];
+                        const float gg = (pre > alo && pre < ahi) ? d[j] : 0.f;
+                        d[j] = asc[j] * gg + (acb[j] * f[j] + acc_[j]);
+                    }
+                } else {
+                    bn_apply_piece(d, f, asc, ash, acb, acc_, alo, ahi,
+                                   bn_apply_fuse67((long long)(tile * 128 + r) * (p.Cout >> 3) + (co0 >> 3) + dslot));
                 }
                 Vec16<T> o;
                 o.pack(d);
                 q = *reinterpret_cast<const uint4*>(&o.raw);
+                if constexpr (!DG) {
+                    if (cg == 0 && ((inbd >> i) & 1u))
+                        *reinterpret_cast<uint4*>(reinterpret_cast<T*>(p.ap_out) + (long long)(tile * 128 + r) * p.ap_os + co0 + dslot * VE) = q;
+                }
             }
             if ((!BUF || DAPPLY) && !((inbd >> i) & 1u)) q = make_uint4(0u, 0u, 0u, 0u);
             *reinterpret_cast<uint4*>(Ds + r * SD + dslot * 16) = q;
@@ -614,11 +630,11 @@
     }
     if (ntl > 0) load_tile(split);
     __syncthreads();
-    if (ntl > 0) commit_tile(smem, smem + NBUF * ABYTES);
+    if (ntl > 0) commit_tile(smem, smem + NBUF * ABYTES, split);
     if (grp == 1) {
         if (ntl > 1) load_tile(split + p.nsplit);
         __syncthreads();
-        if (ntl > 1) commit_tile(smem + ABYTES, smem + NBUF * ABYTES + DBYTES);
+        if (ntl > 1) commit_tile(smem + ABYTES, smem + NBUF * ABYTES + DBYTES, split + p.nsplit);
     }
 #ifdef MPN_DIAG
     if (p.dbg) t_prev = __builtin_amdgcn_s_memtime();
@@ -716,7 +732,7 @@
         MPN_WG_STAMP(2);
         if (more) {
             const int nb = NBUF == 2 ? ((it + ahead) & 1) : 0;
-            commit_tile(smem + nb * ABYTES, smem + NBUF * ABYTES + nb * DBYTES);
+            commit_tile(smem + nb * ABYTES, smem + NBUF * ABYTES + nb * DBYTES, split + (it + ahead) * p.nsplit);
         }
         if constexpr (DG) {
             const int tile = split + it * p.nsplit;
@@ -787,6 +803,11 @@
 template <typename T, int TAPS, int RBA, int RBD, int WM, bool STAGGER>
 __global__ __launch_bounds__(512, 1) void conv_wgrad_bf16_kernel(const WgradParams p) {
     conv_wgrad_bf16_body<T, TAPS, RBA, RBD, WM, STAGGER>(p, blockIdx.x, gridDim.x);
+}
+
+template <typename T, int RBA, int RBD, int WM>
+__global__ __launch_bounds__(512, 1) void conv1x1_wgrad_apply_kernel(const WgradParams p) {
+    conv_wgrad_bf16_body<T, 1, RBA, RBD, WM, false, false, true>(p, blockIdx.x, gridDim.x);
 }
 
 template <typename T, int RBA, int RBD, int WM, bool DAPPLY>
@@ -850,6 +871,17 @@
     static mpn_attr_mask_t attr_mask{0};
     MPN_HIP(mpn_ensure_dynamic_lds((const void*)conv_wgrad_bf16_kernel<T, TAPS, RBA, RBD, WM, STAGGER>, smem, &attr_mask));
     conv_wgrad_bf16_kernel<T, TAPS, RBA, RBD, WM, STAGGER><<<dim3((unsigned)(p.n_cg * p.n_cb * p.nsplit)), dim3(512), smem, st>>>(p);
+    MPN_LAUNCH_CHECK();
+    return MPN_OK;
+}
+
+template <typename T, int RBA, int RBD, int WM>
+int launch_wgrad_apply(const WgradParams& p, hipStream_t st) {
+    constexpr int smem = 2 * 128 * (RBA + 32) + 2 * 128 * (RBD + 32) + 2 * (RBA / 2) * (int)sizeof(float) + 4 * (RBD / 2) * (int)sizeof(float);
+    static_assert(smem <= 160 * 1024, "LDS budget");
+    static mpn_attr_mask_t attr_mask{0};
+    MPN_HIP(mpn_ensure_dynamic_lds((const void*)conv1x1_wgrad_apply_kernel<T, RBA, RBD, WM>, smem, &attr_mask));
+    conv1x1_wgrad_apply_kernel<T, RBA, RBD, WM><<<dim3((unsigned)(p.n_cg * p.n_cb * p.nsplit)), dim3(512), smem, st>>>(p);
     MPN_LAUNCH_CHECK();
     return MPN_OK;
 }
@@ -1145,3 +1177,42 @@
     return conv1x1_bwd_fused_impl(x, g, w, dx, wpart, bn_part, N, H, W, Cin, Cout, x_stride, g_stride, dx_stride, dtype, in_scale, in_shift,
                                   in_act, &ap, stream);
 }
+
+extern "C" int mpn_conv1x1_bwd_weight_apply_supported(int Cin, int Cout, int dtype) {
+    return (dtype == MPN_BF16 && Cin > 0 && Cout > 0 && Cin % 8 == 0 && Cout % 8 == 0 && !wgrad_thin1x1(Cin, Cout, 1)) ? 1 : 0;
+}
+
+extern "C" int mpn_conv1x1_bwd_weight_apply(const void* x, const void* g, const void* y_raw, void* dy_out, float* wpart, int N, int H, int W,
+                                            int Cin, int Cout, int x_stride, int g_stride, int y_stride, int out_stride, int dtype,
+                                            const float* in_scale, const float* in_shift, int in_act, const float* ap_scale,
+                                            const float* ap_shift, const float* ap_mean, const float* ap_invstd, const float* ap_k1,
+                                            const float* ap_k2, int ap_act, mpn_stream_t stream) {
+    MPN_REQUIRE(mpn_conv1x1_bwd_weight_apply_supported(Cin, Cout, dtype), MPN_ERR_BAD_SHAPE, "conv1x1_bwd_weight_apply: layer not covered (Cin %d, Cout %d, dtype %d)", Cin, Cout, dtype);
+    MPN_REQUIRE(x && g && y_raw && dy_out && wpart && N > 0 && H > 0 && W > 0, MPN_ERR_BAD_ARG, "conv1x1_bwd_weight_apply: bad arguments");
+    MPN_REQUIRE(ap_scale && ap_shift && ap_mean && ap_invstd && ap_k1 && ap_k2, MPN_ERR_BAD_ARG, "conv1x1_bwd_weight_apply: bad batch-norm arguments");
+    MPN_REQUIRE((in_scale == nullptr) == (in_shift == nullptr), MPN_ERR_BAD_ARG, "conv1x1_bwd_weight_apply: scale/shift mismatch");
+    MPN_REQUIRE(mpn_aligned16(x) && mpn_aligned16(g) && mpn_aligned16(y_raw) && mpn_aligned16(dy_out), MPN_ERR_BAD_ALIGN,
+                "conv1x1_bwd_weight_apply: pointers must be 16-byte aligned");
+    MPN_REQUIRE(dy_out != x && dy_out != y_raw, MPN_ERR_BAD_ARG, "conv1x1_bwd_weight_apply: dy_out must not alias x or y_raw");
+    const WgradGeom geo = wgrad_geom(N, H, W, Cin, Cout, 1, 2);
+    MPN_REQUIRE(dy_out != g || geo.n_cg == 1, MPN_ERR_BAD_ARG, "conv1x1_bwd_weight_apply: in place only with one input-channel tile (Cin <= 128)");
+    WgradParams p = {};
+    p.x = x; p.dy = g; p.part = wpart; p.in_scale = in_scale; p.in_shift = in_shift; p.in_act = in_act;
+    p.N = N; p.H = H; p.W = W; p.Cin = Cin; p.Cout = Cout;
+    p.xs = x_stride > 0 ? x_stride : Cin; p.dys = g_stride > 0 ? g_stride : Cout;
+    p.ap_x = y_raw; p.ap_xs = y_stride > 0 ? y_stride : Cout; p.ap_out = dy_out; p.ap_os = out_stride > 0 ? out_stride : Cout;
+    MPN_REQUIRE(p.xs >= Cin && p.dys >= Cout && p.ap_xs >= Cout && p.ap_os >= Cout && p.xs % 8 == 0 && p.dys % 8 == 0 && p.ap_xs % 8 == 0 &&
+                p.ap_os % 8 == 0, MPN_ERR_BAD_SHAPE, "conv1x1_bwd_weight_apply: pixel strides must be multiples of 8 not below the channel counts");
+    const long long M = (long long)N * H * W;
+    MPN_REQUIRE(M * p.xs < (1ll << 30) && M * p.dys < (1ll << 30) && M * p.ap_xs < (1ll << 30) && M * p.ap_os < (1ll << 30), MPN_ERR_BAD_SHAPE,
+                "conv1x1_bwd_weight_apply: tensors must span fewer than 2^31 bytes");
+    p.tiles_x = (W + 15) / 16; p.tiles_y = (H + 7) / 8;
+    p.M = M;
+    p.ntiles = geo.ntiles; p.nsplit = geo.nsplit; p.n_cg = geo.n_cg; p.n_cb = geo.n_cb; p.xcd_remap = 1;
+    p.ap_scale = ap_scale; p.ap_shift = ap_shift; p.ap_mean = ap_mean; p.ap_invstd = ap_invstd; p.ap_k1 = ap_k1; p.ap_k2 = ap_k2; p.ap_act = ap_act;
+#ifdef MPN_DIAG
+    p.dbg = nullptr;
+#endif
+    hipStream_t st = (hipStream_t)stream;
+    return launch_wgrad_apply<bf16_t, 256, 256, 4>(p, st);
+}
diff --git a/multiposenet_amd/csrc/stem.hip b/multiposenet_amd/csrc/stem.hip
--- a/multiposenet_amd/csrc/stem.hip
+++ b/multiposenet_amd/csrc/stem.hip
@@ -395,10 +395,11 @@
     }
 }
 
-template <bool U8, int MB>
+struct StemApply { const bf16_t* y_raw; const float *scale, *shift, *mean, *invstd, *k1, *k2; int act; };
+template <bool U8, int MB, bool AP = false>
 __global__ __launch_bounds__(kThreads) void stem_wgrad_mfma_kernel(const void* __restrict__ images, const bf16_t* __restrict__ dy,
                                                                    float* __restrict__ part, int N, int H, int W, int OH, int OW,
-                                                                   int pad_t, int pad_l, int tiles_x, int tiles_y) {
+                                                                   int pad_t, int pad_l, int tiles_x, int tiles_y, const StemApply ap) {
     typedef H16<bf16_t> HT;
     typedef HT::x8 x8;
     typedef HT::x4 x4;
@@ -408,6 +409,7 @@
     extern __shared__ __attribute__((aligned(16))) unsigned char stem_smem[];
     float* patch = reinterpret_cast<float*>(stem_smem);
     unsigned char* dimg = stem_smem + kPR * kPS * sizeof(float);
+    float* apc = reinterpret_cast<float*>(dimg + kTile * kFwdTW * DRS);
     const int ntiles = N * tiles_y * tiles_x;
     const int lane = threadIdx.x & 63, wv = threadIdx.x >> 6;
     const int n = lane & 15, kg = lane >> 4, q = n >> 2, pq = n & 3;
@@ -415,6 +417,18 @@
     constexpr int DV = kTile * kFwdTW * VPP / kThreads;
     float pv[kPR];
     uint4 dv[DV];
+    uint4 ev[AP ? DV : 1];
+    float alo = -INFINITY, ahi = INFINITY;
+    unsigned fmask = 0u;
+    if constexpr (AP) {
+        for (int c = threadIdx.x; c < C0; c += kThreads) {
+            const float s_ = ap.scale[c], b_ = ap.k2[c], i_ = ap.invstd[c];
+            apc[c] = s_; apc[C0 + c] = ap.shift[c];
+            bn_apply_fold(s_, ap.mean[c], i_, ap.k1[c], b_, apc[2 * C0 + c], apc[3 * C0 + c]);
+        }
+        alo = (ap.act != MPN_ACT_NONE) ? 0.f : -INFINITY;
+        ahi = (ap.act == MPN_ACT_RELU6) ? 6.f : INFINITY;
+    }
     unsigned long long pmask = 0ull;
     unsigned dmask = 0u;
     const int p_pc = threadIdx.x < kPC ? threadIdx.x : 0;
@@ -426,6 +440,7 @@
         const int iy0 = ty * kTile * 2 - pad_t, ix0 = tx * kFwdTW * 2 - pad_l;
         pmask = 0ull;
         dmask = 0u;
+        fmask = 0u;
         int tid = threadIdx.x;
         asm volatile("" : "+v"(tid));
         {
@@ -448,7 +463,14 @@
             const int vq = i % VPP, px = i / VPP;
             const int oy = ty * kTile + px / kFwdTW, ox = tx * kFwdTW + px % kFwdTW;
             const bool ok = oy < OH && ox < OW;
-            dv[k] = *reinterpret_cast<const uint4*>(dy + (ok ? (((long long)img * OH + oy) * OW + ox) * C0 + vq * 8 : 0));
+            const long long off = ok ? (((long long)img * OH + oy) * OW + ox) * C0 + vq * 8 : 0;
+            dv[k] = *reinterpret_cast<const uint4*>(dy + off);
+            if constexpr (AP) {
+                typedef unsigned u32x4_t __attribute__((ext_vector_type(4)));
+                const u32x4_t q4 = __builtin_nontemporal_load(reinterpret_cast<const u32x4_t*>(ap.y_raw + off));
+                ev[k] = make_uint4(q4.x, q4.y, q4.z, q4.w);
+                fmask |= (bn_apply_fuse67(off >> 3) ? 1u : 0u) << k;
+            }
             dmask |= (ok ? 1u : 0u) << k;
         }
     };
@@ -464,7 +486,28 @@
         for (int k = 0; k < DV; ++k) {
             const int i = tid + k * kThreads;
             const int vq = i % VPP, px = i / VPP;
-            *reinterpret_cast<uint4*>(dimg + px * DRS + vq * 16) = ((dmask >> k) & 1u) ? dv[k] : make_uint4(0u, 0u, 0u, 0u);
+            uint4 o4 = dv[k];
+            if constexpr (AP) {
+                Vec16<bf16_t> vd, vx;
+                vd.raw = dv[k];
+                vx.raw = ev[k];
+                float d[8], f[8], sc[8], sh[8], cb[8], cc[8];
+                vd.unpack(d);
+                vx.unpack(f);
+#pragma unroll
+                for (int j4 = 0; j4 < 8; j4 += 4) {
+                    const float4 q0 = *reinterpret_cast<const float4*>(apc + vq * 8 + j4), q1 = *reinterpret_cast<const float4*>(apc + C0 + vq * 8 + j4);
+                    const float4 q2 = *reinterpret_cast<const float4*>(apc + 2 * C0 + vq * 8 + j4), q3 = *reinterpret_cast<const float4*>(apc + 3 * C0 + vq * 8 + j4);
+                    sc[j4] = q0.x; sc[j4 + 1] = q0.y; sc[j4 + 2] = q0.z; sc[j4 + 3] = q0.w;
+                    sh[j4] = q1.x; sh[j4 + 1] = q1.y; sh[j4 + 2] = q1.z; sh[j4 + 3] = q1.w;
+                    cb[j4] = q2.x; cb[j4 + 1] = q2.y; cb[j4 + 2] = q2.z; cb[j4 + 3] = q2.w;
+                    cc[j4] = q3.x; cc[j4 + 1] = q3.y; cc[j4 + 2] = q3.z; cc[j4 + 3] = q3.w;
+                }
+                bn_apply_piece(d, f, sc, sh, cb, cc, alo, ahi, (fmask >> k) & 1u);
+                vd.pack(d);
+                o4 = vd.raw;
+            }
+            *reinterpret_cast<uint4*>(dimg + px * DRS + vq * 16) = ((dmask >> k) & 1u) ? o4 : make_uint4(0u, 0u, 0u, 0u);
         }
     };
     int kbase[2];
@@ -484,6 +527,7 @@
     int t = blockIdx.x;
     if (t < ntiles) {
         load_tile(t);
+        if constexpr (AP) __syncthreads();
         commit_tile();
     }
     for (; t < ntiles; t += gridDim.x) {
@@ -543,13 +587,13 @@
     }
 }
 
-template <bool U8, int MB>
+template <bool U8, int MB, bool AP = false>
 int launch_stem_wgrad_mfma(int grid, hipStream_t st, const void* images, const void* dy, float* part, int N, int H, int W, int OH,
-                           int OW, int pt, int pl, int tiles_x, int tiles_y) {
-    constexpr int sm = kPR * kPS * (int)sizeof(float) + kTile * kFwdTW * (16 * MB * 2 + 16);
+                           int OW, int pt, int pl, int tiles_x, int tiles_y, const StemApply& ap = StemApply{}) {
+    constexpr int sm = kPR * kPS * (int)sizeof(float) + kTile * kFwdTW * (16 * MB * 2 + 16) + (AP ? 4 * 16 * MB * (int)sizeof(float) : 0);
     static mpn_attr_mask_t attr_mask{0};
-    MPN_HIP(mpn_ensure_dynamic_lds((const void*)stem_wgrad_mfma_kernel<U8, MB>, sm, &attr_mask));
-    stem_wgrad_mfma_kernel<U8, MB><<<grid, kThreads, sm, st>>>(images, (const bf16_t*)dy, part, N, H, W, OH, OW, pt, pl, tiles_x, tiles_y);
+    MPN_HIP(mpn_ensure_dynamic_lds((const void*)stem_wgrad_mfma_kernel<U8, MB, AP>, sm, &attr_mask));
+    stem_wgrad_mfma_kernel<U8, MB, AP><<<grid, kThreads, sm, st>>>(images, (const bf16_t*)dy, part, N, H, W, OH, OW, pt, pl, tiles_x, tiles_y, ap);
     return MPN_OK;
 }
 
@@ -678,3 +722,39 @@
     MPN_LAUNCH_CHECK();
     return MPN_OK;
 }
+
+extern "C" int mpn_stem_conv_bwd_weight_apply_supported(int C0, int dtype) {
+    return (dtype == MPN_BF16 && C0 > 0 && C0 <= kMaxC0 && C0 % 16 == 0) ? 1 : 0;
+}
+
+extern "C" int mpn_stem_conv_bwd_weight_apply(const void* images, int images_u8, const void* g, const void* y_raw, float* part, int N,
+                                              int H, int W, int C0, int dtype, const float* ap_scale, const float* ap_shift,
+                                              const float* ap_mean, const float* ap_invstd, const float* ap_k1, const float* ap_k2,
+                                              int ap_act, mpn_stream_t stream) {
+    if (int rc = check(N, H, W, C0, dtype)) return rc;
+    MPN_REQUIRE(mpn_stem_conv_bwd_weight_apply_supported(C0, dtype), MPN_ERR_BAD_SHAPE, "stem_wgrad_apply: needs bf16 and C0 (%d) a multiple of 16", C0);
+    MPN_REQUIRE(images && g && y_raw && part && ap_scale && ap_shift && ap_mean && ap_invstd && ap_k1 && ap_k2, MPN_ERR_BAD_ARG,
+                "stem_wgrad_apply: null pointer");
+    MPN_REQUIRE(mpn_aligned16(g) && mpn_aligned16(y_raw), MPN_ERR_BAD_ALIGN, "stem_wgrad_apply: pointers must be 16-byte aligned");
+    int OH, OW, pt, pl;
+    same_pad(H, &OH, &pt);
+    same_pad(W, &OW, &pl);
+    const int tiles_y = (OH + kTile - 1) / kTile, tx32 = (OW + kFwdTW - 1) / kFwdTW;
+    const int grid = mpn_stem_conv_wgrad_num_parts(N, H, W);
+    hipStream_t st = (hipStream_t)stream;
+    const StemApply ap = {(const bf16_t*)y_raw, ap_scale, ap_shift, ap_mean, ap_invstd, ap_k1, ap_k2, ap_act};
+    int rc;
+#define MPN_STEM_WGA(MB)                                                                                                           \
+    rc = images_u8 ? launch_stem_wgrad_mfma<true, MB, true>(grid, st, images, g, part, N, H, W, OH, OW, pt, pl, tx32, tiles_y, ap) \
+                   : launch_stem_wgrad_mfma<false, MB, true>(grid, st, images, g, part, N, H, W, OH, OW, pt, pl, tx32, tiles_y, ap)
+    switch (C0 / 16) {
+        case 1: MPN_STEM_WGA(1); break;
+        case 2: MPN_STEM_WGA(2); break;
+        case 3: MPN_STEM_WGA(3); break;
+        default: MPN_STEM_WGA(4); break;
+    }
+#undef MPN_STEM_WGA
+    if (rc) return rc;
+    MPN_LAUNCH_CHECK();
+    return MPN_OK;
+}
diff --git a/multiposenet_amd/net.py b/multiposenet_amd/net.py
--- a/multiposenet_amd/net.py
+++ b/multiposenet_amd/net.py
@@ -101,6 +101,10 @@
 
 
 DP_DEEP_FROM_BLOCK = 7
+
+
+WGRAD_APPLY_POLICY = frozenset({(128, 128), (128, 256), (256, 256), (256, 512)})
+WGRAD_APPLY_STEM = True
 
 
 def backbone_deep_begin_of(arena, first_block=DP_DEEP_FROM_BLOCK):
@@ -170,6 +174,7 @@
         self._head_grad = self.grad[ok:ob + nb]
         self.fuse_dw_bn = True
         self.fuse_conv_bn = True
+        self.fuse_wgrad_apply = True
         self._l2 = None
         self._wd = None
         self.cache_inference_affine = False
@@ -289,6 +294,10 @@
         g["pw"] = [torch.empty_like(t) for t in b["pw"]]
         g["dw"] = [torch.empty_like(t) for t in b["dw"]]
         g["stem"] = torch.empty_like(b["stem"])
+        g["pw_applied"] = {}
+        for i, blk in enumerate(self.blocks):
+            if self._wgrad_apply(blk["pw"]) and blk["pw"].cin > 128 and b["pw"][i].shape not in g["pw_applied"]:
+                g["pw_applied"][b["pw"][i].shape] = torch.empty_like(b["pw"][i])
         lib, dc = ops._lib.lib(), ops._lib.dtype_code(dt)
         sites = []
         grouped_np = {}
@@ -567,22 +576,35 @@
         if phase == 1:
             g["bb_chain"] = (dA, reduced, lateral_added)
             return
+        if self.fuse_wgrad_apply and WGRAD_APPLY_STEM and ops.stem_conv_bwd_weight_apply_supported(g["stem"].shape[3], self.dtype):
+            ops.bn_backward(self.stem_bn, g["stem"], b["stem"], sp, reduced_parts=reduced, apply=False)
+            ops.stem_conv_bwd_weight_apply(images, g["stem"], b["stem"], self.stem_bn, slab[id(self.stem_dw)])
+            return
         ops.bn_backward(self.stem_bn, g["stem"], b["stem"], sp, reduced_parts=reduced)
         ops.stem_conv_bwd_weight(images, g["stem"], self.stem_dw, slab[id(self.stem_dw)], reduce=False)
+
+    def _wgrad_apply(self, pw):
+        return (self.fuse_wgrad_apply and (pw.cin, pw.cout) in WGRAD_APPLY_POLICY
+                and ops.conv1x1_bwd_weight_apply_supported(pw.cin, pw.cout, self.dtype))
 
     def _backward_pointwise(self, b, g, sp, slab, i, dA, reduced, raw):
         blk = self.blocks[i]
         pw, x, dY = blk["pw"], b["dw"][i], g["dw"][i]
         fused = self.fuse_conv_bn and ops.conv1x1_bwd_fused_supported(pw.cin, pw.cout, self.dtype) and pw.cin <= 64
         apply = fused and ops.conv1x1_bwd_fused_apply_supported(pw.cin, pw.cout, self.dtype)
-        ops.bn_backward(blk["pw_bn"], dA, b["pw"][i], sp, reduced_parts=reduced, raw=raw, apply=not apply)
+        wga = not fused and self._wgrad_apply(pw)
+        ops.bn_backward(blk["pw_bn"], dA, b["pw"][i], sp, reduced_parts=reduced, raw=raw, apply=not (apply or wga))
         rows = 0
         with _lib.tagged("pointwise"):
             if fused:
                 rows = ops.conv1x1_bwd_fused(x, dA, pw.w, blk["dw_bn"], dY, slab[id(pw.dw)], sp,
                                              apply_bn=blk["pw_bn"] if apply else None, y_raw=b["pw"][i] if apply else None)
             else:
-                ops.conv_bwd_weight(x, dA, 1, blk["dw_bn"].affine, pw.dw, slab[id(pw.dw)], reduce=False)
+                if wga:
+                    dA = ops.conv1x1_bwd_weight_apply(x, dA, b["pw"][i], blk["pw_bn"], blk["dw_bn"].affine,
+                                                      dA if pw.cin <= 128 else g["pw_applied"][dA.shape], slab[id(pw.dw)])
+                else:
+                    ops.conv_bwd_weight(x, dA, 1, blk["dw_bn"].affine, pw.dw, slab[id(pw.dw)], reduce=False)
                 if self.fuse_conv_bn and ops.conv_bwd_data_bn_supported(pw.cout, pw.cin, 1, self.dtype):
                     rows = ops.conv_bwd_data_bn(dA, pw.packed.bwd, pw.cin, 1, blk["dw_bn"], x, dY, sp)
                 else:
diff --git a/multiposenet_amd/ops.py b/multiposenet_amd/ops.py
--- a/multiposenet_amd/ops.py
+++ b/multiposenet_amd/ops.py
@@ -169,6 +169,25 @@
     call("mpn_conv1x1_bwd_fused", ptr(x), ptr(dy), ptr(w), ptr(out), ptr(wpart), ptr(bn_part), N, H, W, cin, cout, _slice_stride(x, cin),
          _slice_stride(dy, cout), _slice_stride(out, cin), _lib.dtype_code(x.dtype), ptr(bn.scale), ptr(bn.shift), int(bn.act), stream_ptr())
     return rows
+
+
+def conv1x1_bwd_weight_apply_supported(cin, cout, dtype):
+    return _lib.lib().mpn_conv1x1_bwd_weight_apply_supported(int(cin), int(cout), _lib.dtype_code(dtype)) == 1
+
+
+def conv1x1_bwd_weight_apply(x, g, y_raw, apply_bn, affine, dy_out, part):
+    N, H, W, cin = x.shape
+    cout = g.shape[3]
+    if part.numel() < conv_wgrad_num_parts(N, H, W, cin, cout, 1, x.dtype) * cin * cout:
+        raise ValueError("conv1x1_bwd_weight_apply: partial slab too small")
+    if dy_out.shape != g.shape or dy_out.dtype != g.dtype:
+        raise ValueError("conv1x1_bwd_weight_apply: dy_out must have g's shape and dtype")
+    sc, sh, act = _aff(affine)
+    a = apply_bn
+    call("mpn_conv1x1_bwd_weight_apply", ptr(x), ptr(g), ptr(y_raw), ptr(dy_out), ptr(part), N, H, W, cin, cout, _slice_stride(x, cin),
+         _slice_stride(g, cout), _slice_stride(y_raw, cout), _slice_stride(dy_out, cout), _lib.dtype_code(x.dtype), sc, sh, act,
+         ptr(a.scale), ptr(a.shift), ptr(a.mean), ptr(a.invstd), ptr(a.k1), ptr(a.k2), int(a.act), stream_ptr())
+    return dy_out
 
 
 def conv_wgrad_num_parts(N, H, W, cin, cout, ksize, dtype):
@@ -577,6 +596,21 @@
     return dw_out
 
 
+def stem_conv_bwd_weight_apply_supported(c0, dtype):
+    return _lib.lib().mpn_stem_conv_bwd_weight_apply_supported(int(c0), _lib.dtype_code(dtype)) == 1
+
+
+def stem_conv_bwd_weight_apply(images, g, y_raw, apply_bn, part):
+    N, H, W, _ = images.shape
+    c0 = g.shape[3]
+    if part.numel() < _lib.lib().mpn_stem_conv_wgrad_num_parts(N, H, W) * 27 * c0:
+        raise ValueError("stem_conv_bwd_weight_apply: partial slab too small")
+    a = apply_bn
+    call("mpn_stem_conv_bwd_weight_apply", ptr(images), int(images.dtype == torch.uint8), ptr(g), ptr(y_raw), ptr(part), N, H, W, c0,
+         _lib.dtype_code(g.dtype), ptr(a.scale), ptr(a.shift), ptr(a.mean), ptr(a.invstd), ptr(a.k1), ptr(a.k2), int(a.act), stream_ptr())
+    return part
+
+
 def bilinear_up_fwd(x, upsample, out, channel_offset, affine=None):
     N, h, w, C = x.shape
     sc, sh, act = _aff(affine)
```

New measurement: 4307 images/s, median of 6. Within noise of the previous version (+0.4%).
